# Leqr/MSMP-PDE

Measured on AMD Instinct MI355X. Metric: rollout-steps/sec (whole node), E2 nx=100 tw=25, higher is better.
Workload: dtype f32; 1 GPU; E2 MSMP-PDE (MP_PDE_SolverLEMLinGated), 2048 graphs x nx=100, time_window=25, 6 gated layer pairs, radius graph n=3; graphs_total=2048, graphs_per_gpu=2048, nodes_per_gpu=204800, edges_per_gpu=1204224, parallelism=dp1 (graph-sharded, no collective in the rollout), sub_batches=1, range_policy_switched_to_exact_fp32=False, preheat=170 untimed steps (>= 1 s) after the 5 warm-up steps

## Files before the change

### include/msmp_pde.h

```cpp
#ifndef MSMP_PDE_H
#define MSMP_PDE_H

#include <stddef.h>
#include <stdint.h>

#if defined(__GNUC__)
#pragma GCC visibility push(default)
#endif

#ifdef __cplusplus
extern "C" {
#endif

#define MSMP_HIDDEN 128
#define MSMP_MAX_VARS 8

#define MSMP_OK               0
#define MSMP_ERR_ARG         -1
#define MSMP_ERR_UNSUPPORTED -2
#define MSMP_ERR_WORKSPACE   -3
#define MSMP_ERR_HIP         -4

#define MSMP_LAYER_RESIDUAL_SWISH 0
#define MSMP_LAYER_LIN            1
#define MSMP_LAYER_DENSE_MESSAGE  16

typedef void* msmp_stream_t;

#define MSMP_ABI_VERSION 400
int msmp_version(void);
const char* msmp_last_error(void);

#define MSMP_STATUS_INPUT_RANGE    1
#define MSMP_STATUS_NODE_SATURATED 2
#define MSMP_STATUS_NONFINITE      4
int msmp_last_status(int* flags_out, int reset);
int msmp_tune(const char* key, int value);
int msmp_tune_query(const char* key);

int64_t msmp_packed_layer_floats(int tw, int nv);

int msmp_pack_layer_f32(const float* w1, const float* b1, const float* w2, const float* b2,
                        const float* w3, const float* b3, const float* w4, const float* b4,
                        int tw, int nv, float* packed_out, msmp_stream_t stream);

size_t msmp_build_csr_workspace_bytes(int64_t n_edges, int64_t n_nodes);
int msmp_build_csr(const int64_t* edge_index, int64_t n_edges, int64_t n_nodes,
                   int32_t* rowptr_out, int32_t* col_out, int32_t* tgt_out,
                   void* workspace, size_t workspace_bytes, msmp_stream_t stream);

int msmp_radius_graph_count_f64(const double* x, int dim, const int32_t* graph_ptr, int64_t n_graphs,
                                int64_t n_nodes, double r, int max_neighbors,
                                int32_t* rowptr_out, msmp_stream_t stream);
int msmp_radius_graph_fill_f64(const double* x, int dim, const int32_t* graph_ptr, int64_t n_graphs,
                               int64_t n_nodes, double r, int max_neighbors, const int32_t* rowptr,
                               int64_t n_edges, int64_t* edge_index_out, msmp_stream_t stream);

int msmp_knn_graph_f64(const double* x, int dim, const int32_t* graph_ptr, int64_t n_graphs,
                       int64_t n_nodes, int k, int64_t n_edges, int32_t* rowptr_out,
                       int64_t* edge_index_out, msmp_stream_t stream);

int msmp_edge_mlp_f32(const float* h, const float* u, const float* pos, const float* vars,
                      const int32_t* tgt, const int32_t* col, int64_t n_nodes, int64_t n_edges,
                      int tw, int nv, const float* packed, float* msg_out, msmp_stream_t stream);

int msmp_edge_aggregate_f32(const float* h, const float* u, const float* pos, const float* vars,
                            const int32_t* rowptr, const int32_t* col, const int32_t* tgt,
                            int64_t n_nodes, int64_t n_edges, int max_in_degree, int tw, int nv,
                            const float* packed, float* agg_out, msmp_stream_t stream);

int msmp_node_project_f32(const float* h, const float* u, const float* pos, const float* vars,
                          int64_t n_nodes, int tw, int nv, const float* packed, float* p_out,
                          float* q_out, msmp_stream_t stream);
int msmp_edge_aggregate_projected_f32(const float* p, const float* q, const int32_t* rowptr,
                                      const int32_t* col, const int32_t* tgt, int64_t n_nodes,
                                      int64_t n_edges, int max_in_degree, int tw, int nv,
                                      const float* packed, float* agg_out, msmp_stream_t stream);

#define MSMP_TILE_NCAP  32
#define MSMP_TILE_EDGES 128
typedef struct {
    int32_t tile_nodes;
    int32_t group_nodes;
    int32_t n_tiles;
    const int32_t* tile_node;
    const int32_t* tile_count;
    const int32_t* tile_halo;
    const int32_t* edge_slot;
    int32_t listed;
    int32_t period_tiles;
    int32_t period_nodes;
} msmp_tiles_t;
int msmp_build_tiles(const int32_t* rowptr, const int32_t* col, int64_t n_nodes, int64_t n_edges, int group_nodes,
                     int32_t* tile_node_out, int32_t* tile_count_out, int32_t* tile_halo_out, int32_t* edge_slot_out,
                     int32_t* stats_out, msmp_stream_t stream);
int msmp_node_feature_stride(int tw, int nv);
int msmp_prepare_nodes(const void* x, int x_f64, const void* pos, int pos_f64, int64_t n_nodes, int tw, double L, double tmax,
                       int n_cols, const void* const* cols, const int* col_f64, const double* col_div, float* u_out,
                       float* pos_x_out, float* pos_t_out, float* vars_out, float* feat_out, msmp_stream_t stream);
int msmp_pack_node_features_f32(const float* u, const float* pos, const float* vars, int64_t n_nodes, int tw, int nv,
                                float* feat_out, msmp_stream_t stream);
int msmp_edge_aggregate_tiled_f32(const float* h, const float* u, const float* pos, const float* vars, const float* feat,
                                  const float* p, const float* q, const int32_t* rowptr, const msmp_tiles_t* tiles, int64_t n_nodes,
                                  int64_t n_edges, int tw, int nv, const float* packed, float* agg_out, msmp_stream_t stream);

int msmp_scatter_mean_f32(const float* msg, const int32_t* rowptr, int64_t n_nodes,
                          float* agg_out, msmp_stream_t stream);

int msmp_node_update_f32(const float* h, const float* agg, const float* vars, int64_t n_nodes, int nv,
                         const float* packed, int mode, float* out, msmp_stream_t stream);

int msmp_node_tail_f32(const float* h, const float* agg_main, const float* agg_gate, const float* vars,
                       const int32_t* graph_ptr, int64_t n_nodes, int64_t n_graphs, int max_graph_nodes, int nv,
                       const float* packed_main, const float* packed_gate, int mode, float eps, float* out,
                       msmp_stream_t stream);

int msmp_instance_norm_f32(const float* x, const int32_t* graph_ptr, int64_t n_graphs,
                           int max_graph_nodes, float eps, float* out, msmp_stream_t stream);

int msmp_gate_blend_f32(const float* h, const float* gate_pre, const float* main_pre,
                        const int32_t* graph_ptr, int64_t n_graphs, int max_graph_nodes, float eps,
                        float* out, msmp_stream_t stream);

size_t msmp_mp_layer_workspace_bytes(int64_t n_nodes, int64_t n_edges, int gated, int max_in_degree);
int msmp_mp_layer_f32(const float* h, const float* u, const float* pos, const float* vars,
                      const float* feat, const int32_t* rowptr, const int32_t* col, const int32_t* tgt,
                      const msmp_tiles_t* tiles, const int32_t* graph_ptr, int64_t n_nodes, int64_t n_edges, int64_t n_graphs,
                      int max_in_degree, int max_graph_nodes, int tw, int nv, const float* packed_main,
                      const float* packed_gate, int mode,
                      float eps, float* h_out, void* workspace, size_t workspace_bytes,
                      msmp_stream_t stream);

typedef struct {
    const float* w1;
    const float* b1;
    const float* w2;
    const float* b2;
    const float* u;
    float dt;
    int32_t time_window;
    float* out;
} msmp_decoder_t;
int msmp_mp_layer_decode_f32(const float* h, const float* u, const float* pos, const float* vars,
                             const float* feat, const int32_t* rowptr, const int32_t* col, const int32_t* tgt,
                             const msmp_tiles_t* tiles, const int32_t* graph_ptr, int64_t n_nodes, int64_t n_edges, int64_t n_graphs,
                             int max_in_degree, int max_graph_nodes, int tw, int nv, const float* packed_main,
                             const float* packed_gate, int mode,
                             float eps, float* h_out, const msmp_decoder_t* dec, void* workspace, size_t workspace_bytes,
                             msmp_stream_t stream);

int64_t msmp_packed_lem_floats(void);
int msmp_pack_lem_f32(const float* weights, const float* weights_lin_z, const float* bias,
                      const float* bias_lin_z, const float* mlp_w0, const float* mlp_b0,
                      const float* mlp_w1, const float* mlp_b1, int ninp, float* packed_out,
                      msmp_stream_t stream);

int msmp_lem_input_stride(int ninp);

int msmp_lem_encoder_f32(const float* xin, int64_t n_nodes, int t_len, int ninp, float dt,
                         const float* packed, int with_mlp, float* h_out, msmp_stream_t stream);

int msmp_decoder_f32(const float* h, const float* u, int64_t n_nodes, int tw, const float* w1,
                     const float* b1, const float* w2, const float* b2, float dt, float* out,
                     msmp_stream_t stream);

int msmp_decoder2d_f32(const float* hd, const float* u, int64_t n_nodes, int tw, const float* w1,
                       const float* b1, const float* w2, const float* b2, float dt, float* out,
                       msmp_stream_t stream);

size_t msmp_linear_swish_workspace_bytes(int k, int n_out);
int msmp_linear_swish_f32(const float* x, int64_t rows, int k, const float* w, const float* bias, int n_out, float* out,
                          void* workspace, size_t workspace_bytes, msmp_stream_t stream);

int msmp_lem_encoder_nodes_f32(const float* u, const float* pos_x, const float* pos_t, const float* vars, const float* dt_cum,
                               int64_t n_nodes, int tw, int nv, int two_d, float dt, const float* packed, int with_mlp,
                               float* h_out, msmp_stream_t stream);

int64_t msmp_lem_saved_floats(int64_t n_nodes, int t_len);
int msmp_lem_train_fwd_f32(const float* xin, int64_t n_nodes, int t_len, int ninp, float dt, const float* packed,
                           const float* y0, const float* z0, float* saved, float* y_out, float* z_out, msmp_stream_t stream);
int64_t msmp_packed_lem_bwd_floats(void);
int msmp_pack_lem_bwd_f32(const float* weights, const float* weights_lin_z, int ninp, float* packed_out,
                          msmp_stream_t stream);
int msmp_lem_train_bwd_f32(const float* grad_y, const float* saved, const float* y0, const float* z0, int64_t n_nodes, int t_len,
                           float dt, const float* packed_bwd, float* dg_out, msmp_stream_t stream);

size_t msmp_mp_layer_bwd_workspace_bytes(int64_t n_nodes, int64_t n_edges, int tw, int nv, int gated);
int msmp_mp_layer_bwd_f32(const float* grad_out, const float* h, const float* u, const float* pos, const float* vars,
                          const int32_t* rowptr, const int32_t* col, const int32_t* tgt, const int32_t* src_rowptr,
                          const int32_t* src_perm, const int32_t* graph_ptr,
                          int64_t n_nodes, int64_t n_edges, int64_t n_graphs, int tw, int nv,
                          const float* const* params_main, const float* const* params_gate, int mode, float eps,
                          float* dh_out, float* const* grads_main, float* const* grads_gate, void* workspace,
                          size_t workspace_bytes, msmp_stream_t stream);

int msmp_adamw_f32(int n_tensors, float* const* params, const float* const* grads, float* const* exp_avg,
                   float* const* exp_avg_sq, const int64_t* numel, float lr, float beta1, float beta2, float eps,
                   float weight_decay, int64_t step, msmp_stream_t stream);
int msmp_adamw_capturable_f32(int n_tensors, float* const* params, const float* const* grads, float* const* exp_avg,
                              float* const* exp_avg_sq, const int64_t* numel, const float* lr_dev, float beta1, float beta2,
                              float eps, float weight_decay, int64_t* step_dev, msmp_stream_t stream);

size_t msmp_reduce_workspace_bytes(int cols);
int msmp_colsum_f32(const float* x, int64_t rows, int cols, int group, float* out, void* workspace, size_t workspace_bytes,
                    msmp_stream_t stream);
int msmp_sqerr_sum_f32(const float* a, const float* b, int64_t n, float* out, void* workspace, size_t workspace_bytes,
                       msmp_stream_t stream);

int msmp_edge_concat_f32(const float* h, const float* u, const float* pos, const float* vars, const int32_t* tgt,
                         const int32_t* col, int64_t n_edges, int tw, int nv, int ld, float* out, msmp_stream_t stream);
int msmp_mean_bwd_dswish_f32(const float* dagg, const int32_t* rowptr, const int32_t* tgt, const float* a2, int64_t n_edges,
                             float* out, msmp_stream_t stream);
int msmp_instance_norm_bwd_f32(const float* x, const float* grad_y, const int32_t* graph_ptr, int64_t n_graphs, float eps,
                               float* dx_out, msmp_stream_t stream);
int msmp_gate_blend_bwd_f32(const float* grad_out, const float* h, const float* gate_pre, const float* main_pre,
                            const int32_t* graph_ptr, int64_t n_graphs, float eps, float* d_gate_pre, float* d_main_pre,
                            float* dh_out, msmp_stream_t stream);

int64_t msmp_grad_weights_workspace_floats(int n_jobs, const int64_t* rows, const int* k2);
int msmp_grad_weights_f32(int n_jobs, const float* const* a, const float* const* b, const int64_t* rows, const int* lda,
                          const int* ldb, const int* k2, float* const* out_w, float* const* out_b, float* workspace,
                          int64_t workspace_floats, msmp_stream_t stream);
int msmp_grad_weights_cat_f32(int n_jobs, const float* const* a, const float* const* b, const float* const* b2, const int64_t* rows,
                              const int* lda, const int* ldb, const int* ldb2, const int* ksplit, const int* k2, float* const* out_w,
                              float* const* out_b, float* workspace, int64_t workspace_floats, msmp_stream_t stream);

int64_t msmp_packed_mlp2_floats(int k_in);
int msmp_mlp2_input_stride(int k_in);
int msmp_pack_mlp2_f32(const float* w1, const float* b1, const float* w2, const float* b2, int k_in, float* packed_out,
                       msmp_stream_t stream);
int msmp_mlp2_swish_f32(const float* x, int64_t n_nodes, int k_in, const float* packed, float* out, msmp_stream_t stream);

size_t msmp_linear_workspace_bytes(int k, int n_out);
int msmp_linear_f32(const float* x, int ldx, int64_t rows, int k, const float* w, int ldw, const float* bias, int n_out, int mode,
                    float* out, int ld_out, void* workspace, size_t workspace_bytes, msmp_stream_t stream);
int msmp_wide_gather_swish_f32(const float* p, const float* q, const int32_t* tgt, const int32_t* col, int64_t n_edges, int width, int ld,
                               float* out, msmp_stream_t stream);
int msmp_wide_scatter_mean_f32(const float* msg, const int32_t* rowptr, int64_t n_nodes, int width, int ld, float* agg_out, msmp_stream_t stream);
int msmp_wide_swish_f32(const float* x, int64_t n_floats, float* out, msmp_stream_t stream);
int msmp_wide_lem_z_f32(const float* g, int64_t n_nodes, int width, float dt, float* z, float* dtbar_out, msmp_stream_t stream);
int msmp_wide_lem_y_f32(const float* lin, const float* dtbar, int64_t n_floats, float* y, msmp_stream_t stream);
int msmp_wide_norm_blend_f32(const float* h, const float* gate_pre, const float* main_pre, const int32_t* graph_ptr, int64_t n_graphs,
                             int width, int ld, float eps, float* out, msmp_stream_t stream);

#define MSMP_K_EDGE_MLP     0
#define MSMP_K_SCATTER_MEAN 1
#define MSMP_K_NODE_UPDATE  2
#define MSMP_K_NORM         3
// ... 16 lines not shown
```

### msmp-pde_amd/_lib.py

```python
import ctypes
import os
from ctypes import c_int, c_int64, c_size_t, c_void_p, c_float, c_double, c_char_p

PKG = os.path.dirname(os.path.abspath(__file__))
LIB_PATH = os.environ.get('MSMP_LIB_PATH') or os.path.join(PKG, 'libmsmp_pde.so')

class MsmpTiles(ctypes.Structure):
    _fields_ = [('tile_nodes', ctypes.c_int32), ('group_nodes', ctypes.c_int32), ('n_tiles', ctypes.c_int32), ('tile_node', c_void_p), ('tile_count', c_void_p),
                ('tile_halo', c_void_p), ('edge_slot', c_void_p), ('listed', ctypes.c_int32), ('period_tiles', ctypes.c_int32), ('period_nodes', ctypes.c_int32)]


class MsmpDecoder(ctypes.Structure):
    _fields_ = [('w1', c_void_p), ('b1', c_void_p), ('w2', c_void_p), ('b2', c_void_p), ('u', c_void_p), ('dt', ctypes.c_float),
                ('time_window', ctypes.c_int32), ('out', c_void_p)]


MSMP_TILE_NCAP = 32
MSMP_TILE_EDGES = 128
MSMP_TILE_GROUP_EDGES = 32
MSMP_LAYER_RESIDUAL_SWISH = 0
MSMP_LAYER_LIN = 1
MSMP_ERR_UNSUPPORTED = -2
MSMP_MAX_VARS = 8
HIDDEN = 128
MSMP_ABI_VERSION = 400
MSMP_STATUS_INPUT_RANGE, MSMP_STATUS_NODE_SATURATED, MSMP_STATUS_NONFINITE = 1, 2, 4

SIGNATURES = {
    'msmp_version': (c_int, []),
    'msmp_last_error': (c_char_p, []),
    'msmp_last_status': (c_int, [ctypes.POINTER(c_int), c_int]),
    'msmp_tune': (c_int, [c_char_p, c_int]),
    'msmp_tune_query': (c_int, [c_char_p]),
    'msmp_packed_layer_floats': (c_int64, [c_int, c_int]),
    'msmp_pack_layer_f32': (c_int, [c_void_p] * 8 + [c_int, c_int, c_void_p, c_void_p]),
    'msmp_build_csr_workspace_bytes': (c_size_t, [c_int64, c_int64]),
    'msmp_build_csr': (c_int, [c_void_p, c_int64, c_int64, c_void_p, c_void_p, c_void_p, c_void_p, c_size_t, c_void_p]),
    'msmp_radius_graph_count_f64': (c_int, [c_void_p, c_int, c_void_p, c_int64, c_int64, c_double, c_int, c_void_p, c_void_p]),
    'msmp_radius_graph_fill_f64': (c_int, [c_void_p, c_int, c_void_p, c_int64, c_int64, c_double, c_int, c_void_p, c_int64,
                                           c_void_p, c_void_p]),
    'msmp_knn_graph_f64': (c_int, [c_void_p, c_int, c_void_p, c_int64, c_int64, c_int, c_int64, c_void_p, c_void_p, c_void_p]),
    'msmp_edge_mlp_f32': (c_int, [c_void_p] * 6 + [c_int64, c_int64, c_int, c_int, c_void_p, c_void_p, c_void_p]),
    'msmp_scatter_mean_f32': (c_int, [c_void_p, c_void_p, c_int64, c_void_p, c_void_p]),
    'msmp_node_update_f32': (c_int, [c_void_p, c_void_p, c_void_p, c_int64, c_int, c_void_p, c_int, c_void_p, c_void_p]),
    'msmp_instance_norm_f32': (c_int, [c_void_p, c_void_p, c_int64, c_int, c_float, c_void_p, c_void_p]),
    'msmp_gate_blend_f32': (c_int, [c_void_p, c_void_p, c_void_p, c_void_p, c_int64, c_int, c_float, c_void_p, c_void_p]),
    'msmp_edge_aggregate_f32': (c_int, [c_void_p] * 7 + [c_int64, c_int64, c_int, c_int, c_int, c_void_p, c_void_p, c_void_p]),
    'msmp_node_project_f32': (c_int, [c_void_p] * 4 + [c_int64, c_int, c_int, c_void_p, c_void_p, c_void_p, c_void_p]),
    'msmp_edge_aggregate_projected_f32': (c_int, [c_void_p] * 5 + [c_int64, c_int64, c_int, c_int, c_int, c_void_p, c_void_p, c_void_p]),
    'msmp_build_tiles': (c_int, [c_void_p, c_void_p, c_int64, c_int64, c_int, c_void_p, c_void_p, c_void_p, c_void_p, c_void_p, c_void_p]),
    'msmp_node_feature_stride': (c_int, [c_int, c_int]),
    'msmp_prepare_nodes': (c_int, [c_void_p, c_int, c_void_p, c_int, c_int64, c_int, c_double, c_double, c_int, c_void_p, c_void_p, c_void_p,
                                   c_void_p, c_void_p, c_void_p, c_void_p, c_void_p, c_void_p]),
    'msmp_pack_node_features_f32': (c_int, [c_void_p, c_void_p, c_void_p, c_int64, c_int, c_int, c_void_p, c_void_p]),
    'msmp_edge_aggregate_tiled_f32': (c_int, [c_void_p] * 8 + [ctypes.POINTER(MsmpTiles), c_int64, c_int64, c_int, c_int, c_void_p, c_void_p, c_void_p]),
    'msmp_mp_layer_workspace_bytes': (c_size_t, [c_int64, c_int64, c_int, c_int]),
    'msmp_mp_layer_f32': (c_int, [c_void_p] * 8 + [ctypes.POINTER(MsmpTiles), c_void_p] + [c_int64, c_int64, c_int64, c_int, c_int, c_int, c_int, c_void_p, c_void_p, c_int,
                                                   c_float, c_void_p, c_void_p, c_size_t, c_void_p]),
    'msmp_mp_layer_decode_f32': (c_int, [c_void_p] * 8 + [ctypes.POINTER(MsmpTiles), c_void_p] + [c_int64, c_int64, c_int64, c_int, c_int, c_int, c_int, c_void_p, c_void_p, c_int,
                                                          c_float, c_void_p, ctypes.POINTER(MsmpDecoder), c_void_p, c_size_t, c_void_p]),
    'msmp_packed_lem_floats': (c_int64, []),
    'msmp_pack_lem_f32': (c_int, [c_void_p] * 8 + [c_int, c_void_p, c_void_p]),
    'msmp_lem_input_stride': (c_int, [c_int]),
    'msmp_lem_encoder_f32': (c_int, [c_void_p, c_int64, c_int, c_int, c_float, c_void_p, c_int, c_void_p, c_void_p]),
    'msmp_decoder_f32': (c_int, [c_void_p, c_void_p, c_int64, c_int, c_void_p, c_void_p, c_void_p, c_void_p, c_float, c_void_p, c_void_p]),
    'msmp_decoder2d_f32': (c_int, [c_void_p, c_void_p, c_int64, c_int, c_void_p, c_void_p, c_void_p, c_void_p, c_float, c_void_p, c_void_p]),
    'msmp_node_tail_f32': (c_int, [c_void_p] * 5 + [c_int64, c_int64, c_int, c_int, c_void_p, c_void_p, c_int, c_float, c_void_p, c_void_p]),
    'msmp_lem_encoder_nodes_f32': (c_int, [c_void_p] * 5 + [c_int64, c_int, c_int, c_int, c_float, c_void_p, c_int, c_void_p, c_void_p]),
    'msmp_lem_saved_floats': (c_int64, [c_int64, c_int]),
    'msmp_lem_train_fwd_f32': (c_int, [c_void_p, c_int64, c_int, c_int, c_float] + [c_void_p] * 7),
    'msmp_packed_lem_bwd_floats': (c_int64, []),
    'msmp_pack_lem_bwd_f32': (c_int, [c_void_p, c_void_p, c_int, c_void_p, c_void_p]),
    'msmp_lem_train_bwd_f32': (c_int, [c_void_p] * 4 + [c_int64, c_int, c_float, c_void_p, c_void_p, c_void_p]),
    'msmp_edge_concat_f32': (c_int, [c_void_p] * 6 + [c_int64, c_int, c_int, c_int, c_void_p, c_void_p]),
    'msmp_mean_bwd_dswish_f32': (c_int, [c_void_p] * 4 + [c_int64, c_void_p, c_void_p]),
    'msmp_instance_norm_bwd_f32': (c_int, [c_void_p, c_void_p, c_void_p, c_int64, c_float, c_void_p, c_void_p]),
    'msmp_gate_blend_bwd_f32': (c_int, [c_void_p] * 5 + [c_int64, c_float, c_void_p, c_void_p, c_void_p, c_void_p]),
    'msmp_grad_weights_workspace_floats': (c_int64, [c_int, c_void_p, c_void_p]),
    'msmp_grad_weights_f32': (c_int, [c_int] + [c_void_p] * 9 + [c_int64, c_void_p]),
    'msmp_grad_weights_cat_f32': (c_int, [c_int] + [c_void_p] * 12 + [c_int64, c_void_p]),
    'msmp_mp_layer_bwd_workspace_bytes': (c_size_t, [c_int64, c_int64, c_int, c_int, c_int]),
    'msmp_mp_layer_bwd_f32': (c_int, [c_void_p] * 11 + [c_int64, c_int64, c_int64, c_int, c_int, c_void_p, c_void_p, c_int, c_float,
                                      c_void_p, c_void_p, c_void_p, c_void_p, c_size_t, c_void_p]),
    'msmp_adamw_f32': (c_int, [c_int, c_void_p, c_void_p, c_void_p, c_void_p, c_void_p, c_float, c_float, c_float, c_float, c_float, c_int64, c_void_p]),
    'msmp_adamw_capturable_f32': (c_int, [c_int, c_void_p, c_void_p, c_void_p, c_void_p, c_void_p, c_void_p, c_float, c_float, c_float, c_float, c_void_p, c_void_p]),
    'msmp_reduce_workspace_bytes': (c_size_t, [c_int]),
    'msmp_colsum_f32': (c_int, [c_void_p, c_int64, c_int, c_int, c_void_p, c_void_p, c_size_t, c_void_p]),
    'msmp_sqerr_sum_f32': (c_int, [c_void_p, c_void_p, c_int64, c_void_p, c_void_p, c_size_t, c_void_p]),
    'msmp_packed_mlp2_floats': (c_int64, [c_int]),
    'msmp_mlp2_input_stride': (c_int, [c_int]),
    'msmp_pack_mlp2_f32': (c_int, [c_void_p] * 4 + [c_int, c_void_p, c_void_p]),
    'msmp_mlp2_swish_f32': (c_int, [c_void_p, c_int64, c_int, c_void_p, c_void_p, c_void_p]),
    'msmp_linear_swish_workspace_bytes': (c_size_t, [c_int, c_int]),
    'msmp_linear_swish_f32': (c_int, [c_void_p, c_int64, c_int, c_void_p, c_void_p, c_int, c_void_p, c_void_p, c_size_t, c_void_p]),
    'msmp_linear_workspace_bytes': (c_size_t, [c_int, c_int]),
    'msmp_linear_f32': (c_int, [c_void_p, c_int, c_int64, c_int, c_void_p, c_int, c_void_p, c_int, c_int, c_void_p, c_int, c_void_p, c_size_t, c_void_p]),
    'msmp_wide_gather_swish_f32': (c_int, [c_void_p, c_void_p, c_void_p, c_void_p, c_int64, c_int, c_int, c_void_p, c_void_p]),
    'msmp_wide_scatter_mean_f32': (c_int, [c_void_p, c_void_p, c_int64, c_int, c_int, c_void_p, c_void_p]),
    'msmp_wide_swish_f32': (c_int, [c_void_p, c_int64, c_void_p, c_void_p]),
    'msmp_wide_lem_z_f32': (c_int, [c_void_p, c_int64, c_int, c_float, c_void_p, c_void_p, c_void_p]),
    'msmp_wide_lem_y_f32': (c_int, [c_void_p, c_void_p, c_int64, c_void_p, c_void_p]),
    'msmp_wide_norm_blend_f32': (c_int, [c_void_p, c_void_p, c_void_p, c_void_p, c_int64, c_int, c_int, c_float, c_void_p, c_void_p]),
    'msmp_timing_enable': (c_int, [c_int]),
    'msmp_timing_reset': (c_int, []),
    'msmp_timing_read': (c_int, [c_int, ctypes.POINTER(c_int64), ctypes.POINTER(c_double)]),
}

K_EDGE_MLP, K_SCATTER_MEAN, K_NODE_UPDATE, K_NORM, K_LEM, K_NODE_PROJ, K_DECODER = 0, 1, 2, 3, 4, 5, 6
MSMP_LAYER_DENSE_MESSAGE = 16

_lib = None


class MsmpError(RuntimeError):
    pass


def lib():
    global _lib
    if _lib is None:
        if not os.path.exists(LIB_PATH):
            raise MsmpError(f'{LIB_PATH} not found: build it with `python msmp-pde_amd/build.py` '
                            '(or __graft_entry__.build()); there is no CPU fallback')
        handle = ctypes.CDLL(LIB_PATH)
        for name, (res, args) in SIGNATURES.items():
            fn = getattr(handle, name)
            fn.restype = res
            fn.argtypes = args
        if handle.msmp_version() != MSMP_ABI_VERSION:
            raise MsmpError(f'{LIB_PATH} reports ABI version {handle.msmp_version()}, this binding was written for {MSMP_ABI_VERSION}: '
                            'rebuild it with `python msmp-pde_amd/build.py`')
        _lib = handle
    return _lib


def check(rc, what=''):
    if rc != 0:
        msg = lib().msmp_last_error()
        raise MsmpError(f'{what} failed with code {rc}: {msg.decode() if msg else ""}')


def ptr(t):
    return None if t is None else t.data_ptr()


PARAM_EPOCH = [0]


def invalidate_packed_weights(*_args, **_kwargs):
    PARAM_EPOCH[0] += 1


def _install_optimizer_hook():
    try:
        from torch.optim.optimizer import register_optimizer_step_post_hook
        register_optimizer_step_post_hook(invalidate_packed_weights)
    except Exception as exc:
        import warnings
        warnings.warn(f'msmp_pde_amd: no global optimizer hook ({exc}); call invalidate_packed_weights() after fused optimizer steps')


_install_optimizer_hook()

_raw_stream = None


def current_stream():
    global _raw_stream
    import torch
    if _raw_stream is None:
        _raw_stream = getattr(torch._C, '_cuda_getCurrentRawStream', False)
    if _raw_stream:
        return _raw_stream(torch.cuda.current_device())
    return torch.cuda.current_stream().cuda_stream


def timing_read(kernel):
    n, ms = c_int64(0), c_double(0.0)
    check(lib().msmp_timing_read(kernel, ctypes.byref(n), ctypes.byref(ms)), 'msmp_timing_read')
    return n.value, ms.value


class MsmpRangeWarning(RuntimeWarning):
    """A value left the range the default (fp16-split) kernels represent: results are saturated or not finite."""


_STATUS_TEXT = {
    MSMP_STATUS_INPUT_RANGE: 'an input feature (u, pos / L or a variables column) has |x| > 255 or is not finite',
    MSMP_STATUS_NODE_SATURATED: 'a hidden-state / aggregate row has |x| > 255 or is NaN (saturated at 255.87 in the GEMM operands)',
    MSMP_STATUS_NONFINITE: 'the InstanceNorm statistics of a graph are not finite (an activation above 1023 overflowed fp16 upstream)',
}
_status_seen = [0]


def last_status(reset=False):
    flags = c_int(0)
    check(lib().msmp_last_status(ctypes.byref(flags), int(bool(reset))), 'msmp_last_status')
    if reset:
        _status_seen[0] = 0
    return flags.value


def status_check():
# ... 29 lines not shown
```

### msmp-pde_amd/csrc/aux_kernels.hip

```cpp
#include <stdarg.h>
#include "graph_norm.h"
#include <vector>
#include "mfma_tiles.h"

namespace msmp {

static thread_local char g_err[512] = "";

void set_error(const char* fmt, ...) {
    va_list ap;
    va_start(ap, fmt);
    vsnprintf(g_err, sizeof(g_err), fmt, ap);
    va_end(ap);
}

int check_launch(const char* what) {
    const hipError_t e = hipGetLastError();
    if (e != hipSuccess) {
        set_error("%s: %s", what, hipGetErrorString(e));
        return MSMP_ERR_HIP;
    }
    return MSMP_OK;
}

// ... 367 lines not shown
    MSMP_REQUIRE(flags_out, MSMP_ERR_ARG, "msmp_last_status: null pointer");
    int* dp = status_ptr();
    *flags_out = 0;
    if (g_status_mode == 1) {
        *flags_out = __atomic_load_n(g_status_host, __ATOMIC_RELAXED);
        if (reset) __atomic_store_n(g_status_host, 0, __ATOMIC_RELAXED);
    } else if (g_status_mode == 2) {
        hipError_t e = hipMemcpy(flags_out, dp, sizeof(int), hipMemcpyDeviceToHost);
        if (e == hipSuccess && reset) e = hipMemset(dp, 0, sizeof(int));
        MSMP_REQUIRE(e == hipSuccess, MSMP_ERR_HIP, "msmp_last_status: %s", hipGetErrorString(e));
    } else {
        MSMP_REQUIRE(false, MSMP_ERR_HIP, "msmp_last_status: no status word (allocation failed)");
    }
    return MSMP_OK;
}

extern "C" int msmp_version(void) { return MSMP_ABI_VERSION; }
extern "C" const char* msmp_last_error(void) { return g_err; }

extern "C" int64_t msmp_packed_layer_floats(int tw, int nv) {
    if (tw <= 0 || nv < 1 || nv > MSMP_MAX_VARS) return -1;
    return packed_layout(tw, nv).total;
}

extern "C" int msmp_pack_layer_f32(const float* w1, const float* b1, const float* w2, const float* b2,
                                   const float* w3, const float* b3, const float* w4, const float* b4,
                                   int tw, int nv, float* packed_out, msmp_stream_t stream) {
    MSMP_REQUIRE(w1 && b1 && w2 && b2 && w3 && b3 && w4 && b4 && packed_out, MSMP_ERR_ARG, "msmp_pack_layer_f32: null pointer");
    MSMP_REQUIRE(tw > 0 && nv >= 1 && nv <= MSMP_MAX_VARS, MSMP_ERR_ARG, "msmp_pack_layer_f32: bad tw=%d nv=%d", tw, nv);
    PackArgs a{w1, b1, w2, b2, w3, b3, w4, b4, tw, nv, packed_out};
    hipLaunchKernelGGL(pack_layer_kernel, dim3(256), dim3(256), 0, (hipStream_t)stream, a);
    hipLaunchKernelGGL(pack_layer_scale_kernel, dim3(4), dim3(256), 0, (hipStream_t)stream, a);
    hipLaunchKernelGGL(pack_layer_split_kernel, dim3(256), dim3(256), 0, (hipStream_t)stream, a);
    return check_launch("pack_layer_kernel");
}

extern "C" int msmp_scatter_mean_f32(const float* msg, const int32_t* rowptr, int64_t n_nodes, float* agg_out,
                                     msmp_stream_t stream) {
    MSMP_REQUIRE(rowptr && agg_out, MSMP_ERR_ARG, "msmp_scatter_mean_f32: null pointer");
    MSMP_REQUIRE(n_nodes > 0 && n_nodes < (1L << 31), MSMP_ERR_ARG, "msmp_scatter_mean_f32: bad n_nodes");
    const unsigned grid = (unsigned)((n_nodes + 7) / 8);
    timing_begin(MSMP_K_SCATTER_MEAN, (hipStream_t)stream);
    hipLaunchKernelGGL(scatter_mean_kernel, dim3(grid), dim3(256), 0, (hipStream_t)stream, msg, rowptr, (long)n_nodes, agg_out, msmp_tune_get("split") ? status_ptr() : nullptr);
    timing_end(MSMP_K_SCATTER_MEAN, (hipStream_t)stream);
    return check_launch("scatter_mean_kernel");
}

static const int kRegNormMaxNodes = 128;

extern "C" int msmp_instance_norm_f32(const float* x, const int32_t* graph_ptr, int64_t n_graphs, int max_graph_nodes, float eps,
                                      float* out, msmp_stream_t stream) {
    const int g_max_graph_nodes = max_graph_nodes;
    MSMP_REQUIRE(x && graph_ptr && out, MSMP_ERR_ARG, "msmp_instance_norm_f32: null pointer");
    MSMP_REQUIRE(n_graphs > 0 && n_graphs < (1L << 31), MSMP_ERR_ARG, "msmp_instance_norm_f32: bad n_graphs");
    timing_begin(MSMP_K_NORM, (hipStream_t)stream);
    if (g_max_graph_nodes > 0 && g_max_graph_nodes <= 104)
        hipLaunchKernelGGL(instance_norm_reg_kernel<13>, dim3((unsigned)n_graphs), dim3(256), 0, (hipStream_t)stream, x, graph_ptr, eps, out);
    else if (g_max_graph_nodes > 0 && g_max_graph_nodes <= kRegNormMaxNodes)
        hipLaunchKernelGGL(instance_norm_reg_kernel<16>, dim3((unsigned)n_graphs), dim3(256), 0, (hipStream_t)stream, x, graph_ptr, eps, out);
    else
    hipLaunchKernelGGL(instance_norm_kernel, dim3((unsigned)n_graphs), dim3(256), 0, (hipStream_t)stream, x, graph_ptr, eps, out);
    timing_end(MSMP_K_NORM, (hipStream_t)stream);
    return check_launch("instance_norm_kernel");
}

extern "C" int msmp_gate_blend_f32(const float* h, const float* gate_pre, const float* main_pre, const int32_t* graph_ptr,
                                   int64_t n_graphs, int max_graph_nodes, float eps, float* out, msmp_stream_t stream) {
    const int g_max_graph_nodes = max_graph_nodes;
    MSMP_REQUIRE(h && gate_pre && main_pre && graph_ptr && out, MSMP_ERR_ARG, "msmp_gate_blend_f32: null pointer");
    MSMP_REQUIRE(n_graphs > 0 && n_graphs < (1L << 31), MSMP_ERR_ARG, "msmp_gate_blend_f32: bad n_graphs");
    timing_begin(MSMP_K_NORM, (hipStream_t)stream);
    if (g_max_graph_nodes > 0 && g_max_graph_nodes <= 104)
        hipLaunchKernelGGL(gate_blend_reg_kernel<13>, dim3((unsigned)n_graphs), dim3(256), 0, (hipStream_t)stream, h, gate_pre,
                           main_pre, graph_ptr, eps, out);
    else if (g_max_graph_nodes > 0 && g_max_graph_nodes <= kRegNormMaxNodes)
        hipLaunchKernelGGL(gate_blend_reg_kernel<16>, dim3((unsigned)n_graphs), dim3(256), 0, (hipStream_t)stream, h, gate_pre,
                           main_pre, graph_ptr, eps, out);
    else
    hipLaunchKernelGGL(gate_blend_kernel, dim3((unsigned)n_graphs), dim3(256), 0, (hipStream_t)stream, h, gate_pre, main_pre,
                       graph_ptr, eps, out);
    timing_end(MSMP_K_NORM, (hipStream_t)stream);
    return check_launch("gate_blend_kernel");
}

static size_t align256(size_t b) { return (b + 255) & ~(size_t)255; }
static bool fused_ok(int max_in_degree) { return max_in_degree >= 0 && max_in_degree <= 256; }

extern "C" size_t msmp_mp_layer_workspace_bytes(int64_t n_nodes, int64_t n_edges, int gated, int max_in_degree) {
    const size_t msg = fused_ok(max_in_degree) ? 0 : align256((size_t)n_edges * H * sizeof(float));
    const size_t nod = align256((size_t)n_nodes * H * sizeof(float));
    (void)gated;
    return msg + nod * 6 + 256;
}

static int mp_layer_impl(const float* h, const float* u, const float* pos, const float* vars, const float* feat,
                         const int32_t* rowptr, const int32_t* col, const int32_t* tgt, const msmp_tiles_t* tiles,
                         const int32_t* graph_ptr,
                         int64_t n_nodes, int64_t n_edges, int64_t n_graphs, int max_in_degree, int max_graph_nodes,
                         int tw, int nv, const float* packed_main, const float* packed_gate, int mode, float eps, float* h_out,
                         const msmp_decoder_t* dec, void* workspace, size_t workspace_bytes, msmp_stream_t stream);

extern "C" int msmp_mp_layer_f32(const float* h, const float* u, const float* pos, const float* vars, const float* feat,
                                 const int32_t* rowptr, const int32_t* col, const int32_t* tgt, const msmp_tiles_t* tiles,
                                 const int32_t* graph_ptr,
                                 int64_t n_nodes, int64_t n_edges, int64_t n_graphs, int max_in_degree, int max_graph_nodes,
                                 int tw, int nv, const float* packed_main, const float* packed_gate, int mode, float eps, float* h_out,
                                 void* workspace, size_t workspace_bytes, msmp_stream_t stream) {
    return mp_layer_impl(h, u, pos, vars, feat, rowptr, col, tgt, tiles, graph_ptr, n_nodes, n_edges, n_graphs, max_in_degree, max_graph_nodes, tw, nv,
                         packed_main, packed_gate, mode, eps, h_out, nullptr, workspace, workspace_bytes, stream);
}

extern "C" int msmp_mp_layer_decode_f32(const float* h, const float* u, const float* pos, const float* vars, const float* feat,
                                        const int32_t* rowptr, const int32_t* col, const int32_t* tgt, const msmp_tiles_t* tiles,
                                        const int32_t* graph_ptr,
                                        int64_t n_nodes, int64_t n_edges, int64_t n_graphs, int max_in_degree, int max_graph_nodes,
                                        int tw, int nv, const float* packed_main, const float* packed_gate, int mode, float eps, float* h_out,
                                        const msmp_decoder_t* dec, void* workspace, size_t workspace_bytes, msmp_stream_t stream) {
    MSMP_REQUIRE(dec, MSMP_ERR_ARG, "msmp_mp_layer_decode_f32: null decoder description");
    MSMP_REQUIRE(dec->time_window == 25 && msmp_tune_get("split") && msmp_tune_get("tail") && max_graph_nodes > 0 && max_graph_nodes <= 128,
                 MSMP_ERR_UNSUPPORTED, "msmp_mp_layer_decode_f32: the fused tail does not apply (time_window %d, max_graph_nodes %d)", dec->time_window,
                 max_graph_nodes);
    return mp_layer_impl(h, u, pos, vars, feat, rowptr, col, tgt, tiles, graph_ptr, n_nodes, n_edges, n_graphs, max_in_degree, max_graph_nodes, tw, nv,
                         packed_main, packed_gate, mode, eps, h_out, dec, workspace, workspace_bytes, stream);
}

static int mp_layer_impl(const float* h, const float* u, const float* pos, const float* vars, const float* feat,
                         const int32_t* rowptr, const int32_t* col, const int32_t* tgt, const msmp_tiles_t* tiles,
                         const int32_t* graph_ptr,
                         int64_t n_nodes, int64_t n_edges, int64_t n_graphs, int max_in_degree, int max_graph_nodes,
                         int tw, int nv, const float* packed_main, const float* packed_gate, int mode, float eps, float* h_out,
                         const msmp_decoder_t* dec, void* workspace, size_t workspace_bytes, msmp_stream_t stream) {
    MSMP_REQUIRE(h && u && pos && vars && rowptr && col && tgt && graph_ptr && packed_main && h_out && workspace,
                 MSMP_ERR_ARG, "msmp_mp_layer_f32: null pointer");
    MSMP_REQUIRE(h_out != h, MSMP_ERR_ARG, "msmp_mp_layer_f32: h_out may not alias h");
    MSMP_REQUIRE(!tiles || msmp_tiles_ok(tiles, n_nodes), MSMP_ERR_ARG, "msmp_mp_layer_f32: tile descriptor does not cover %ld nodes", (long)n_nodes);
    const int gated = packed_gate != nullptr;
    const bool dense = (mode & MSMP_LAYER_DENSE_MESSAGE) != 0;
    mode &= ~MSMP_LAYER_DENSE_MESSAGE;
    MSMP_REQUIRE(!gated || mode == MSMP_LAYER_LIN, MSMP_ERR_ARG, "msmp_mp_layer_f32: the gated pair uses GNN_LayerLin layers");
    const size_t need = msmp_mp_layer_workspace_bytes(n_nodes, n_edges, gated, max_in_degree);
    MSMP_REQUIRE(workspace_bytes >= need, MSMP_ERR_WORKSPACE, "msmp_mp_layer_f32: workspace %zu < %zu", workspace_bytes, need);
    const bool fused = fused_ok(max_in_degree);
    char* ws = (char*)workspace;
    float* msg = (float*)ws;
    if (!fused) ws += align256((size_t)n_edges * H * sizeof(float));
    const size_t nod = align256((size_t)n_nodes * H * sizeof(float));
    float* const agg = (float*)ws;
    float* pre_main = (float*)(ws + nod);
    float* pre_gate = (float*)(ws + 2 * nod);
    float* pbuf = (float*)(ws + 3 * nod);
    float* qbuf = (float*)(ws + 4 * nod);
    int rc;
    int tile_mode = (tiles && n_edges > 0 && msmp_tune_get("split")) ? msmp_tune_get("tile") : 0;
    if (tile_mode == 2 && n_edges < (int64_t)76 * tiles->n_tiles) tile_mode = 0;
    if (tile_mode == 3) tile_mode = 2;
    auto aggregate = [&](const float* packed, float* agg) -> int {
        if (fused && !dense && tile_mode == 2)
            return msmp_edge_aggregate_tiled_f32(h, u, pos, vars, feat, nullptr, nullptr, rowptr, tiles, n_nodes, n_edges, tw, nv, packed, agg, stream);
        if (fused && !dense && tile_mode == 1) {
            const int r = msmp_node_project_f32(h, u, pos, vars, n_nodes, tw, nv, packed, pbuf, qbuf, stream);
            return r ? r : msmp_edge_aggregate_tiled_f32(nullptr, nullptr, nullptr, nullptr, nullptr, pbuf, qbuf, rowptr, tiles, n_nodes, n_edges, tw,
                                                         nv, packed, agg, stream);
        }
        if (fused && !dense) {
            const int r = msmp_node_project_f32(h, u, pos, vars, n_nodes, tw, nv, packed, pbuf, qbuf, stream);
            return r ? r : msmp_edge_aggregate_projected_f32(pbuf, qbuf, rowptr, col, tgt, n_nodes, n_edges, max_in_degree, tw,
                                                              nv, packed, agg, stream);
        }
        if (fused)
            return msmp_edge_aggregate_f32(h, u, pos, vars, rowptr, col, tgt, n_nodes, n_edges, max_in_degree, tw, nv, packed,
                                           agg, stream);
        const int r = msmp_edge_mlp_f32(h, u, pos, vars, tgt, col, n_nodes, n_edges, tw, nv, packed, msg, stream);
        return r ? r : msmp_scatter_mean_f32(msg, rowptr, n_nodes, agg, stream);
    };
    if (msmp_tune_get("split") && msmp_tune_get("tail") && max_graph_nodes > 0 && max_graph_nodes <= 128) {
        rc = MSMP_ERR_UNSUPPORTED;
        if (gated && fused && !dense && tile_mode == 2 && msmp_tune_get("pair") && (msmp_tune_get("pair") == 2 || n_nodes <= 65536))
            rc = msmp_edge_aggregate_tiled_pair(h, u, pos, vars, feat, rowptr, tiles, n_nodes, n_edges, tw, nv, packed_gate, packed_main, pre_gate,
                                                agg, stream);
        else if (gated && fused && !dense && !tile_mode)
            rc = msmp_pair_project_aggregate(h, u, pos, vars, rowptr, col, tgt, n_nodes, n_edges, max_in_degree, tw, nv, packed_gate,
                                             packed_main, pbuf, qbuf, pre_main, (float*)(ws + 5 * nod), pre_gate, agg, stream);
        if (rc == MSMP_ERR_UNSUPPORTED) {
            if (gated && (rc = aggregate(packed_gate, pre_gate))) return rc;
            if ((rc = aggregate(packed_main, agg))) return rc;
        } else if (rc) return rc;
        return msmp_node_tail_impl(h, agg, gated ? pre_gate : nullptr, vars, graph_ptr, n_nodes, n_graphs, max_graph_nodes, nv,
                                   packed_main, packed_gate, mode, eps, h_out, dec, stream);
    }
    MSMP_REQUIRE(!dec, MSMP_ERR_UNSUPPORTED, "msmp_mp_layer_decode_f32: the fused tail does not apply");
    if (gated) {
        if ((rc = aggregate(packed_gate, agg))) return rc;
        if ((rc = msmp_node_update_f32(h, agg, vars, n_nodes, nv, packed_gate, MSMP_LAYER_LIN, pre_gate, stream))) return rc;
    }
    if ((rc = aggregate(packed_main, agg))) return rc;
    if ((rc = msmp_node_update_f32(h, agg, vars, n_nodes, nv, packed_main, mode, pre_main, stream))) return rc;
    if (gated) return msmp_gate_blend_f32(h, pre_gate, pre_main, graph_ptr, n_graphs, max_graph_nodes, eps, h_out, stream);
    return msmp_instance_norm_f32(pre_main, graph_ptr, n_graphs, max_graph_nodes, eps, h_out, stream);
}
```

### msmp-pde_amd/csrc/mlp_kernels.hip

```cpp
#include <string.h>
#include "mfma_tiles.h"
#include "decoder_body.h"

namespace msmp {

struct EdgeArgs {
    const float* h;
    const float* u;
    const float* pos;
    const float* vars;
    const int* tgt;
    const int* col;
    const int* rowptr;
    long n_edges, n_nodes;
    int tile_nodes;
    int xcd_map;
    int tw, nv, nc1;
    const float* w1;
    const float* w2;
    const float* w2s;
    const float* scales;
    const float* b1;
    const float* b2;
    const float* P;
// ... 1074 lines not shown
    const int c = lane & 31, hh = lane >> 5;
    const int n0 = a.graph_ptr[blockIdx.x], n1 = a.graph_ptr[blockIdx.x + 1];
    const int cnt = n1 - n0;
    if (cnt <= 0) return;
    const long n = (long)n0 + wave * 32 + c;
    const long nc = n < n1 ? n : n1 - 1;

    PROF_DECL
#pragma unroll
    for (int i = 0; i < 4; ++i) {
        const int e = tid + 256 * i, row = e >> 3, f = e & 7;
        const float v = a.vars[(size_t)min(n0 + row, n1 - 1) * a.nv + min(f, a.nv - 1)];
        xvl[e] = v * (row < cnt && f < a.nv ? 1.0f : 0.f);
    }
    f32x16 tau[4];
    if (GATED) {
        tail_rows_issue(a.h, a.agg[1], n0, n1, 0, rowbuf, tid);
        head_compute(rowbuf, n0, n1, a.h, a.agg[1], a.vars, nc, a.nv, a.b3[1], a.b4[1], a.w3vh[1], a.w3s[1], a.w4t[1], a.scales[1], lds, xvl, tid, lane,
                     c, hh, tau, [&] { tail_rows_issue(a.h, a.agg[0], n0, n1, 0, rowbuf, tid); }, true, tot PROF_PASS);
        PROF_MARK(0);
        tile_t_instance_norm(tau, wave, cnt, uniform_ro(a.scales[1], 7) * (1.0f / TAIL_ACT_SCALE), a.eps, part, tot, tid, c, hh, a.status);
#pragma unroll
        for (int T = 0; T < 4; ++T)
#pragma unroll
            for (int r = 0; r < 16; ++r) tau[T][r] = sigmoidf_(tau[T][r]);
        PROF_MARK(1);
    } else {
        tail_rows_issue(a.h, a.agg[0], n0, n1, 0, rowbuf, tid);
    }
    f32x16 y[4];
    head_compute(rowbuf, n0, n1, a.h, a.agg[0], a.vars, nc, a.nv, a.b3[0], a.b4[0], a.w3vh[0], a.w3s[0], a.w4t[0], a.scales[0], lds, xvl, tid, lane, c, hh,
                 y, [] {}, GATED || a.mode == MSMP_LAYER_LIN, tot PROF_PASS);
    PROF_MARK(2);
    const size_t base = ((size_t)n0 + wave * 32 + 4 * hh) * H + 4 * c;
    const int lim = cnt - wave * 32 - 4 * hh;
    const bool full = wave * 32 + 32 <= cnt;
    const bool need_h = GATED || a.mode != MSMP_LAYER_LIN;
    f32x4 hx[16];
    if (need_h) {
        if (full) {
#pragma unroll
            for (int r = 0; r < 16; ++r) hx[r] = *reinterpret_cast<const f32x4*>(a.h + base + (size_t)((r & 3) + 8 * (r >> 2)) * H);
        } else {
#pragma unroll
            for (int r = 0; r < 16; ++r) {
                const int row = (r & 3) + 8 * (r >> 2);
                hx[r] = row < lim ? *reinterpret_cast<const f32x4*>(a.h + base + (size_t)row * H) : f32x4{0.f, 0.f, 0.f, 0.f};
            }
        }
    }
    float unit = uniform_ro(a.scales[0], 7) * (1.0f / TAIL_ACT_SCALE);
    if (!GATED && a.mode != MSMP_LAYER_LIN) {
#pragma unroll
        for (int T = 0; T < 4; ++T)
#pragma unroll
            for (int r = 0; r < 16; ++r) y[T][r] = hx[r][T] + swishf(y[T][r] * unit);
        unit = 1.0f;
    }
    tile_t_instance_norm(y, wave, cnt, unit, a.eps, part, tot, tid, c, hh, a.status);
    if (need_h) {
        float mx = 0.f;
#pragma unroll
        for (int r = 0; r < 16; ++r) mx = fmaxf(fmaxf(fmaxf(fabsf(hx[r][0]), fabsf(hx[r][1])), fmaxf(fabsf(hx[r][2]), fabsf(hx[r][3]))), mx);
        if (mx > NODE_RANGE) status_raise(a.status, MSMP_STATUS_NODE_SATURATED);
    }
    PROF_MARK(3);
    if (GATED) {
#pragma unroll
        for (int T = 0; T < 4; ++T)
#pragma unroll
            for (int r = 0; r < 16; ++r) y[T][r] = fmaf(tau[T][r], swishf(y[T][r]) - hx[r][T], hx[r][T]);
    }
    if (full) {
#pragma unroll
        for (int r = 0; r < 16; ++r)
            *reinterpret_cast<f32x4*>(a.out + base + (size_t)((r & 3) + 8 * (r >> 2)) * H) = f32x4{y[0][r], y[1][r], y[2][r], y[3][r]};
    } else {
#pragma unroll
        for (int r = 0; r < 16; ++r) {
            const int row = (r & 3) + 8 * (r >> 2);
            if (row < lim) *reinterpret_cast<f32x4*>(a.out + base + (size_t)row * H) = f32x4{y[0][r], y[1][r], y[2][r], y[3][r]};
        }
    }
    PROF_MARK(4);
    if (a.dec.w1) {
        using G = DecSplit<25, 16, 3, 14>;
        static_assert(16 * 8 * G::LP <= 2 * SPLIT_CHUNK_FLOATS && 16 * 8 * G::LP <= 2 * ROWBUF_FLOATS, "decoder tables must fit the dead buffers");
        __syncthreads();
        const int q = tid & 7, nl = tid >> 3;
        float* mrow = (nl < 16 ? lds : rowbuf) + (nl & 15) * 8 * G::LP;
        for (int p = 0; p < cnt; p += 32) {
            const bool live = p + nl < cnt;
            const long nn = live ? (long)n0 + p + nl : (long)n1 - 1;
            decoder_split_node<25, 16, 3, 14, true>(a.out + (size_t)nn * H, mrow, q, live, nn, a.dec, [] { __syncthreads(); });
            __syncthreads();
        }
    }
    PROF_FLUSH
}

}

using namespace msmp;

extern int g_lem_tail;
extern int g_lem_share;
static int* split_status() { return msmp_tune_get("split") ? msmp::status_ptr() : nullptr; }
static int g_split = 1;

extern "C" int msmp_edge_mlp_f32(const float* h, const float* u, const float* pos, const float* vars,
                                 const int32_t* tgt, const int32_t* col, int64_t n_nodes, int64_t n_edges,
                                 int tw, int nv, const float* packed, float* msg_out, msmp_stream_t stream) {
    MSMP_REQUIRE(h && u && pos && vars && tgt && col && packed && msg_out, MSMP_ERR_ARG, "msmp_edge_mlp_f32: null pointer");
    MSMP_REQUIRE(n_nodes > 0 && n_edges >= 0 && tw > 0 && nv >= 1 && nv <= MSMP_MAX_VARS, MSMP_ERR_ARG,
                 "msmp_edge_mlp_f32: bad sizes N=%ld E=%ld tw=%d nv=%d", (long)n_nodes, (long)n_edges, tw, nv);
    MSMP_REQUIRE(n_edges < (1L << 31) && n_nodes < (1L << 31), MSMP_ERR_UNSUPPORTED, "msmp_edge_mlp_f32: int32 index range");
    if (n_edges == 0) return MSMP_OK;
    const PackedLayout L = packed_layout(tw, nv);
    EdgeArgs a{h, u, pos, vars, tgt, col, nullptr, (long)n_edges, (long)n_nodes, 0, 0, tw, nv, L.nc1,
               packed + L.w1, packed + L.w2, packed + L.w2s, packed + L.scales, packed + L.b1, packed + L.b2, nullptr, nullptr, msg_out, nullptr, split_status()};
    constexpr int NB = 2;
    const unsigned grid = (unsigned)((n_edges + 128 * NB - 1) / (128 * NB));
    timing_begin(MSMP_K_EDGE_MLP, (hipStream_t)stream);
    hipLaunchKernelGGL((edge_mlp_kernel<NB, false, false>), dim3(grid), dim3(256), 0, (hipStream_t)stream, a);
    timing_end(MSMP_K_EDGE_MLP, (hipStream_t)stream);
    return check_launch("edge_mlp_kernel");
}

extern "C" int msmp_node_project_f32(const float* h, const float* u, const float* pos, const float* vars, int64_t n_nodes,
                                     int tw, int nv, const float* packed, float* p_out, float* q_out, msmp_stream_t stream) {
    MSMP_REQUIRE(h && u && pos && vars && packed && p_out && q_out, MSMP_ERR_ARG, "msmp_node_project_f32: null pointer");
    MSMP_REQUIRE(n_nodes > 0 && n_nodes < (1L << 31) && tw > 0 && nv >= 1 && nv <= MSMP_MAX_VARS, MSMP_ERR_ARG,
                 "msmp_node_project_f32: bad sizes");
    const PackedLayout L = packed_layout(tw, nv);
    ProjArgs a{h, u, pos, vars, (long)n_nodes, tw, nv, L.nc1, packed + L.w1, packed + L.b1, p_out, q_out};
    const unsigned grid = (unsigned)((n_nodes + 127) / 128);
    timing_begin(MSMP_K_NODE_PROJ, (hipStream_t)stream);
    if (g_split) {
        ProjSplitArgs sa{a, packed + L.w1t, packed + L.scales};
        hipLaunchKernelGGL(node_proj_split_kernel, dim3(grid), dim3(256), 0, (hipStream_t)stream, sa);
    } else
        hipLaunchKernelGGL(node_proj_kernel, dim3(grid), dim3(256), 0, (hipStream_t)stream, a);
    timing_end(MSMP_K_NODE_PROJ, (hipStream_t)stream);
    return check_launch("node_proj_kernel");
}

static int g_edge_nb = 0;

static int g_pair = 1;
constexpr int64_t PAIR_MAX_NODES = 65536;
static int g_decoder = 1;
static int g_tile_arith = 1;
static int g_tile_align = 0;
static int g_tile = 2;
static int g_bwd_gemm = 1;
static int g_dec_fuse = 0;
static int g_tail = 1;
int msmp_tune_get(const char* key) {
    if (!strcmp(key, "split")) return g_split;
    if (!strcmp(key, "tail")) return g_tail;
    if (!strcmp(key, "bwd_gemm")) return g_bwd_gemm;
    if (!strcmp(key, "pair")) return g_pair;
    if (!strcmp(key, "tile")) return g_tile;
    if (!strcmp(key, "tile_arith")) return g_tile_arith;
    if (!strcmp(key, "tile_align")) return g_tile_align;
    if (!strcmp(key, "decoder")) return g_decoder;
    if (!strcmp(key, "dec_fuse")) return g_dec_fuse;
    if (!strcmp(key, "lem_tail")) return g_lem_tail;
    if (!strcmp(key, "lem_share")) return g_lem_share;
    return 0;
}

extern "C" int msmp_tune_query(const char* key) { return key ? msmp_tune_get(key) : 0; }

extern "C" int msmp_tune(const char* key, int value) {
    if (key && !strcmp(key, "tail")) { g_tail = value; return MSMP_OK; }
    if (key && !strcmp(key, "bwd_gemm")) { g_bwd_gemm = value; return MSMP_OK; }
    if (key && !strcmp(key, "pair")) { g_pair = value; return MSMP_OK; }
    if (key && !strcmp(key, "tile")) { g_tile = value; return MSMP_OK; }
    if (key && !strcmp(key, "tile_arith")) { g_tile_arith = value; return MSMP_OK; }
    if (key && !strcmp(key, "tile_align")) { g_tile_align = value; return MSMP_OK; }
    if (key && !strcmp(key, "decoder")) { g_decoder = value != 0; return MSMP_OK; }
    if (key && !strcmp(key, "dec_fuse")) { g_dec_fuse = value != 0; return MSMP_OK; }
    if (key && !strcmp(key, "lem_tail")) { g_lem_tail = value != 0; return MSMP_OK; }
    if (key && !strcmp(key, "lem_share") && value >= 1 && value <= 16) { g_lem_share = value; return MSMP_OK; }
    if (key && !strcmp(key, "edge_nb")) { g_edge_nb = value; return MSMP_OK; }
    if (key && !strcmp(key, "split")) { g_split = value; return MSMP_OK; }
    msmp::set_error("msmp_tune: unknown key");
    return MSMP_ERR_ARG;
}

static int edge_aggregate(const float* h, const float* u, const float* pos, const float* vars, const float* P, const float* Q,
                          const int32_t* rowptr, const int32_t* col, const int32_t* tgt, int64_t n_nodes, int64_t n_edges,
                          int max_in_degree, int tw, int nv, const float* packed, float* agg_out, msmp_stream_t stream,
                          const char* who) {
    MSMP_REQUIRE(rowptr && col && tgt && packed && agg_out, MSMP_ERR_ARG, "%s: null pointer", who);
    MSMP_REQUIRE(n_nodes > 0 && n_edges >= 0 && tw > 0 && nv >= 1 && nv <= MSMP_MAX_VARS && max_in_degree >= 0, MSMP_ERR_ARG,
                 "%s: bad sizes", who);
    MSMP_REQUIRE(n_edges < (1L << 31) && n_nodes < (1L << 31), MSMP_ERR_UNSUPPORTED, "%s: int32 index range", who);
    if (n_edges == 0) {
        const hipError_t me = hipMemsetAsync(agg_out, 0, (size_t)n_nodes * H * sizeof(float), (hipStream_t)stream);
        MSMP_REQUIRE(me == hipSuccess, MSMP_ERR_HIP, "%s: memset: %s", who, hipGetErrorString(me));
        return MSMP_OK;
    }
    MSMP_REQUIRE(max_in_degree <= 256, MSMP_ERR_UNSUPPORTED,
                 "%s: max in-degree %d > 256 (use msmp_edge_mlp_f32 + msmp_scatter_mean_f32)", who, max_in_degree);
    const int edges_per_tile = (P && max_in_degree <= 128 && g_edge_nb != 2) ? 128 : 256;
    const PackedLayout L = packed_layout(tw, nv);
    int tile_nodes = max_in_degree > 0 ? edges_per_tile / max_in_degree : edges_per_tile;
    if (tile_nodes > 256) tile_nodes = 256;
    EdgeArgs a{h, u, pos, vars, tgt, col, rowptr, (long)n_edges, (long)n_nodes, tile_nodes, 0, tw, nv, L.nc1,
               packed + L.w1, packed + L.w2, packed + L.w2s, packed + L.scales, packed + L.b1, packed + L.b2, P, Q, nullptr, agg_out, split_status()};
    const unsigned grid = (unsigned)((n_nodes + tile_nodes - 1) / tile_nodes);
    timing_begin(MSMP_K_EDGE_MLP, (hipStream_t)stream);
    if (P && edges_per_tile == 128 && g_split) hipLaunchKernelGGL((edge_mlp_kernel_occ2<1, true, true, true>), dim3(grid), dim3(256), 0, (hipStream_t)stream, a);
    else if (P && edges_per_tile == 128) hipLaunchKernelGGL((edge_mlp_kernel<1, true, true>), dim3(grid), dim3(256), 0, (hipStream_t)stream, a);
    else if (P) hipLaunchKernelGGL((edge_mlp_kernel<2, true, true>), dim3(grid), dim3(256), 0, (hipStream_t)stream, a);
    else hipLaunchKernelGGL((edge_mlp_kernel<2, true, false>), dim3(grid), dim3(256), 0, (hipStream_t)stream, a);
    timing_end(MSMP_K_EDGE_MLP, (hipStream_t)stream);
    return check_launch("edge_mlp_kernel<fused mean>");
}

int msmp_pair_project_aggregate(const float* h, const float* u, const float* pos, const float* vars, const int32_t* rowptr,
                                const int32_t* col, const int32_t* tgt, int64_t n_nodes, int64_t n_edges, int max_in_degree, int tw,
                                int nv, const float* packed_a, const float* packed_b, float* p_a, float* q_a, float* p_b, float* q_b,
                                float* agg_a, float* agg_b, msmp_stream_t stream) {
    if (!g_pair || (g_pair == 1 && n_nodes > PAIR_MAX_NODES)) return MSMP_ERR_UNSUPPORTED;
    if (!g_split || g_edge_nb == 2) return MSMP_ERR_UNSUPPORTED;
    if (n_edges <= 0 || max_in_degree <= 0 || max_in_degree > 128 || n_edges >= (1L << 31) || n_nodes >= (1L << 31)) return MSMP_ERR_UNSUPPORTED;
    const PackedLayout L = packed_layout(tw, nv);
    hipStream_t st = (hipStream_t)stream;
    ProjSplitArgs2 pa;
    const float* packed[2] = {packed_a, packed_b};
    float* pp[2] = {p_a, p_b};
    float* qq[2] = {q_a, q_b};
    float* agg[2] = {agg_a, agg_b};
    for (int i = 0; i < 2; ++i)
        pa.head[i] = ProjSplitArgs{ProjArgs{h, u, pos, vars, (long)n_nodes, tw, nv, L.nc1, packed[i] + L.w1, packed[i] + L.b1, pp[i], qq[i]},
                                   packed[i] + L.w1t, packed[i] + L.scales};
    timing_begin(MSMP_K_NODE_PROJ, st);
    hipLaunchKernelGGL(node_proj_split_pair_kernel, dim3((unsigned)((n_nodes + 127) / 128), 2), dim3(256), 0, st, pa);
    timing_end(MSMP_K_NODE_PROJ, st);
    int tile_nodes = 128 / max_in_degree;
    if (tile_nodes > 256) tile_nodes = 256;
    EdgeArgs2 ea;
    for (int i = 0; i < 2; ++i)
        ea.head[i] = EdgeArgs{nullptr, nullptr, nullptr, nullptr, tgt, col, rowptr, (long)n_edges, (long)n_nodes, tile_nodes, 0, tw, nv, L.nc1,
                              packed[i] + L.w1, packed[i] + L.w2, packed[i] + L.w2s, packed[i] + L.scales, packed[i] + L.b1,
                              packed[i] + L.b2, pp[i], qq[i], nullptr, agg[i], split_status()};
    timing_begin(MSMP_K_EDGE_MLP, st);
    hipLaunchKernelGGL(edge_mlp_pair_kernel_occ2, dim3((unsigned)((n_nodes + tile_nodes - 1) / tile_nodes), 2), dim3(256), 0, st, ea);
    timing_end(MSMP_K_EDGE_MLP, st);
    return check_launch("edge_mlp_pair_kernel_occ2");
}

extern "C" int msmp_edge_aggregate_f32(const float* h, const float* u, const float* pos, const float* vars,
                                       const int32_t* rowptr, const int32_t* col, const int32_t* tgt, int64_t n_nodes,
                                       int64_t n_edges, int max_in_degree, int tw, int nv, const float* packed,
                                       float* agg_out, msmp_stream_t stream) {
    MSMP_REQUIRE(h && u && pos && vars, MSMP_ERR_ARG, "msmp_edge_aggregate_f32: null pointer");
    return edge_aggregate(h, u, pos, vars, nullptr, nullptr, rowptr, col, tgt, n_nodes, n_edges, max_in_degree, tw, nv, packed,
                          agg_out, stream, "msmp_edge_aggregate_f32");
}

extern "C" int msmp_edge_aggregate_projected_f32(const float* p, const float* q, const int32_t* rowptr, const int32_t* col,
                                                 const int32_t* tgt, int64_t n_nodes, int64_t n_edges, int max_in_degree,
                                                 int tw, int nv, const float* packed, float* agg_out, msmp_stream_t stream) {
    MSMP_REQUIRE(p && q, MSMP_ERR_ARG, "msmp_edge_aggregate_projected_f32: null pointer");
    return edge_aggregate(nullptr, nullptr, nullptr, nullptr, p, q, rowptr, col, tgt, n_nodes, n_edges, max_in_degree, tw, nv,
                          packed, agg_out, stream, "msmp_edge_aggregate_projected_f32");
}

#if MSMP_PROF
extern "C" __attribute__((visibility("default"))) int msmp_debug_prof(unsigned long long* out16, int reset) {
    if (reset) { unsigned long long z[16] = {0}; return (int)hipMemcpyToSymbol(HIP_SYMBOL(g_prof), z, sizeof(z)); }
    return (int)hipMemcpyFromSymbol(out16, HIP_SYMBOL(g_prof), 16 * sizeof(unsigned long long));
}
#endif

extern "C" int msmp_node_tail_f32(const float* h, const float* agg_main, const float* agg_gate, const float* vars,
                                  const int32_t* graph_ptr, int64_t n_nodes, int64_t n_graphs, int max_graph_nodes, int nv,
                                  const float* packed_main, const float* packed_gate, int mode, float eps, float* out,
                                  msmp_stream_t stream) {
    return msmp_node_tail_impl(h, agg_main, agg_gate, vars, graph_ptr, n_nodes, n_graphs, max_graph_nodes, nv, packed_main, packed_gate, mode,
                               eps, out, nullptr, stream);
}

int msmp_node_tail_impl(const float* h, const float* agg_main, const float* agg_gate, const float* vars, const int32_t* graph_ptr,
                        int64_t n_nodes, int64_t n_graphs, int max_graph_nodes, int nv, const float* packed_main, const float* packed_gate,
                        int mode, float eps, float* out, const msmp_decoder_t* dec, msmp_stream_t stream) {
    MSMP_REQUIRE(h && agg_main && vars && graph_ptr && packed_main && out, MSMP_ERR_ARG, "msmp_node_tail_f32: null pointer");
    MSMP_REQUIRE((agg_gate != nullptr) == (packed_gate != nullptr), MSMP_ERR_ARG, "msmp_node_tail_f32: give both gate arguments or none");
    MSMP_REQUIRE(n_nodes > 0 && n_graphs > 0 && n_graphs < (1L << 31) && nv >= 1 && nv <= MSMP_MAX_VARS, MSMP_ERR_ARG,
                 "msmp_node_tail_f32: bad sizes");
    MSMP_REQUIRE(mode == MSMP_LAYER_LIN || mode == MSMP_LAYER_RESIDUAL_SWISH, MSMP_ERR_ARG, "msmp_node_tail_f32: bad mode %d", mode);
    MSMP_REQUIRE(!packed_gate || mode == MSMP_LAYER_LIN, MSMP_ERR_ARG, "msmp_node_tail_f32: the gated pair uses GNN_LayerLin layers");
    MSMP_REQUIRE(out != h, MSMP_ERR_ARG, "msmp_node_tail_f32: out may not alias h");
    MSMP_REQUIRE(max_graph_nodes > 0 && max_graph_nodes <= 128, MSMP_ERR_UNSUPPORTED,
                 "msmp_node_tail_f32: graphs of up to 128 nodes (got max_graph_nodes=%d); use the piecewise entry points", max_graph_nodes);
    MSMP_REQUIRE(g_split, MSMP_ERR_UNSUPPORTED, "msmp_node_tail_f32: only on the fp16-split matrix path");
    const PackedLayout L = packed_layout(1, nv);
    const float* pg = packed_gate ? packed_gate : packed_main;
    TailArgs a{h, {agg_main, agg_gate}, vars, graph_ptr, nv, mode, eps,
               {packed_main + L.b3, pg + L.b3}, {packed_main + L.b4, pg + L.b4}, {packed_main + L.w3vh, pg + L.w3vh},
               {packed_main + L.w3s, pg + L.w3s}, {packed_main + L.w4t, pg + L.w4t}, {packed_main + L.scales, pg + L.scales}, out, split_status(), DecW{}};
    if (dec) {
        MSMP_REQUIRE(dec->w1 && dec->b1 && dec->w2 && dec->b2 && dec->out, MSMP_ERR_ARG, "msmp_mp_layer_decode_f32: null pointer in the decoder description");
        MSMP_REQUIRE(dec->time_window == 25, MSMP_ERR_UNSUPPORTED, "msmp_mp_layer_decode_f32: the fused decoder is built for time_window 25 (got %d)", dec->time_window);
        a.dec = DecW{dec->w1, dec->b1, dec->w2, dec->b2, dec->u, dec->dt, dec->out};
    }
    timing_begin(MSMP_K_NODE_UPDATE, (hipStream_t)stream);
    if (packed_gate) hipLaunchKernelGGL(node_tail_split_kernel<true>, dim3((unsigned)n_graphs), dim3(256), 0, (hipStream_t)stream, a);
    else hipLaunchKernelGGL(node_tail_split_kernel<false>, dim3((unsigned)n_graphs), dim3(256), 0, (hipStream_t)stream, a);
    timing_end(MSMP_K_NODE_UPDATE, (hipStream_t)stream);
    return check_launch("node_tail_split_kernel");
}

extern "C" int msmp_node_update_f32(const float* h, const float* agg, const float* vars, int64_t n_nodes, int nv,
                                    const float* packed, int mode, float* out, msmp_stream_t stream) {
    MSMP_REQUIRE(h && agg && vars && packed && out, MSMP_ERR_ARG, "msmp_node_update_f32: null pointer");
    MSMP_REQUIRE(n_nodes > 0 && nv >= 1 && nv <= MSMP_MAX_VARS, MSMP_ERR_ARG, "msmp_node_update_f32: bad sizes");
    MSMP_REQUIRE(mode == MSMP_LAYER_LIN || mode == MSMP_LAYER_RESIDUAL_SWISH, MSMP_ERR_ARG, "msmp_node_update_f32: bad mode %d", mode);
    MSMP_REQUIRE(out != h, MSMP_ERR_ARG, "msmp_node_update_f32: out may not alias h");
    const PackedLayout L = packed_layout(1, nv);
    NodeArgs a{h, agg, vars, (long)n_nodes, nv, mode, packed + L.w3, packed + L.w4,
               packed + L.b3, packed + L.b4, packed + L.w3v, out};
    constexpr int NB = 1;
    const unsigned grid = (unsigned)((n_nodes + 128 * NB - 1) / (128 * NB));
    timing_begin(MSMP_K_NODE_UPDATE, (hipStream_t)stream);
    if (g_split) {
        NodeSplitArgs sa{a, packed + L.w3s, packed + L.scales};
        hipLaunchKernelGGL(node_update_split_kernel, dim3(grid), dim3(256), 0, (hipStream_t)stream, sa);
    } else
        hipLaunchKernelGGL(node_update_kernel<NB>, dim3(grid), dim3(256), 0, (hipStream_t)stream, a);
// ... 4 lines not shown
```

### msmp-pde_amd/csrc/tile_kernels.hip

```cpp
#include "mfma_tiles.h"

#define TILE_SCHED_BARRIER() __builtin_amdgcn_sched_barrier(0)

namespace msmp {

#if MSMP_PROF_TILE
__device__ unsigned long long g_prof_tile[16];
#define TPROF_DECL unsigned pacc[12] = {0, 0, 0, 0, 0, 0, 0, 0, 0, 0, 0, 0}; unsigned tp = (unsigned)__builtin_readcyclecounter();
#define TPROF(i) do { const unsigned t_ = (unsigned)__builtin_readcyclecounter(); pacc[i] += t_ - tp; tp = t_; } while (0)
#define TPROF_FLUSH if (tid == 0 && (blockIdx.x & 63) == 0) { for (int i_ = 0; i_ < 12; ++i_) atomicAdd(&g_prof_tile[i_], (unsigned long long)pacc[i_]); atomicAdd(&g_prof_tile[15], 1ull); }
#else
#define TPROF_DECL
#define TPROF(i)
#define TPROF_FLUSH
#endif

constexpr int TILE_NCAP = MSMP_TILE_NCAP;
constexpr int TILE_EDGES = MSMP_TILE_EDGES;
constexpr int PQLD = H + 4;
constexpr int BROW_T = 72;
constexpr int FRAG_SKEW = 32;
__device__ __forceinline__ int frag_row(int chunk, int slot) { return (chunk * 32 + slot) * BROW_T + chunk * FRAG_SKEW; }
constexpr float ACT_SCALE = 64.0f;
constexpr float NODE_SCALE = 256.0f;
constexpr float NODE_MAX = 65504.0f;
__device__ __forceinline__ float node_scaled(float x) { return __builtin_amdgcn_fmed3f(x * NODE_SCALE, -NODE_MAX, NODE_MAX); }

__global__ __launch_bounds__(128) void build_tiles_kernel(const int* __restrict__ rowptr, const int* __restrict__ col, int n_nodes,
                                                          int tile_nodes, int group_nodes, int* __restrict__ tile_node,
                                                          int* __restrict__ tile_count, int* __restrict__ tile_halo,
                                                          int* __restrict__ edge_slot, int* __restrict__ stats) {
    __shared__ int s_col[TILE_EDGES];
    __shared__ int s_first[TILE_EDGES];
    __shared__ int s_slot[TILE_EDGES];
    __shared__ int s_halo[5];
    __shared__ int s_stat[6];
    const int t = blockIdx.x, k = threadIdx.x;
    const int n0 = t * tile_nodes, n1 = min(n0 + tile_nodes, n_nodes);
    const int nt = n1 - n0;
    const int g = k >> 5, kk = k & 31;
    const int gf = min(n0 + g * group_nodes, n1), gl = min(gf + group_nodes, n1);
    const int ge0 = rowptr[gf], ge1 = rowptr[gl];
    const bool valid = kk < ge1 - ge0 && kk < 32;
    const int e = ge0 + kk;
    int j = -1;
    if (valid) j = col[e];
    s_col[k] = j;
    __syncthreads();
    int first = 0, owner = k;
    if (valid && (j < n0 || j >= n1)) {
        first = 1;
        for (int i = 0; i < k; ++i)
            if (s_col[i] == j) { first = 0; owner = i; break; }
    }
    s_first[k] = first;
    if (k < 6) s_stat[k] = (k == 0 || k == 3) ? 0x7fffffff : (k == 1 || k == 4) ? -1 : 0;
    __syncthreads();
    if (first) {
        int* st3 = s_stat + (j < n0 ? 0 : 3);
        atomicMin(st3, j);
        atomicMax(st3 + 1, j);
        atomicAdd(st3 + 2, 1);
    }
    __syncthreads();
    if (k == 0) {
        const int lo_min = s_stat[0], lo_max = s_stat[1], lo_cnt = s_stat[2], hi_min = s_stat[3], hi_max = s_stat[4], hi_cnt = s_stat[5];
        const bool ranged = (lo_cnt == 0 || lo_max - lo_min + 1 == lo_cnt) && (hi_cnt == 0 || hi_max - hi_min + 1 == hi_cnt);
        s_halo[0] = lo_cnt ? lo_min : 0; s_halo[1] = lo_cnt; s_halo[2] = hi_cnt ? hi_min : 0; s_halo[3] = hi_cnt; s_halo[4] = ranged;
    }
    __syncthreads();
    const bool ranged = s_halo[4] != 0;
    int slot = 0;
    if (valid) {
        if (j >= n0 && j < n1) slot = j - n0;
        else if (ranged) slot = j < n0 ? nt + (j - s_halo[0]) : nt + s_halo[1] + (j - s_halo[2]);
        else if (first) {
            int before = 0;
            for (int i = 0; i < k; ++i) before += s_first[i];
            slot = nt + before;
        }
    }
    s_slot[k] = slot;
    __syncthreads();
    if (valid && !(j >= n0 && j < n1) && !first && !ranged) slot = s_slot[owner];
    if (valid) {
        int ts = gf - n0;
        while (ts + 1 < gl - n0 && rowptr[n0 + ts + 1] <= e) ++ts;
        edge_slot[(size_t)t * TILE_EDGES + k] = ts | (min(slot, 255) << 8);
        if (first && slot < TILE_NCAP) tile_node[(size_t)t * TILE_NCAP + slot] = j;
    } else
        edge_slot[(size_t)t * TILE_EDGES + k] = 0;
    if (k < TILE_NCAP && k < nt) tile_node[(size_t)t * TILE_NCAP + k] = n0 + k;
    __syncthreads();
    const int total = nt + s_stat[2] + s_stat[5];
    if (k == 0) {
        tile_count[t] = min(total, TILE_NCAP);
        const bool use = ranged && total <= TILE_NCAP;
        tile_halo[4 * t + 0] = use ? s_halo[0] : 0;
        tile_halo[4 * t + 1] = use ? s_halo[1] : -1;
        tile_halo[4 * t + 2] = use ? s_halo[2] : 0;
        tile_halo[4 * t + 3] = use ? s_halo[3] : 0;
        atomicMax(&stats[0], total);
        if (!use) atomicAdd(&stats[2], 1);
    }
    if (kk == 0) atomicMax(&stats[1], ge1 - ge0);
    __syncthreads();
    if (k < TILE_NCAP && k >= total) tile_node[(size_t)t * TILE_NCAP + k] = n0;
}

__global__ __launch_bounds__(256) void pack_features_kernel(const float* __restrict__ u, const float* __restrict__ pos,
                                                            const float* __restrict__ vars, long n, int tw, int nv, int stride,
                                                            float* __restrict__ out, int* status) {
    const long i = (long)blockIdx.x * 256 + threadIdx.x;
    if (i >= n * stride) return;
    const long node = i / stride;
    const int k = (int)(i - node * stride);
    float v = 0.f;
    if (k < tw) v = u[node * tw + k];
    else if (k == tw) v = pos[node];
    else if (k <= tw + nv) v = vars[node * nv + (k - tw - 1)];
    out[i] = v;
    if (out_of_range(v)) status_raise(status, MSMP_STATUS_INPUT_RANGE);
}

struct PrepArgs {
    const void* x;
    const void* pos;
    const void* col[MSMP_MAX_VARS];
    double col_div[MSMP_MAX_VARS];
    int col_f64[MSMP_MAX_VARS];
    int x_f64, pos_f64, n_cols;
    double L, tmax;
    long n;
    int tw, stride;
    float *u, *pos_x, *pos_t, *vars, *feat;
    int* status;
};
__device__ __forceinline__ float prep_load(const void* p, int f64, long i) {
    return f64 ? (float)reinterpret_cast<const double*>(p)[i] : reinterpret_cast<const float*>(p)[i];
}
__device__ __forceinline__ float prep_div(const void* p, int f64, long i, double d) {
    return f64 ? (float)(reinterpret_cast<const double*>(p)[i] / d) : reinterpret_cast<const float*>(p)[i] / (float)d;
}
__global__ __launch_bounds__(256) void prepare_nodes_kernel(PrepArgs a) {
    const int groups = a.stride >> 2;
    const long i = (long)blockIdx.x * 256 + threadIdx.x;
    if (i >= a.n * groups) return;
    const long node = groups == 8 ? i >> 3 : (groups == 16 ? i >> 4 : i / groups);
    const int k0 = 4 * (int)(i - node * groups);
    const int nv = 1 + a.n_cols;
    f32x4 out = {0.f, 0.f, 0.f, 0.f};
    bool bad = false;
#pragma unroll
    for (int m = 0; m < 4; ++m) {
        const int k = k0 + m;
        float v = 0.f;
        if (k < a.tw) {
            v = prep_load(a.x, a.x_f64, node * a.tw + k);
            a.u[node * a.tw + k] = v;
        } else if (k == a.tw) {
            v = prep_div(a.pos, a.pos_f64, 2 * node + 1, a.L);
            a.pos_x[node] = v;
        } else if (k == a.tw + 1) {
            v = prep_div(a.pos, a.pos_f64, 2 * node, a.tmax);
            a.pos_t[node] = v;
            a.vars[node * nv] = v;
        } else if (k <= a.tw + nv) {
            const int c = k - a.tw - 2;
            v = prep_div(a.col[c], a.col_f64[c], node, a.col_div[c]);
            a.vars[node * nv + 1 + c] = v;
        }
        out[m] = v;
        bad |= out_of_range(v);
    }
    if (a.feat) *reinterpret_cast<f32x4*>(a.feat + node * a.stride + k0) = out;
    if (bad) status_raise(a.status, MSMP_STATUS_INPUT_RANGE);
}

struct TileArgs {
    const float* h;
    const float* u;
    const float* pos;
    const float* vars;
    const float* feat;
    const float* P;
    const float* Q;
    const int* rowptr;
    const int* tile_node;
    const int* tile_halo;
    const int* edge_slot;
    long n_nodes, n_edges;
    int tile_nodes, group_nodes;
    int period_tiles, period_nodes;
    unsigned period_magic;
    int tw, nv, nc1;
    const float* w1s;
    const float* w2s;
    const float* scales;
    const float* b1;
    const float* b2;
    float* agg;
    int* status;
};

constexpr int WHALF_FLOATS = SPLIT_CHUNK_FLOATS / 2;
constexpr int WBUF_FLOATS = 2 * WHALF_FLOATS;
constexpr int TILE_MAIN_FLOATS = WBUF_FLOATS + 2 * TILE_NCAP * PQLD;
constexpr int TILE_LUT_FLOATS = 32;
constexpr int TILE_LDS_FLOATS = TILE_MAIN_FLOATS + TILE_LUT_FLOATS;
static_assert((8 * 32 * BROW_T + 8 * FRAG_SKEW) * 2 <= TILE_MAIN_FLOATS * 4, "fragment tile of the folded projections must fit");

struct WHalf {
    f32x4 r[2];
};
__device__ __forceinline__ void whalf_load(WHalf& w, const float* __restrict__ half_chunk, int tid) {
#pragma unroll
    for (int i = 0; i < 2; ++i) w.r[i] = *reinterpret_cast<const f32x4*>(half_chunk + 4 * (tid + 256 * i));
}
__device__ __forceinline__ void whalf_store(const WHalf& w, float* buf, int tid) {
#pragma unroll
    for (int i = 0; i < 2; ++i) *reinterpret_cast<f32x4*>(buf + 4 * (tid + 256 * i)) = w.r[i];
}
__device__ __forceinline__ void whalf_dma(const float* __restrict__ half_chunk, float* buf, int tid) {
#pragma unroll
    for (int i = 0; i < 2; ++i)
        __builtin_amdgcn_global_load_lds((const __attribute__((address_space(1))) void*)(half_chunk + 4 * (tid + 256 * i)),
                                         (__attribute__((address_space(3))) void*)(buf + 4 * (tid + 256 * i)), 16, 0, 0);
}

using half4v = __attribute__((ext_vector_type(4))) _Float16;

template <int MODE, bool LISTED>
__device__ __forceinline__ void edge_tile_body(const TileArgs& a, float* lds) {
    constexpr bool FOLD = MODE != 0;
    float* wbuf = lds;
    float* pl = lds + WBUF_FLOATS;
    float* ql = pl + TILE_NCAP * PQLD;
    const int tid = threadIdx.x, lane = tid & 63, wave = tid >> 6;
    const int c = lane & 31, hh = lane >> 5;
    TPROF_DECL
    constexpr bool packed_feat = MODE == 2;
    int tm = blockIdx.x, node_off = 0;
    long n_end = a.n_nodes;
    if (a.period_tiles > 0) {
        const int q = a.period_tiles == 1 ? (int)blockIdx.x : (int)__umulhi((unsigned)blockIdx.x, a.period_magic);
        tm = (int)blockIdx.x - q * a.period_tiles;
        node_off = q * a.period_nodes;
        n_end = (long)node_off + a.period_nodes;
    }
    const int tile_n0 = node_off + tm * a.tile_nodes;
    const int tile_n1 = (int)min((long)tile_n0 + a.tile_nodes, n_end);
    const int nt_ = tile_n1 - tile_n0;
    int h_lo = 0, h_nlo = 0, h_hi = 0, h_nhi = 0;
    if (!LISTED) {
        h_lo = a.tile_halo[4 * tm] + node_off; h_nlo = a.tile_halo[4 * tm + 1]; h_hi = a.tile_halo[4 * tm + 2] + node_off; h_nhi = a.tile_halo[4 * tm + 3];
    }
    auto node_of = [&](int slot) -> int {
        const int r = slot - nt_;
        int node = r < h_nlo + h_nhi ? h_hi + (r - h_nlo) : tile_n0;
        node = r < h_nlo ? h_lo + r : node;
        node = r < 0 ? tile_n0 + slot : node;
        return node;
    };

    const int sl = a.edge_slot[(size_t)tm * TILE_EDGES + wave * 32 + c];
    const int gf = min(tile_n0 + wave * a.group_nodes, tile_n1), gl = min(gf + a.group_nodes, tile_n1);
    const int* rp = a.rowptr - node_off;
    const int rp_base = rp[__builtin_amdgcn_readfirstlane(gf)];
    const int rp_row = gf + min(c, max(gl - gf - 1, 0));
    int rp_lo = rp[rp_row], rp_hi = rp[rp_row + 1];
    int er0 = 0, edeg = 0;
    auto edge_ranges = [&]() {
        __builtin_amdgcn_sched_barrier(0);
        asm volatile("" : "+v"(rp_lo), "+v"(rp_hi));
        er0 = rp_lo - rp_base;
        edeg = c < gl - gf ? rp_hi - rp_lo : 0;
    };
    if (tid < 16) {
        unsigned* lut = reinterpret_cast<unsigned*>(lds + TILE_MAIN_FLOATS);
        lut[2 * tid] = ((tid & 1) ? 0x3C00u : 0u) | ((tid & 2) ? 0x3C000000u : 0u);
        lut[2 * tid + 1] = ((tid & 4) ? 0x3C00u : 0u) | ((tid & 8) ? 0x3C000000u : 0u);
    }
    const float* prow = pl + (sl & 255) * PQLD + 4 * hh;
    const float* qrow = ql + ((sl >> 8) & 255) * PQLD + 4 * hh;

    float b2v[4];
    int rnode[4], fnode;
    if (LISTED) {
        const int* tnode = a.tile_node + (size_t)tm * TILE_NCAP;
#pragma unroll
        for (int i = 0; i < 4; ++i) rnode[i] = tnode[(tid >> 5) + 8 * i];
        fnode = tnode[tid >> 3];
#pragma unroll
        for (int i = 0; i < 4; ++i) rnode[i] += node_off;
        fnode += node_off;
    } else {
#pragma unroll
        for (int i = 0; i < 4; ++i) rnode[i] = node_of((tid >> 5) + 8 * i);
        fnode = node_of(tid >> 3);
    }

    WHalf ws;
    whalf_load(ws, a.w2s, tid);

    if (!FOLD) {
        const int piece = tid & 31;
        f32x4 pv[4], qv[4];
#pragma unroll
        for (int i = 0; i < 4; ++i) {
            pv[i] = *reinterpret_cast<const f32x4*>(a.P + (size_t)rnode[i] * H + 4 * piece) * ACT_SCALE;
            qv[i] = *reinterpret_cast<const f32x4*>(a.Q + (size_t)rnode[i] * H + 4 * piece) * ACT_SCALE;
        }
#pragma unroll
        for (int T = 0; T < 4; ++T) b2v[T] = a.b2[32 * T + c];
        edge_ranges();
#pragma unroll
        for (int i = 0; i < 4; ++i) {
            const int slot = (tid >> 5) + 8 * i;
            *reinterpret_cast<f32x4*>(pl + slot * PQLD + 4 * piece) = pv[i];
            *reinterpret_cast<f32x4*>(ql + slot * PQLD + 4 * piece) = qv[i];
        }
        whalf_store(ws, wbuf, tid);
        __syncthreads();
        TPROF(0);
    } else {
        _Float16* bt = reinterpret_cast<_Float16*>(lds);
        const int ntail = a.nc1 - 8;
        unsigned woff = (unsigned)((wave * 2 * 64 + lane) * 16);
        asm volatile("" : "+v"(woff));
        auto wfrag = [&](int ch, int s, int plane) {
            const char* base = reinterpret_cast<const char*>(a.w1s) + (size_t)ch * (SPLIT_CHUNK_FLOATS * 4) + (s * 8 + plane) * 1024;
            return *reinterpret_cast<const half8*>(base + woff);
        };
        half8 wp[3][2][2], wq[3][2][2];
        f32x4 b1v[4];
        auto wload = [&](int i) {
            const int chp = i < 4 ? i : 8, chq = i < 4 ? 4 + i : (ntail > 1 ? 9 : 8);
#pragma unroll
            for (int s = 0; s < 2; ++s)
#pragma unroll
                for (int p = 0; p < 2; ++p) { wp[i % 3][s][p] = wfrag(chp, s, p); wq[i % 3][s][p] = wfrag(chq, s, p); }
        };
        {
            f32x4 hv[4];
#pragma unroll
            for (int i = 0; i < 4; ++i) hv[i] = *reinterpret_cast<const f32x4*>(a.h + (size_t)rnode[i] * H + 4 * (tid & 31));
            const int g = tid & 7;
            float tx[2][4] = {{0.f, 0.f, 0.f, 0.f}, {0.f, 0.f, 0.f, 0.f}};
            if (packed_feat) {
#pragma unroll
                for (int jc = 0; jc < 2; ++jc) {
                    const bool on = jc < ntail;
                    const f32x4 fv = *reinterpret_cast<const f32x4*>(a.feat + (size_t)fnode * (32 * ntail) + 32 * (on ? jc : 0) + 4 * g);
#pragma unroll
                    for (int m = 0; m < 4; ++m) tx[jc][m] = on ? fv[m] : 0.f;
                }
            } else {
#pragma unroll
                for (int jc = 0; jc < 2; ++jc)
                    if (jc < ntail) {
#pragma unroll
                        for (int m = 0; m < 4; ++m) {
                            const int k = 32 * jc + 4 * g + m;
                            const float uv = a.u[(size_t)fnode * a.tw + min(k, a.tw - 1)];
                            const float vv = a.vars[(size_t)fnode * a.nv + min(max(k - a.tw - 1, 0), a.nv - 1)];
                            tx[jc][m] = k < a.tw ? uv : (k == a.tw ? a.pos[fnode] : (k <= a.tw + a.nv ? vv : 0.f));
                        }
                    }
            }
#pragma unroll
            for (int q = 0; q < 4; ++q) b1v[q] = *reinterpret_cast<const f32x4*>(a.b1 + 32 * wave + 8 * q + 4 * hh);
            wload(0);
            wload(1);
            edge_ranges();
#pragma unroll
            for (int i = 0; i < 4; ++i) {
                half2v h01, l01, h23, l23;
                split_node_pair(hv[i][0], hv[i][1], h01, l01);
                split_node_pair(hv[i][2], hv[i][3], h23, l23);
                const int piece = tid & 31;
                _Float16* row = bt + frag_row(piece >> 3, (tid >> 5) + 8 * i) + 4 * (piece & 7);
                *reinterpret_cast<half4v*>(row) = half4v{h01[0], h01[1], h23[0], h23[1]};
                *reinterpret_cast<half4v*>(row + 32) = half4v{l01[0], l01[1], l23[0], l23[1]};
            }
#pragma unroll
            for (int jc = 0; jc < 2; ++jc) {
                if (jc < ntail) {
                    half2v ph[2], pl2[2], qh[2], ql2[2];
#pragma unroll
                    for (int m = 0; m < 2; ++m) {
                        split_node_pair(tx[jc][2 * m], tx[jc][2 * m + 1], ph[m], pl2[m]);
                        const int k = 32 * jc + 4 * g + 2 * m;
                        const half2v nm = {(_Float16)(k <= a.tw ? -1.f : 0.f), (_Float16)(k + 1 <= a.tw ? -1.f : 0.f)};
                        qh[m] = ph[m] * nm;
                        ql2[m] = pl2[m] * nm;
                    }
                    _Float16* rp_ = bt + frag_row(4 + 2 * jc, tid >> 3) + 4 * g;
                    _Float16* rq_ = bt + frag_row(5 + 2 * jc, tid >> 3) + 4 * g;
                    *reinterpret_cast<half4v*>(rp_) = half4v{ph[0][0], ph[0][1], ph[1][0], ph[1][1]};
                    *reinterpret_cast<half4v*>(rp_ + 32) = half4v{pl2[0][0], pl2[0][1], pl2[1][0], pl2[1][1]};
                    *reinterpret_cast<half4v*>(rq_) = half4v{qh[0][0], qh[0][1], qh[1][0], qh[1][1]};
                    *reinterpret_cast<half4v*>(rq_ + 32) = half4v{ql2[0][0], ql2[0][1], ql2[1][0], ql2[1][1]};
                }
            }
        }
        __syncthreads();
        TPROF(0);

        const float sc = uniform_ro(a.scales, 0) * NODE_SCALE;
        f32x16 accP, accQ;
#pragma unroll
        for (int q = 0; q < 4; ++q) {
            const f32x4 bv = b1v[q];
#pragma unroll
            for (int m = 0; m < 4; ++m) { accP[4 * q + m] = bv[m] * sc; accQ[4 * q + m] = 0.f; }
        }
        auto afrag = [&](int ch, half8 (&ahi)[2], half8 (&alo)[2]) {
            const _Float16* row = bt + frag_row(ch, c) + 8 * hh;
#pragma unroll
            for (int s = 0; s < 2; ++s) {
                ahi[s] = *reinterpret_cast<const half8*>(row + 16 * s);
                alo[s] = *reinterpret_cast<const half8*>(row + 32 + 16 * s);
            }
        };
        auto mma3 = [&](f32x16& acc, const half8& ahi, const half8& alo, const half8& whi, const half8& wlo) {
            MSMP_MFMA_LOLO(2, acc, wlo, alo);
            acc = __builtin_amdgcn_mfma_f32_32x32x16_f16(wlo, ahi, acc, 0, 0, 0);
            acc = __builtin_amdgcn_mfma_f32_32x32x16_f16(whi, alo, acc, 0, 0, 0);
            acc = __builtin_amdgcn_mfma_f32_32x32x16_f16(whi, ahi, acc, 0, 0, 0);
        };
#pragma unroll
        for (int ch = 0; ch < 4; ++ch) {
            const int cur = ch % 3;
            if (ch + 2 < 4 || (ch + 2 == 4 && ntail > 0)) wload(ch + 2);
            half8 ahi[2], alo[2];
            afrag(ch, ahi, alo);
#pragma unroll
            for (int s = 0; s < 2; ++s) {
                mma3(accP, ahi[s], alo[s], wp[cur][s][0], wp[cur][s][1]);
                mma3(accQ, ahi[s], alo[s], wq[cur][s][0], wq[cur][s][1]);
            }
        }
        for (int jc = 0; jc < ntail; ++jc) {
            half8 phi[2], plo[2], qhi[2], qlo[2];
            afrag(4 + 2 * jc, phi, plo);
            afrag(5 + 2 * jc, qhi, qlo);
#pragma unroll
            for (int s = 0; s < 2; ++s) {
                const half8 whi = jc == 0 ? wp[1][s][0] : wq[1][s][0], wlo = jc == 0 ? wp[1][s][1] : wq[1][s][1];
                mma3(accP, phi[s], plo[s], whi, wlo);
                mma3(accQ, qhi[s], qlo[s], whi, wlo);
            }
        }
        TPROF(1);
#pragma unroll
        for (int T = 0; T < 4; ++T) b2v[T] = a.b2[32 * T + c];
        __syncthreads();
#pragma unroll
        for (int q = 0; q < 4; ++q) {
            *reinterpret_cast<f32x4*>(pl + c * PQLD + 32 * wave + 8 * q + 4 * hh) = f32x4{accP[4 * q], accP[4 * q + 1], accP[4 * q + 2], accP[4 * q + 3]};
            *reinterpret_cast<f32x4*>(ql + c * PQLD + 32 * wave + 8 * q + 4 * hh) = f32x4{accQ[4 * q], accQ[4 * q + 1], accQ[4 * q + 2], accQ[4 * q + 3]};
        }
        whalf_store(ws, wbuf, tid);
        __syncthreads();
        TPROF(2);
    }

    f32x16 y[4];
    {
        const float s2 = uniform_ro(a.scales, 1) * ACT_SCALE;
#pragma unroll
        for (int T = 0; T < 4; ++T) {
            float bv = b2v[T] * s2;
            asm volatile("" : "+v"(bv));
#pragma unroll
            for (int r = 0; r < 16; ++r) y[T][r] = bv;
        }
        __builtin_amdgcn_sched_barrier(0);
    }
    f32x4 pq[4];
    auto gather_step = [&](int t, int s) {
#pragma unroll
        for (int j = 0; j < 2; ++j) {
            pq[j] = *reinterpret_cast<const f32x4*>(prow + 32 * t + 16 * s + 8 * j);
            pq[2 + j] = *reinterpret_cast<const f32x4*>(qrow + 32 * t + 16 * s + 8 * j);
        }
    };
    float zt[8];
    const float act_g = FOLD ? uniform_ro(a.scales, 0) * (NODE_SCALE / ACT_SCALE) : 1.0f;
    const float act_ct = (-1.44269504088896340736f / ACT_SCALE) * (FOLD ? uniform_ro(a.scales, 4) * (ACT_SCALE / NODE_SCALE) : 1.0f);
    auto act_slice = [&](int i) {
        const int j = i >> 1, m0 = 2 * (i & 1);
#if MSMP_PRECISE_ACT
        for (int m = m0; m < m0 + 2; ++m) zt[4 * j + m] = ACT_SCALE * swishf((pq[j][m] + pq[2 + j][m]) * (1.0f / (ACT_SCALE * act_g)));
        (void)act_ct;
#else
        const f32x2 x = f32x2{pq[j][m0], pq[j][m0 + 1]} + f32x2{pq[2 + j][m0], pq[2 + j][m0 + 1]};
        const f32x2 t = x * f32x2{act_ct, act_ct};
        const f32x2 d = f32x2{__builtin_amdgcn_exp2f(t[0]), __builtin_amdgcn_exp2f(t[1])} * f32x2{act_g, act_g} + f32x2{act_g, act_g};
        const f32x2 z = x * f32x2{__builtin_amdgcn_rcpf(d[0]), __builtin_amdgcn_rcpf(d[1])};
        zt[4 * j + m0] = z[0];
        zt[4 * j + m0 + 1] = z[1];
#endif
    };
    half8 bhi[2], blo[2];
    gather_step(0, 0);
#pragma unroll
    for (int i = 0; i < 4; ++i) act_slice(i);
    split8(zt, bhi[0], blo[0]);
    TPROF(3);
#pragma unroll
    for (int u = 0; u < 7; ++u) {
        const int par = u & 1;
        whalf_dma(a.w2s + (size_t)(u + 1) * WHALF_FLOATS, wbuf + (par ^ 1) * WHALF_FLOATS, tid);
        const half8* w = reinterpret_cast<const half8*>(wbuf + par * WHALF_FLOATS) + lane;
        half8 ahi[4], alo[4];
#pragma unroll
        for (int T = 0; T < 2; ++T) {
            ahi[T] = w[(T * 2 + 0) * 64];
            alo[T] = w[(T * 2 + 1) * 64];
        }
        gather_step((u + 1) >> 1, (u + 1) & 1);
#pragma unroll
        for (int T = 2; T < 4; ++T) {
            ahi[T] = w[(T * 2 + 0) * 64];
            alo[T] = w[(T * 2 + 1) * 64];
        }
        TILE_SCHED_BARRIER();
#pragma unroll
        for (int T = 0; T < 4; ++T) {
            MSMP_MFMA_LOLO(2, y[T], blo[par], alo[T]);
            y[T] = __builtin_amdgcn_mfma_f32_32x32x16_f16(bhi[par], alo[T], y[T], 0, 0, 0);
            y[T] = __builtin_amdgcn_mfma_f32_32x32x16_f16(blo[par], ahi[T], y[T], 0, 0, 0);
            y[T] = __builtin_amdgcn_mfma_f32_32x32x16_f16(bhi[par], ahi[T], y[T], 0, 0, 0);
            TILE_SCHED_BARRIER();
            act_slice(T);
            if (T == 3) split8(zt, bhi[par ^ 1], blo[par ^ 1]);
            TILE_SCHED_BARRIER();
        }
        TPROF(4);
        __syncthreads();
        TPROF(5);
    }

    const float kinv = uniform_ro(a.scales, 1);
    const float inv2 = uniform_ro(a.scales, 5) * (1.0f / ACT_SCALE);
    const float cexp = -1.44269504088896340736f * inv2;
    auto swish2 = [&](int T, int r0, int r1) {
#pragma unroll
        for (int r = r0; r < r1; r += 2) {
#if MSMP_PRECISE_ACT
            y[T][r] = ACT_SCALE * swishf(y[T][r] * inv2);
            y[T][r + 1] = ACT_SCALE * swishf(y[T][r + 1] * inv2);
            (void)kinv; (void)cexp;
#else
            const f32x2 yy = {y[T][r], y[T][r + 1]};
            const f32x2 t = yy * f32x2{cexp, cexp};
            const f32x2 e = f32x2{__builtin_amdgcn_exp2f(t[0]), __builtin_amdgcn_exp2f(t[1])};
            const f32x2 d = e * f32x2{kinv, kinv} + f32x2{kinv, kinv};
            const f32x2 z = yy * f32x2{__builtin_amdgcn_rcpf(d[0]), __builtin_amdgcn_rcpf(d[1])};
            y[T][r] = z[0];
            y[T][r + 1] = z[1];
#endif
        }
    };
    half8 sf[2];
    {
        constexpr int par = 1;
        const half8* w = reinterpret_cast<const half8*>(wbuf + par * WHALF_FLOATS) + lane;
        half8 ahi[4], alo[4];
#pragma unroll
        for (int T = 0; T < 4; ++T) {
            ahi[T] = w[(T * 2 + 0) * 64];
            alo[T] = w[(T * 2 + 1) * 64];
        }
        TILE_SCHED_BARRIER();
#pragma unroll
        for (int T = 0; T < 4; ++T) {
            MSMP_MFMA_LOLO(2, y[T], blo[par], alo[T]);
            y[T] = __builtin_amdgcn_mfma_f32_32x32x16_f16(bhi[par], alo[T], y[T], 0, 0, 0);
            TILE_SCHED_BARRIER();
            if (T > 0) swish2(T - 1, 0, 6);
            TILE_SCHED_BARRIER();
            y[T] = __builtin_amdgcn_mfma_f32_32x32x16_f16(blo[par], ahi[T], y[T], 0, 0, 0);
            TILE_SCHED_BARRIER();
            if (T > 0) swish2(T - 1, 6, 12);
            TILE_SCHED_BARRIER();
            y[T] = __builtin_amdgcn_mfma_f32_32x32x16_f16(bhi[par], ahi[T], y[T], 0, 0, 0);
            TILE_SCHED_BARRIER();
            if (T > 0) swish2(T - 1, 12, 16);
            if (T == 0) {
                const unsigned mask = edeg >= 32 ? 0xffffffffu : ((1u << edeg) - 1u) << (er0 & 31);
                const char* lut = reinterpret_cast<const char*>(lds + TILE_MAIN_FLOATS);
                using u32x2 = __attribute__((ext_vector_type(2))) unsigned;
#pragma unroll
                for (int s = 0; s < 2; ++s) {
                    const u32x2 lo = *reinterpret_cast<const u32x2*>(lut + 8 * ((mask >> (16 * s + 4 * hh)) & 15u));
                    const u32x2 hi = *reinterpret_cast<const u32x2*>(lut + 8 * ((mask >> (16 * s + 8 + 4 * hh)) & 15u));
                    const u32x4 wv = {lo[0], lo[1], hi[0], hi[1]};
                    sf[s] = __builtin_bit_cast(half8, wv);
                }
            }
            TILE_SCHED_BARRIER();
        }
        TPROF(4);
    }
    f32x4 fr[4];
    {
        float* ftab = pl + wave * 32;
        if (hh == 0) ftab[c] = (1.0f / ACT_SCALE) / (float)max(edeg, 1);
#pragma unroll
        for (int q = 0; q < 4; ++q) fr[q] = *reinterpret_cast<const f32x4*>(ftab + 8 * q + 4 * hh);
    }
    {
        half8 mh[2], ml[2];
        auto splitT = [&](int T) {
#pragma unroll
            for (int s = 0; s < 2; ++s) {
                float v[8];
#pragma unroll
                for (int j = 0; j < 8; ++j) v[j] = y[T][8 * s + j];
                split8(v, mh[s], ml[s]);
            }
        };
        splitT(0);
#pragma unroll
        for (int T = 0; T < 4; ++T) {
            const half8 h0 = mh[0], l0 = ml[0], h1 = mh[1], l1 = ml[1];
            f32x16 z16;
#pragma unroll
            for (int r = 0; r < 16; ++r) z16[r] = 0.f;
            TILE_SCHED_BARRIER();
            y[T] = __builtin_amdgcn_mfma_f32_32x32x16_f16(sf[0], l0, z16, 0, 0, 0);
            TILE_SCHED_BARRIER();
            if (T == 0) swish2(3, 0, 8);
            TILE_SCHED_BARRIER();
            y[T] = __builtin_amdgcn_mfma_f32_32x32x16_f16(sf[0], h0, y[T], 0, 0, 0);
            TILE_SCHED_BARRIER();
            if (T == 0) swish2(3, 8, 16);
            TILE_SCHED_BARRIER();
            y[T] = __builtin_amdgcn_mfma_f32_32x32x16_f16(sf[1], l1, y[T], 0, 0, 0);
            TILE_SCHED_BARRIER();
            if (T < 3) splitT(T + 1);
            TILE_SCHED_BARRIER();
            y[T] = __builtin_amdgcn_mfma_f32_32x32x16_f16(sf[1], h1, y[T], 0, 0, 0);
            TILE_SCHED_BARRIER();
        }
    }
    TPROF(7);
    {
        const int ng = gl - gf;
        float* out = a.agg + (size_t)gf * H + c;
        bool bad = false;
#pragma unroll
        for (int q = 0; q < 4; ++q) {
            if (8 * q < ng) {
#pragma unroll
                for (int m = 0; m < 4; ++m) {
                    const int row = 8 * q + 4 * hh + m;
                    if (row < ng) {
#pragma unroll
                        for (int T = 0; T < 4; ++T) {
                            const float v = y[T][4 * q + m] * fr[q][m];
                            out[(size_t)row * H + 32 * T] = v;
                            bad |= out_of_range(v);
                        }
                    }
                }
            }
        }
        if (bad) status_raise(a.status, MSMP_STATUS_NODE_SATURATED);
    }
    TPROF(9);
    TPROF_FLUSH
}

template <int MODE, bool LISTED>
__global__ __launch_bounds__(256, 3) void edge_tile_kernel(TileArgs a) {
    __shared__ __attribute__((aligned(16))) float lds[TILE_LDS_FLOATS];
    edge_tile_body<MODE, LISTED>(a, lds);
}

struct TileArgs2 {
    TileArgs head[2];
};
template <int MODE, bool LISTED>
__global__ __launch_bounds__(256, 3) void edge_tile_pair_kernel(TileArgs2 a) {
    __shared__ __attribute__((aligned(16))) float lds[TILE_LDS_FLOATS];
    edge_tile_body<MODE, LISTED>(a.head[blockIdx.y], lds);
}

}

using namespace msmp;

#if MSMP_PROF_TILE
extern "C" __attribute__((visibility("default"))) int msmp_debug_prof_tile(unsigned long long* out16, int reset) {
    if (reset) { unsigned long long z[16] = {0}; return (int)hipMemcpyToSymbol(HIP_SYMBOL(g_prof_tile), z, sizeof(z)); }
    return (int)hipMemcpyFromSymbol(out16, HIP_SYMBOL(g_prof_tile), 16 * sizeof(unsigned long long));
}
#endif

extern "C" int msmp_node_feature_stride(int tw, int nv) {
    if (tw <= 0 || nv < 1 || nv > MSMP_MAX_VARS) return -1;
    return 32 * tail_chunks(tw, nv);
}

extern "C" int msmp_pack_node_features_f32(const float* u, const float* pos, const float* vars, int64_t n_nodes, int tw, int nv,
                                           float* feat_out, msmp_stream_t stream) {
    MSMP_REQUIRE(u && pos && vars && feat_out, MSMP_ERR_ARG, "msmp_pack_node_features_f32: null pointer");
    const int stride = msmp_node_feature_stride(tw, nv);
    MSMP_REQUIRE(n_nodes > 0 && stride > 0, MSMP_ERR_ARG, "msmp_pack_node_features_f32: bad sizes");
    const long total = (long)n_nodes * stride;
    hipLaunchKernelGGL(pack_features_kernel, dim3((unsigned)((total + 255) / 256)), dim3(256), 0, (hipStream_t)stream, u, pos, vars,
                       (long)n_nodes, tw, nv, stride, feat_out, msmp_tune_get("split") ? status_ptr() : nullptr);
    return check_launch("pack_features_kernel");
}

extern "C" int msmp_prepare_nodes(const void* x, int x_f64, const void* pos, int pos_f64, int64_t n_nodes, int tw, double L, double tmax,
                                  int n_cols, const void* const* cols, const int* col_f64, const double* col_div, float* u_out,
                                  float* pos_x_out, float* pos_t_out, float* vars_out, float* feat_out, msmp_stream_t stream) {
    MSMP_REQUIRE(x && pos && u_out && pos_x_out && pos_t_out && vars_out && (n_cols == 0 || (cols && col_f64 && col_div)), MSMP_ERR_ARG,
                 "msmp_prepare_nodes: null pointer");
    MSMP_REQUIRE(n_nodes > 0 && tw > 0 && n_cols >= 0 && n_cols < MSMP_MAX_VARS, MSMP_ERR_ARG, "msmp_prepare_nodes: bad sizes");
    const int stride = msmp_node_feature_stride(tw, 1 + n_cols);
    MSMP_REQUIRE(stride > 0 && stride <= 64 + 32, MSMP_ERR_ARG, "msmp_prepare_nodes: bad sizes");
    PrepArgs a{};
    a.x = x; a.pos = pos; a.x_f64 = x_f64; a.pos_f64 = pos_f64; a.n_cols = n_cols; a.L = L; a.tmax = tmax; a.n = (long)n_nodes; a.tw = tw;
    a.stride = stride; a.u = u_out; a.pos_x = pos_x_out; a.pos_t = pos_t_out; a.vars = vars_out; a.feat = feat_out;
    a.status = msmp_tune_get("split") ? status_ptr() : nullptr;
    for (int c = 0; c < n_cols; ++c) {
        MSMP_REQUIRE(cols[c] && col_div[c] != 0.0, MSMP_ERR_ARG, "msmp_prepare_nodes: bad column %d", c);
        a.col[c] = cols[c]; a.col_f64[c] = col_f64[c]; a.col_div[c] = col_div[c];
    }
    const long total = (long)n_nodes * (stride / 4);
    hipLaunchKernelGGL(prepare_nodes_kernel, dim3((unsigned)((total + 255) / 256)), dim3(256), 0, (hipStream_t)stream, a);
    return check_launch("prepare_nodes_kernel");
}

extern "C" int msmp_build_tiles(const int32_t* rowptr, const int32_t* col, int64_t n_nodes, int64_t n_edges, int group_nodes,
                                int32_t* tile_node_out, int32_t* tile_count_out, int32_t* tile_halo_out, int32_t* edge_slot_out,
                                int32_t* stats_out, msmp_stream_t stream) {
    MSMP_REQUIRE(rowptr && col && tile_node_out && tile_count_out && tile_halo_out && edge_slot_out && stats_out, MSMP_ERR_ARG,
                 "msmp_build_tiles: null pointer");
    MSMP_REQUIRE(n_nodes > 0 && n_edges >= 0 && n_nodes < (1L << 31) && n_edges < (1L << 31), MSMP_ERR_ARG, "msmp_build_tiles: bad sizes");
    MSMP_REQUIRE(group_nodes >= 1 && 4 * group_nodes <= MSMP_TILE_NCAP, MSMP_ERR_ARG, "msmp_build_tiles: group_nodes must be in 1..%d",
                 MSMP_TILE_NCAP / 4);
    hipStream_t st = (hipStream_t)stream;
    const hipError_t me = hipMemsetAsync(stats_out, 0, 3 * sizeof(int32_t), st);
    MSMP_REQUIRE(me == hipSuccess, MSMP_ERR_HIP, "msmp_build_tiles: memset: %s", hipGetErrorString(me));
    const int tile_nodes = 4 * group_nodes;
    const unsigned n_tiles = (unsigned)((n_nodes + tile_nodes - 1) / tile_nodes);
    hipLaunchKernelGGL(build_tiles_kernel, dim3(n_tiles), dim3(128), 0, st, rowptr, col, (int)n_nodes, tile_nodes, group_nodes, tile_node_out,
                       tile_count_out, tile_halo_out, edge_slot_out, stats_out);
    return check_launch("build_tiles_kernel");
}

bool msmp_tiles_ok(const msmp_tiles_t* t, int64_t n_nodes) {
    if (!(t->tile_node && t->tile_count && t->tile_halo && t->edge_slot && t->group_nodes >= 1 && t->tile_nodes == 4 * t->group_nodes &&
          t->tile_nodes <= MSMP_TILE_NCAP && t->n_tiles >= 1))
        return false;
    if (t->period_tiles > 0) {
        return t->period_nodes >= 1 && n_nodes % t->period_nodes == 0 && (int64_t)t->period_tiles * t->tile_nodes >= t->period_nodes &&
               (int64_t)(t->period_tiles - 1) * t->tile_nodes < t->period_nodes && (int64_t)t->n_tiles == n_nodes / t->period_nodes * t->period_tiles &&
               (int64_t)t->n_tiles * t->period_tiles < (1LL << 32);
    }
    return (int64_t)t->n_tiles * t->tile_nodes >= n_nodes && (int64_t)(t->n_tiles - 1) * t->tile_nodes < n_nodes;
}

static TileArgs tile_args(const float* h, const float* u, const float* pos, const float* vars, const float* feat, const float* p, const float* q,
                          const int32_t* rowptr, const msmp_tiles_t* t, int64_t n_nodes, int64_t n_edges, int tw, int nv, const PackedLayout& L,
                          const float* packed, float* agg) {
    TileArgs a{};
    a.h = h; a.u = u; a.pos = pos; a.vars = vars; a.feat = feat; a.P = p; a.Q = q; a.rowptr = rowptr;
    a.tile_node = t->tile_node; a.tile_halo = t->tile_halo; a.edge_slot = t->edge_slot;
    a.n_nodes = (long)n_nodes; a.n_edges = (long)n_edges; a.tile_nodes = t->tile_nodes; a.group_nodes = t->group_nodes;
    a.period_tiles = t->period_tiles > 0 ? t->period_tiles : 0;
    a.period_nodes = t->period_tiles > 0 ? t->period_nodes : 0;
    a.period_magic = t->period_tiles > 1 ? (unsigned)(((1ULL << 32) + t->period_tiles - 1) / t->period_tiles) : 0u;
    a.tw = tw; a.nv = nv; a.nc1 = L.nc1; a.w1s = packed + L.w1s; a.w2s = packed + L.w2s; a.scales = packed + L.scales; a.b1 = packed + L.b1;
    a.b2 = packed + L.b2; a.agg = agg; a.status = status_ptr();
    return a;
}

template <int MODE>
static void launch_tiles(const TileArgs& a, bool listed, unsigned n_tiles, hipStream_t st) {
    if (listed) hipLaunchKernelGGL((edge_tile_kernel<MODE, true>), dim3(n_tiles), dim3(256), 0, st, a);
    else hipLaunchKernelGGL((edge_tile_kernel<MODE, false>), dim3(n_tiles), dim3(256), 0, st, a);
}

extern "C" int msmp_edge_aggregate_tiled_f32(const float* h, const float* u, const float* pos, const float* vars, const float* feat,
                                             const float* p, const float* q, const int32_t* rowptr, const msmp_tiles_t* tiles, int64_t n_nodes,
                                             int64_t n_edges, int tw, int nv, const float* packed, float* agg_out,
                                             msmp_stream_t stream) {
    MSMP_REQUIRE(rowptr && tiles && packed && agg_out, MSMP_ERR_ARG, "msmp_edge_aggregate_tiled_f32: null pointer");
    MSMP_REQUIRE((p != nullptr) == (q != nullptr), MSMP_ERR_ARG, "msmp_edge_aggregate_tiled_f32: give both of p, q or neither");
    const bool fold = p == nullptr;
    MSMP_REQUIRE(!fold || (h && u && pos && vars), MSMP_ERR_ARG, "msmp_edge_aggregate_tiled_f32: null pointer (h, u, pos, vars)");
    MSMP_REQUIRE(msmp_tiles_ok(tiles, n_nodes), MSMP_ERR_ARG, "msmp_edge_aggregate_tiled_f32: the tile descriptor does not cover %ld nodes", (long)n_nodes);
    MSMP_REQUIRE(n_nodes > 0 && n_edges >= 0 && n_nodes < (1L << 31) && n_edges < (1L << 31) && tw > 0 && nv >= 1 && nv <= MSMP_MAX_VARS,
                 MSMP_ERR_ARG, "msmp_edge_aggregate_tiled_f32: bad sizes");
    MSMP_REQUIRE(msmp_tune_get("split"), MSMP_ERR_UNSUPPORTED, "msmp_edge_aggregate_tiled_f32: only on the fp16-split matrix path");
    const PackedLayout L = packed_layout(tw, nv);
    MSMP_REQUIRE(!fold || L.nc1 - 8 <= 2, MSMP_ERR_UNSUPPORTED, "msmp_edge_aggregate_tiled_f32: tw + 1 + nv <= 64");
    const TileArgs a = tile_args(h, u, pos, vars, feat, p, q, rowptr, tiles, n_nodes, n_edges, tw, nv, L, packed, agg_out);
    hipStream_t st = (hipStream_t)stream;
    timing_begin(MSMP_K_EDGE_MLP, st);
    const bool listed = tiles->listed != 0 || !msmp_tune_get("tile_arith");
    if (fold && feat) launch_tiles<2>(a, listed, (unsigned)tiles->n_tiles, st);
    else if (fold) launch_tiles<1>(a, listed, (unsigned)tiles->n_tiles, st);
    else launch_tiles<0>(a, listed, (unsigned)tiles->n_tiles, st);
    timing_end(MSMP_K_EDGE_MLP, st);
    return check_launch("edge_tile_kernel");
}

int msmp_edge_aggregate_tiled_pair(const float* h, const float* u, const float* pos, const float* vars, const float* feat, const int32_t* rowptr,
                                   const msmp_tiles_t* tiles, int64_t n_nodes, int64_t n_edges, int tw, int nv, const float* packed_a,
                                   const float* packed_b, float* agg_a, float* agg_b, msmp_stream_t stream) {
    MSMP_REQUIRE(h && u && pos && vars && rowptr && tiles && packed_a && packed_b && agg_a && agg_b, MSMP_ERR_ARG,
                 "msmp_edge_aggregate_tiled_pair: null pointer");
    MSMP_REQUIRE(msmp_tiles_ok(tiles, n_nodes), MSMP_ERR_ARG, "msmp_edge_aggregate_tiled_pair: the tile descriptor does not cover %ld nodes", (long)n_nodes);
    const PackedLayout L = packed_layout(tw, nv);
    MSMP_REQUIRE(L.nc1 - 8 <= 2 && msmp_tune_get("split"), MSMP_ERR_UNSUPPORTED, "msmp_edge_aggregate_tiled_pair: unsupported configuration");
    TileArgs2 a2;
    a2.head[0] = tile_args(h, u, pos, vars, feat, nullptr, nullptr, rowptr, tiles, n_nodes, n_edges, tw, nv, L, packed_a, agg_a);
    a2.head[1] = tile_args(h, u, pos, vars, feat, nullptr, nullptr, rowptr, tiles, n_nodes, n_edges, tw, nv, L, packed_b, agg_b);
    hipStream_t st = (hipStream_t)stream;
    timing_begin(MSMP_K_EDGE_MLP, st);
    const dim3 grid((unsigned)tiles->n_tiles, 2);
    const bool listed = tiles->listed != 0 || !msmp_tune_get("tile_arith");
    if (feat && listed) hipLaunchKernelGGL((edge_tile_pair_kernel<2, true>), grid, dim3(256), 0, st, a2);
    else if (feat) hipLaunchKernelGGL((edge_tile_pair_kernel<2, false>), grid, dim3(256), 0, st, a2);
    else if (listed) hipLaunchKernelGGL((edge_tile_pair_kernel<1, true>), grid, dim3(256), 0, st, a2);
    else hipLaunchKernelGGL((edge_tile_pair_kernel<1, false>), grid, dim3(256), 0, st, a2);
    timing_end(MSMP_K_EDGE_MLP, st);
    return check_launch("edge_tile_pair_kernel");
}
```

### msmp-pde_amd/graph.py

```python
import math

import torch

from . import _lib
from ._lib import lib, check, ptr, current_stream


import os as _os
_NO_SLICE = _os.environ.get('MSMP_NO_WINDOW_SLICE') == '1'


class Data(object):

    def __init__(self, x=None, edge_index=None, **kwargs):
        self.x = x
        self.edge_index = edge_index
        for k, v in kwargs.items():
            setattr(self, k, v)

    def keys(self):
        return [k for k in self.__dict__ if not k.startswith('_')]

    def to(self, device):
        for k in list(self.__dict__):
            v = self.__dict__[k]
            if torch.is_tensor(v):
                self.__dict__[k] = v.to(device)
            elif isinstance(v, GraphStructure):
                self.__dict__[k] = None if torch.device(device) != v.rowptr.device else v
        return self


class GraphStructure(object):

    def __init__(self, edge_index, batch, n_nodes):
        dev = edge_index.device
        if dev.type != 'cuda':
            raise _lib.MsmpError('GraphStructure needs device tensors (HIP path only, no CPU fallback)')
        L = lib()
        self.n_nodes = int(n_nodes)
        self.n_edges = int(edge_index.shape[1])
        ei = edge_index.contiguous()
        if ei.dtype != torch.int64:
            ei = ei.long()
        counts = torch.bincount(batch, minlength=int(batch[-1].item()) + 1 if batch.numel() else 1)
        self.n_graphs = int(counts.numel())
        self.graph_ptr = torch.zeros(self.n_graphs + 1, dtype=torch.int32, device=dev)
        self.graph_ptr[1:] = torch.cumsum(counts, 0).to(torch.int32)
        self.max_graph_nodes = int(counts.max().item()) if counts.numel() else 0
        self._tgt_long = self._col_long = self._by_source = None
        self.rowptr = torch.empty(self.n_nodes + 1, dtype=torch.int32, device=dev)
        self.col = torch.empty(max(self.n_edges, 1), dtype=torch.int32, device=dev)
        self.tgt = torch.empty(max(self.n_edges, 1), dtype=torch.int32, device=dev)
        ws_bytes = L.msmp_build_csr_workspace_bytes(self.n_edges, self.n_nodes)
        ws = torch.empty(ws_bytes, dtype=torch.uint8, device=dev)
        check(L.msmp_build_csr(ptr(ei), self.n_edges, self.n_nodes, ptr(self.rowptr), ptr(self.col), ptr(self.tgt),
                               ptr(ws), ws_bytes, current_stream()), 'msmp_build_csr')
        self.max_in_degree = int((self.rowptr[1:] - self.rowptr[:-1]).max().item()) if self.n_edges else 0
        self._key = (edge_index.data_ptr(), tuple(edge_index.shape), edge_index._version,
                     batch.data_ptr(), batch._version)
        self._tiles = False
        self._period = False

    def period(self):
        if self._period is not False:
            return self._period
        self._period = None
        b = self.n_graphs
        if b >= 2 and self.n_edges and self.n_nodes % b == 0 and self.n_edges % b == 0 and self.max_graph_nodes * b == self.n_nodes:
            nx, eg = self.n_nodes // b, self.n_edges // b
            dev = self.rowptr.device
            k = torch.arange(b, dtype=torch.int32, device=dev)[:, None]
            same = ((self.col[:self.n_edges].view(b, eg) - k * nx == self.col[:eg]).all()
                    & (self.rowptr[:-1].view(b, nx) - k * eg == self.rowptr[:nx]).all())
            if bool(same):
                self._period = (nx, eg)
        return self._period

    def tiles(self):
        if self._tiles is not False:
            return self._tiles
        self._tiles = None
        if self.n_edges == 0 or self.max_in_degree <= 0 or self.max_in_degree > _lib.MSMP_TILE_GROUP_EDGES:
            return None
        L = lib()
        dev = self.rowptr.device
        gn0 = min(_lib.MSMP_TILE_NCAP // 4, _lib.MSMP_TILE_GROUP_EDGES // self.max_in_degree)
        gn = gn0
        per = self.period()
        align = bool(L.msmp_tune_query(b'tile_align'))
        for _attempt in range(4):
            if gn < max(1, gn0 // 2):
                return None
            tn = 4 * gn
            periodic = per is not None and (per[0] % tn == 0 or align)
            n_src, e_src = (per if periodic else (self.n_nodes, self.n_edges))
            n_meta = (n_src + tn - 1) // tn
            n_tiles = n_meta * (self.n_graphs if periodic else 1)
            if periodic and n_tiles * n_meta >= 1 << 32:
                periodic, n_src, e_src = False, self.n_nodes, self.n_edges
                n_meta = n_tiles = (n_src + tn - 1) // tn
            tile_node = torch.empty(n_meta * _lib.MSMP_TILE_NCAP, dtype=torch.int32, device=dev)
            tile_count = torch.empty(n_meta, dtype=torch.int32, device=dev)
            tile_halo = torch.empty(n_meta * 4, dtype=torch.int32, device=dev)
            edge_slot = torch.empty(n_meta * _lib.MSMP_TILE_EDGES, dtype=torch.int32, device=dev)
            stats = torch.empty(3, dtype=torch.int32, device=dev)
            check(L.msmp_build_tiles(ptr(self.rowptr), ptr(self.col), n_src, e_src, gn, ptr(tile_node), ptr(tile_count),
                                     ptr(tile_halo), ptr(edge_slot), ptr(stats), current_stream()), 'msmp_build_tiles')
            max_nodes, max_edges, n_listed = (int(v) for v in stats.tolist())
            if max_nodes <= _lib.MSMP_TILE_NCAP and max_edges <= _lib.MSMP_TILE_GROUP_EDGES:
                desc = _lib.MsmpTiles(tn, gn, n_tiles, ptr(tile_node), ptr(tile_count), ptr(tile_halo), ptr(edge_slot), int(n_listed > 0),
                                      n_meta if periodic else 0, n_src if periodic else 0)
                self._tiles = (desc, tile_node, tile_count, edge_slot, tile_halo)
                return self._tiles
            gn -= max(1, -(-(max_nodes - _lib.MSMP_TILE_NCAP) // 4)) if max_nodes > _lib.MSMP_TILE_NCAP else 1
        return None

    @property
    def tgt_long(self):
        if self._tgt_long is None:
            self._tgt_long, self._col_long = self.tgt[:self.n_edges].long(), self.col[:self.n_edges].long()
        return self._tgt_long

    @property
    def col_long(self):
        self.tgt_long
        return self._col_long

    def by_source(self):
        if self._by_source is None:
            src = self.col_long
            perm = torch.sort(src, stable=True)[1]
            rowptr = torch.zeros(self.n_nodes + 1, dtype=torch.int32, device=src.device)
            rowptr[1:] = torch.cumsum(torch.bincount(src, minlength=self.n_nodes), 0).to(torch.int32)
            self._by_source = (perm, rowptr)
        return self._by_source

    def by_source32(self):
        if getattr(self, '_by_source32', None) is None:
            perm, rowptr = self.by_source()
            self._by_source32 = (perm.to(torch.int32).contiguous(), rowptr)
        return self._by_source32

    def matches(self, edge_index, batch):
        return self._key == (edge_index.data_ptr(), tuple(edge_index.shape), edge_index._version,
                             batch.data_ptr(), batch._version)


def structure_of(data):
    gs = getattr(data, '_msmp_structure', None)
    if gs is None or not gs.matches(data.edge_index, data.batch):
        gs = GraphStructure(data.edge_index, data.batch, data.x.shape[0])
        data._msmp_structure = gs
    return gs


def _graph_ptr_from_sizes(sizes, device):
    gp = torch.zeros(len(sizes) + 1, dtype=torch.int32)
    gp[1:] = torch.cumsum(torch.as_tensor(sizes, dtype=torch.int64), 0).to(torch.int32)
    return gp.to(device)


def radius_graph(x, r, batch=None, loop=False, max_num_neighbors=32, sizes=None):
    assert not loop
    x2 = x.reshape(x.shape[0], -1).to(torch.float64).contiguous()
    dev = x2.device
    n = x2.shape[0]
    if sizes is None:
        sizes = torch.bincount(batch).tolist() if batch is not None else [n]
    gp = _graph_ptr_from_sizes(sizes, dev)
    L = lib()
    st = current_stream()
    rowptr = torch.empty(n + 1, dtype=torch.int32, device=dev)
    check(L.msmp_radius_graph_count_f64(ptr(x2), x2.shape[1], ptr(gp), len(sizes), n, float(r), int(max_num_neighbors),
                                        ptr(rowptr), st), 'msmp_radius_graph_count_f64')
    e = int(rowptr[-1].item())
    ei = torch.empty((2, e), dtype=torch.int64, device=dev)
    check(L.msmp_radius_graph_fill_f64(ptr(x2), x2.shape[1], ptr(gp), len(sizes), n, float(r), int(max_num_neighbors),
                                       ptr(rowptr), e, ptr(ei), st), 'msmp_radius_graph_fill_f64')
    return ei


def knn_graph(x, k, batch=None, loop=False, sizes=None):
    assert not loop
    x2 = x.reshape(x.shape[0], -1).to(torch.float64).contiguous()
    dev = x2.device
    n = x2.shape[0]
    if sizes is None:
        sizes = torch.bincount(batch).tolist() if batch is not None else [n]
    gp = _graph_ptr_from_sizes(sizes, dev)
    e = sum(s * min(k, s - 1) for s in sizes)
    L = lib()
    rowptr = torch.empty(n + 1, dtype=torch.int32, device=dev)
    ei = torch.empty((2, e), dtype=torch.int64, device=dev)
    check(L.msmp_knn_graph_f64(ptr(x2), x2.shape[1], ptr(gp), len(sizes), n, int(k), e, ptr(rowptr), ptr(ei),
                               current_stream()), 'msmp_knn_graph_f64')
    return ei


def torch_time_axis(pde):
    return torch.linspace(pde.tmin, pde.tmax, pde.grid_size[0], dtype=torch.float64)


class GraphCreator(object):

    def __init__(self, pde, neighbors=2, time_window=5, t_resolution=250, x_resolution=100, device=None):
        assert isinstance(neighbors, int) and isinstance(time_window, int)
        self.pde = pde
        self.n = neighbors
        self.tw = time_window
        self.t_res = t_resolution
        self.x_res = x_resolution
        self.device = device
        self._edge_cache = {}
        self._small = {}

    def _cached(self, key, make):
        v = self._small.get(key)
        if v is None:
            if len(self._small) > 256:
                self._small.clear()
            v = self._small[key] = make()
        return v

    def _steps_on(self, steps, device):
        if torch.is_tensor(steps):
            return steps.to(device=device, dtype=torch.long)
        steps = tuple(int(s) for s in steps)
        return self._cached(('steps', steps, str(device)), lambda: torch.tensor(steps, dtype=torch.long, device=device))

    def _time_axis_on(self, device):
        p = self.pde
        return self._cached(('t', float(p.tmin), float(p.tmax), int(p.grid_size[0]), str(device)),
                            lambda: torch_time_axis(p).to(device))

    def to(self, device):
        self.device = device
        return self

    def create_data(self, datapoints, steps):
        dev, tw = datapoints.device, self.tw
        if not torch.is_tensor(steps) and len(steps) > 0 and all(int(s) == int(steps[0]) for s in steps) and not _NO_SLICE:
            s0 = int(steps[0])
            if tw <= s0 <= datapoints.shape[1] - tw:
                return datapoints[:, s0 - tw:s0], datapoints[:, s0:s0 + tw]
        steps_t = self._steps_on(steps, dev)
        b = self._cached(('b', datapoints.shape[0], str(dev)), lambda: torch.arange(datapoints.shape[0], device=dev)[:, None])
        win = self._cached(('win', tw, str(dev)), lambda: torch.arange(-tw, tw, device=dev)[None, :])
        block = datapoints[b, steps_t[:, None] + win]
        return block[:, :tw], block[:, tw:]

    def _flatten(self, block):
        if f'{self.pde}' == 'AD':
            b, tw, c, nx = block.shape
            return block.permute(0, 3, 2, 1).reshape(b * nx, c * tw)
        b, tw, nx = block.shape
        return block.permute(0, 2, 1).reshape(b * nx, tw)

    def build_edge_index(self, x0, bsz, device):
        name = f'{self.pde}'
        nx = x0.shape[0]
        x0c = x0.detach().to('cpu', torch.float64).contiguous()
        key = (name, self.n, bsz, nx, str(device), bool(getattr(self.pde, 'untructured_grid', False)),
               hash(x0c.numpy().tobytes()))
        if key in self._edge_cache:
            return self._edge_cache[key]
        sizes = [nx] * bsz
        if name in ('CE', 'KF', 'KS', 'AD'):
            if name == 'AD' and getattr(self.pde, 'untructured_grid', False):
# ... 63 lines not shown
```

### msmp-pde_amd/layers.py

```python
import ctypes
import threading

import torch
from torch import nn

from . import _lib
from ._lib import lib, check, ptr, current_stream, HIDDEN
from .graph import GraphStructure


class Swish(nn.Module):

    def __init__(self, beta=1):
        super().__init__()
        self.beta = beta

    def forward(self, x):
        return x * torch.sigmoid(self.beta * x)


def _linear(i, o):
    return nn.Linear(i, o, dtype=torch.float32)


class _Workspace(object):
    _bufs = {}
    _tls = threading.local()

    class _Private(object):
        def __init__(self, device):
            self.device, self.buf = device, None

        def __enter__(self):
            self._outer = getattr(_Workspace._tls, 'private', None)
            _Workspace._tls.private = self
            return self

        def __exit__(self, *exc):
            _Workspace._tls.private = self._outer

        def buffers(self):
            return [self.buf]

    @classmethod
    def private(cls, device):
        return cls._Private(device)

    @classmethod
    def get(cls, nbytes, device):
        p = getattr(cls._tls, 'private', None)
        if p is not None and p.device == device:
            if p.buf is None or p.buf.numel() < nbytes:
                assert not torch.cuda.is_current_stream_capturing() or p.buf is None, 'workspace grew during capture'
                p.buf = torch.empty(nbytes, dtype=torch.uint8, device=device)
            return p.buf
        key = (device, torch.cuda.current_stream(device).cuda_stream)
        buf = cls._bufs.get(key)
        if buf is None or buf.numel() < nbytes:
            buf = torch.empty(nbytes, dtype=torch.uint8, device=device)
            cls._bufs[key] = buf
        return buf


class _MPLayerBase(nn.Module):
    MODE = None

    def __init__(self, in_features, out_features, hidden_features, time_window, n_variables):
        super().__init__()
        if not (in_features == out_features == hidden_features):
            raise ValueError('in_features, hidden_features and out_features must be equal (they are in every class of the reference)')
        self.wide = hidden_features != HIDDEN
        if not 1 <= n_variables <= _lib.MSMP_MAX_VARS:
            raise ValueError(f'n_variables must be in 1..{_lib.MSMP_MAX_VARS}')
        self.in_features, self.out_features, self.hidden_features = in_features, out_features, hidden_features
        self.time_window, self.n_variables = time_window, n_variables
        self.message_net_1 = nn.Sequential(_linear(2 * in_features + time_window + 1 + n_variables, hidden_features), Swish())
        self.message_net_2 = nn.Sequential(_linear(hidden_features, hidden_features), Swish())
        self.update_net_1 = nn.Sequential(_linear(in_features + hidden_features + n_variables, hidden_features), Swish())
        self._make_update_net_2(hidden_features, out_features)
        self._packed = None
        self._packed_key = None
        self._ps = None

    def _params8(self):
        ps = self._ps
        if ps is None or ps[0] is not self.message_net_1[0].weight:
            ps = self._ps = (self.message_net_1[0].weight, self.message_net_1[0].bias, self.message_net_2[0].weight,
                             self.message_net_2[0].bias, self.update_net_1[0].weight, self.update_net_1[0].bias,
                             self.update_net_2[0].weight, self.update_net_2[0].bias)
        return ps

    def packed(self):
        if self.wide:
            raise _lib.MsmpError(f'the packed layer blob exists for hidden width {HIDDEN} only')
        ps = self._params8()
        key = (_lib.PARAM_EPOCH[0], ps[0].data_ptr(), ps[7].data_ptr(), ps[0].dtype) + tuple(p._version for p in ps)
        if key != self._packed_key:
            dev = ps[0].device
            if dev.type != 'cuda' or any(p.device != dev for p in ps):
                raise _lib.MsmpError('layer parameters must be on the GPU (HIP path only, no CPU fallback)')
            L = lib()
            n = L.msmp_packed_layer_floats(self.time_window, self.n_variables)
            blob = torch.empty(n, dtype=torch.float32, device=dev)
            f = [p.detach().to(torch.float32).contiguous() for p in ps]
            check(L.msmp_pack_layer_f32(*[ptr(t) for t in f], self.time_window, self.n_variables, ptr(blob),
                                        current_stream()), 'msmp_pack_layer_f32')
            self._packed, self._packed_key = blob, key
        return self._packed

    def wide_weights(self):
        ps = self._params8()
        key = (_lib.PARAM_EPOCH[0],) + tuple((p.data_ptr(), p._version) for p in ps)
        if key != self._packed_key:
            w1 = ps[0].detach().to(torch.float32)
            W, tw = self.hidden_features, self.time_window
            wp = torch.cat((w1[:, :W], w1[:, 2 * W:]), 1).contiguous()
            wq = torch.cat((w1[:, W:2 * W], -w1[:, 2 * W:2 * W + tw + 1], torch.zeros_like(w1[:, 2 * W + tw + 1:])), 1).contiguous()
            self._packed = (wp, wq) + tuple(p.detach().to(torch.float32).contiguous() for p in ps[1:])
            self._packed_key = key
        return self._packed

    def forward(self, x, u, pos, variables, edge_index, batch, structure=None):
        if structure is None:
            structure = GraphStructure(edge_index, batch, x.shape[0])
        return mp_layer(x, u, pos, variables, structure, self, None)


class GNN_Layer(_MPLayerBase):
    MODE = _lib.MSMP_LAYER_RESIDUAL_SWISH

    def _make_update_net_2(self, h, o):
        self.update_net_2 = nn.Sequential(_linear(h, o), Swish())


class GNN_LayerLin(_MPLayerBase):
    MODE = _lib.MSMP_LAYER_LIN

    def _make_update_net_2(self, h, o):
        self.update_net_2 = nn.Sequential(_linear(h, o))


def _f32c(t):
    return t.detach().to(torch.float32).contiguous()


DENSE_MESSAGE = False


def node_features(u, pos_x, variables):
    L = lib()
    n, tw, nv = u.shape[0], u.shape[1], variables.shape[1]
    stride = L.msmp_node_feature_stride(tw, nv)
    feat = torch.empty(n, stride, dtype=torch.float32, device=u.device)
    check(L.msmp_pack_node_features_f32(ptr(u), ptr(pos_x), ptr(variables), n, tw, nv, ptr(feat), current_stream()),
          'msmp_pack_node_features_f32')
    return feat


def _mp_layer_hip(h, u, pos_x, variables, gs, main, gate, eps, dense_message=None, feat=None, decode=None):
    L = lib()
    n = h.shape[0]
    out = torch.empty_like(h)
    gated = gate is not None
    dense = DENSE_MESSAGE if dense_message is None else dense_message
    mode = main.MODE | (_lib.MSMP_LAYER_DENSE_MESSAGE if dense else 0)
    ws_bytes = L.msmp_mp_layer_workspace_bytes(n, gs.n_edges, int(gated), gs.max_in_degree)
    ws = _Workspace.get(ws_bytes, h.device)
    tiles = gs.tiles()
    if decode is not None:
        c1, c2, u_last, dt, tw = decode
        w = [p.detach().to(torch.float32).contiguous() for p in (c1.weight, c1.bias, c2.weight, c2.bias)]
        pred = torch.empty(n, tw, dtype=torch.float32, device=h.device)
        dec = _lib.MsmpDecoder(ptr(w[0]), ptr(w[1]), ptr(w[2]), ptr(w[3]), ptr(u_last), float(dt), int(tw), ptr(pred))
        rc = L.msmp_mp_layer_decode_f32(ptr(h), ptr(u), ptr(pos_x), ptr(variables), ptr(feat), ptr(gs.rowptr), ptr(gs.col), ptr(gs.tgt),
                                        None if tiles is None else ctypes.byref(tiles[0]), ptr(gs.graph_ptr), n, gs.n_edges, gs.n_graphs, gs.max_in_degree,
                                        gs.max_graph_nodes, main.time_window, main.n_variables, ptr(main.packed()), ptr(gate.packed()) if gated else None,
                                        mode, eps, ptr(out), ctypes.byref(dec), ptr(ws), ws.numel(), current_stream())
        if rc == _lib.MSMP_ERR_UNSUPPORTED:
            return None
        check(rc, 'msmp_mp_layer_decode_f32')
        out._msmp_keep = w
        return out, pred
    check(L.msmp_mp_layer_f32(ptr(h), ptr(u), ptr(pos_x), ptr(variables), ptr(feat), ptr(gs.rowptr), ptr(gs.col), ptr(gs.tgt),
                              None if tiles is None else ctypes.byref(tiles[0]), ptr(gs.graph_ptr), n, gs.n_edges, gs.n_graphs, gs.max_in_degree, gs.max_graph_nodes, main.time_window,
                              main.n_variables,
                              ptr(main.packed()), ptr(gate.packed()) if gated else None, mode, eps, ptr(out),
                              ptr(ws), ws.numel(), current_stream()), 'msmp_mp_layer_f32')
    return out


def _wide_linear(x, k, w, bias, n_out, mode, out, ws):
    L = lib()
    check(L.msmp_linear_f32(ptr(x), x.shape[1], x.shape[0], k, ptr(w), w.shape[1], ptr(bias), n_out, mode, ptr(out), out.shape[1],
                            ptr(ws), ws.numel(), current_stream()), 'msmp_linear_f32')


def _wide_head(h, feat_cat, k_feat, variables, gs, layer, ld, ws):
    L = lib()
    n, W, e = h.shape[0], layer.hidden_features, gs.n_edges
    wp, wq, b1, w2, b2, w3, b3, w4, b4 = layer.wide_weights()
    dev = h.device
    P = torch.empty(n, ld, dtype=torch.float32, device=dev)
    Q = torch.empty(n, ld, dtype=torch.float32, device=dev)
    _wide_linear(feat_cat, k_feat, wp, b1, W, 0, P, ws)
    _wide_linear(feat_cat, k_feat, wq, None, W, 0, Q, ws)
    a1 = torch.empty(max(e, 1), ld, dtype=torch.float32, device=dev)
    check(L.msmp_wide_gather_swish_f32(ptr(P), ptr(Q), ptr(gs.tgt), ptr(gs.col), e, W, ld, ptr(a1), current_stream()), 'msmp_wide_gather_swish_f32')
    msg = torch.empty(max(e, 1), ld, dtype=torch.float32, device=dev)
    if e:
        _wide_linear(a1[:e], W, w2, b2, W, 1, msg[:e], ws)
    agg = torch.empty(n, ld, dtype=torch.float32, device=dev)
    check(L.msmp_wide_scatter_mean_f32(ptr(msg), ptr(gs.rowptr), n, W, ld, ptr(agg), current_stream()), 'msmp_wide_scatter_mean_f32')
    upd_in = torch.cat((h[:, :W], agg[:, :W], variables), 1)
    pad = (-upd_in.shape[1]) % 4
    if pad:
        upd_in = torch.nn.functional.pad(upd_in, (0, pad))
    upd_in = upd_in.contiguous()
    z = torch.empty(n, ld, dtype=torch.float32, device=dev)
    _wide_linear(upd_in, 2 * W + variables.shape[1], w3, b3, W, 1, z, ws)
    y = torch.empty(n, ld, dtype=torch.float32, device=dev)
    _wide_linear(z, W, w4, b4, W, 0, y, ws)
    return y


def _mp_layer_wide(h, u, pos_x, variables, gs, main, gate, eps):
    L = lib()
    W = main.hidden_features
    if main.MODE != _lib.MSMP_LAYER_LIN:
        raise _lib.MsmpError('the width-generic layer path implements GNN_LayerLin (the layer of the GLU classes)')
    ld = 128 * ((W + 127) // 128)
    n = h.shape[0]
    hp = torch.zeros(n, ld, dtype=torch.float32, device=h.device)
    hp[:, :W] = h
    feat_cat = torch.cat((h, u, pos_x.reshape(-1, 1), variables), 1)
    k_feat = feat_cat.shape[1]
    pad = (-feat_cat.shape[1]) % 4
    if pad:
        feat_cat = torch.nn.functional.pad(feat_cat, (0, pad))
    feat_cat = feat_cat.contiguous()
    k_max = max(feat_cat.shape[1], 2 * W + variables.shape[1] + 3)
    ws = _Workspace.get(L.msmp_linear_workspace_bytes(k_max, W), h.device)
    y_main = _wide_head(hp, feat_cat, k_feat, variables, gs, main, ld, ws)
    y_gate = _wide_head(hp, feat_cat, k_feat, variables, gs, gate, ld, ws) if gate is not None else None
    out = torch.empty(n, ld, dtype=torch.float32, device=h.device)
    check(L.msmp_wide_norm_blend_f32(ptr(hp), ptr(y_gate), ptr(y_main), ptr(gs.graph_ptr), gs.n_graphs, W, ld, eps, ptr(out), current_stream()),
          'msmp_wide_norm_blend_f32')
    return out[:, :W].contiguous()


def _mp_layer_wide_autograd(h, u, pos_x, variables, gs, main, gate, eps):
    import torch.nn.functional as F
    i, j = gs.tgt_long, gs.col_long
    n = h.shape[0]
    deg = (gs.rowptr[1:] - gs.rowptr[:-1]).clamp(min=1).to(h.dtype)[:, None]
    batch = torch.repeat_interleave(torch.arange(gs.n_graphs, device=h.device), (gs.graph_ptr[1:] - gs.graph_ptr[:-1]).long())
    cnt = (gs.graph_ptr[1:] - gs.graph_ptr[:-1]).clamp(min=1).to(h.dtype)[:, None]
    pos = pos_x.reshape(-1, 1)

    def head(layer):
        sw = lambda x: x * torch.sigmoid(x)
        cat = torch.cat((h[i], h[j], u[i] - u[j], pos[i] - pos[j], variables[i]), -1)
        m = sw(layer.message_net_2[0](sw(layer.message_net_1[0](cat))))
        agg = torch.zeros(n, m.shape[1], dtype=m.dtype, device=m.device).index_add_(0, i, m) / deg
        y = layer.update_net_2[0](sw(layer.update_net_1[0](torch.cat((h, agg, variables), -1))))
        mean = torch.zeros(gs.n_graphs, y.shape[1], dtype=y.dtype, device=y.device).index_add_(0, batch, y) / cnt
        yc = y - mean[batch]
        var = torch.zeros_like(mean).index_add_(0, batch, yc * yc) / cnt
        return yc / torch.sqrt(var + eps)[batch]

    out = head(main)
    if gate is None:
        return out
    tau = torch.sigmoid(head(gate))
    return (1.0 - tau) * h + tau * (out * torch.sigmoid(out))


def mp_layer(h, u, pos_x, variables, structure, main, gate=None, eps=1e-5, dense_message=None, feat=None, decode=None):
    gs = structure
    if gs is None or h.device.type != 'cuda':
        raise _lib.MsmpError('mp_layer needs CUDA tensors and a GraphStructure (HIP path only, no CPU fallback)')
    need_grad = torch.is_grad_enabled() and (h.requires_grad or any(p.requires_grad for p in main._params8()))
    if main.wide:
        if need_grad:
            return _mp_layer_wide_autograd(h, u.to(h.dtype), pos_x, variables.to(h.dtype), gs, main, gate, eps)
        return _mp_layer_wide(_f32c(h), _f32c(u), _f32c(pos_x).reshape(-1), _f32c(variables), gs, main, gate, eps)
    hd, u, pos_x, variables = _f32c(h), _f32c(u), _f32c(pos_x).reshape(-1), _f32c(variables)
    n = hd.shape[0]
    assert n == gs.n_nodes and hd.shape[1] == HIDDEN and u.shape[1] == main.time_window
    assert variables.shape[1] == main.n_variables and pos_x.numel() == n
    if not need_grad:
        return _mp_layer_hip(hd, u, pos_x, variables, gs, main, gate, eps, dense_message, feat, decode)
    assert decode is None, 'the fused decoder epilogue is an inference path'

    from .autograd import MPLayerFunction
    params = list(main._params8()) + (list(gate._params8()) if gate is not None else [])
    hin = h if (h.dtype == torch.float32 and h.is_contiguous()) else h.to(torch.float32).contiguous()
    return MPLayerFunction.apply(hin, u, pos_x, variables, gs, main, gate, eps, _mp_layer_hip, *params)
```

### msmp-pde_amd/solvers.py

```python
import functools

import torch
from torch import nn

from . import _lib
from ._lib import lib, check, ptr, current_stream, PARAM_EPOCH
from .graph import structure_of
from .layers import GNN_Layer, GNN_LayerLin, Swish, mp_layer, node_features
from .lem import LEM, LEMS
from .reductions import bias_add

_DECODER = {20: (15, 4, 10), 25: (16, 3, 14), 50: (12, 2, 10)}


class _Linear(nn.Linear):

    def forward(self, x):
        if self.bias is None or not (x.is_cuda and x.dtype == torch.float32 and torch.is_grad_enabled() and self.bias.requires_grad):
            return super().forward(x)
        y = torch.nn.functional.linear(x, self.weight)
        return bias_add(y.reshape(-1, y.shape[-1]), self.bias).view(y.shape)


def _lin(i, o):
# ... 190 lines not shown
        if self.hidden_features != 128:
            return self.lemoutput_mlp(self.embedding_lem.forward_nodes(self._step_inputs(u, pos_x, pos_t, variables, dt)))
        grad = torch.is_grad_enabled() and any(p.requires_grad for p in self.embedding_lem.parameters())
        if not grad:
            h = self.embedding_lem.encode_nodes(u, pos_x, pos_t, variables, dt, self.TWO_D, self.lemoutput_mlp)
            if h is not None:
                return h
        lem_in = self._step_inputs(u, pos_x, pos_t, variables, dt)
        if grad:
            h = self.embedding_lem.forward_nodes(lem_in)
            return self.lemoutput_mlp(h)
        return self.embedding_lem.encode(lem_in, self.lemoutput_mlp)

    def _step_inputs(self, u, pos_x, pos_t, variables, dt):
        tw, n = self.time_window, u.shape[0]
        if self.TWO_D:
            ts = dt.view(1, tw) + pos_t
            x = torch.stack([pos_x.expand(n, tw), u[:, :tw], u[:, tw:], ts], -1)
            return torch.cat((x, variables[:, None, 1:].expand(n, tw, variables.shape[1] - 1)), -1)
        t_len = u.shape[1]
        return torch.cat((pos_x[:, None, :].expand(n, t_len, 1), u[:, :, None],
                          variables[:, None, :].expand(n, t_len, variables.shape[1])), -1)

    def _g2_pair(self, h, u, pos_x, variables, gs, i):
        t = self.swish(mp_layer(h, u, pos_x, variables, gs, self.gnn_layers_gate[i], None))
        tau = torch.tanh(_OutEdgeMean.apply((t[gs.col_long] - t[gs.tgt_long]) ** 2, gs))
        return (1.0 - tau) * h + tau * self.swish(mp_layer(h, u, pos_x, variables, gs, self.gnn_layers[i], None))

    def _embed_packed(self, dev):
        lin1, lin2 = self.embedding_mlp[0], self.embedding_mlp[2]
        ps = (lin1.weight, lin1.bias, lin2.weight, lin2.bias)
        key = (PARAM_EPOCH[0],) + tuple((p.data_ptr(), p._version, str(p.device)) for p in ps)
        if getattr(self, '_embed_key', None) != key:
            L = lib()
            f = [p.detach().to(torch.float32).contiguous() for p in ps]
            blob = torch.empty(L.msmp_packed_mlp2_floats(lin1.in_features), dtype=torch.float32, device=dev)
            check(L.msmp_pack_mlp2_f32(*[ptr(t) for t in f], lin1.in_features, ptr(blob), current_stream()), 'msmp_pack_mlp2_f32')
            self._embed_blob, self._embed_key = blob, key
        return self._embed_blob

    def _embed_hip(self, u, pos_x, variables):
        L = lib()
        k_in = self.embedding_mlp[0].in_features
        blob = self._embed_packed(u.device)
        stride = L.msmp_mlp2_input_stride(k_in)
        pad = u.new_zeros(u.shape[0], stride - k_in)
        x = torch.cat((u, pos_x, variables, pad), -1).contiguous()
        assert x.shape[1] == stride
        out = torch.empty(u.shape[0], self.hidden_features, dtype=torch.float32, device=u.device)
        check(L.msmp_mlp2_swish_f32(ptr(x), u.shape[0], k_in, ptr(blob), ptr(out), current_stream()), 'msmp_mlp2_swish_f32')
        return out

    def _dt(self, dev):
        dkey = (self.time_window, float(self.pde.dt), str(dev))
        if getattr(self, '_dt_key', None) != dkey:
            with torch.inference_mode(False):
                self._dt_cum, self._dt_key = torch.cumsum(torch.ones(self.time_window, dtype=torch.float32, device=dev) * self.pde.dt, 0), dkey
        return self._dt_cum

    def warm_caches(self, dev=None):
        dev = dev or next(self.parameters()).device
        for layers in (self.gnn_layers, getattr(self, 'gnn_layers_gate', ())):
            for layer in layers:
                layer.wide_weights() if layer.wide else layer.packed()
        if self.LEM_ENCODER and not self.LSTM_ENCODER and self.hidden_features == 128 and not isinstance(self.embedding_lem, LEMS):
            self.embedding_lem._pack(self.lemoutput_mlp)
        elif not self.LEM_ENCODER and not self.LSTM_ENCODER:
            self._embed_packed(dev)
        self._dt(dev)

    INPUT_RANGE = 255.0

    def input_range(self, data):
        prep = self._prepare(data, False)
        if prep is None:
            raise RuntimeError('input_range: device tensors of dtype float32 / float64 expected')
        u, pos_x, _, variables, _ = prep
        return float(max(u.abs().max(), pos_x.abs().max(), variables.abs().max()))

    def validate_inputs(self, data):
        r = self.input_range(data)
        if not r <= self.INPUT_RANGE:
            raise ValueError(f'node features reach |x| = {r:.4g} > {self.INPUT_RANGE:g}: the fp16-split matrix path would saturate them; '
                             "rescale the data or select the exact-fp32 kernels with lib().msmp_tune(b'split', 0)")
        return r

    sub_batches = 1

    range_policy = 'auto'
    _range_exact = False
    _range_probed = False

    def _range_switch(self, flags, when):
        self._range_exact = True
        _lib._range_report(flags, f'{type(self).__name__}: {when}; this model now runs on the exact-fp32 MFMA kernels (no range limit, about 2x slower). '
                                  'Rescale the data to keep the fast path; model._range_exact = False switches back.')
        _lib.last_status(reset=True)

    def _dispatch(self, data):
        if self.sub_batches > 1 and not torch.is_grad_enabled() and data.x.is_cuda and not torch.cuda.is_current_stream_capturing() \
                and not isinstance(getattr(self, 'embedding_lem', None), LEMS):
            return self._forward_sub_batches(data, int(self.sub_batches))
        return self._forward(data)

    def forward(self, data):
        policy = self.range_policy
        if policy == 'warn' or not data.x.is_cuda or not lib().msmp_tune_query(b'split'):
            _lib.status_check()
            return self._dispatch(data)
        if not self._range_exact:
            flags = _lib.last_status()
            if flags:
                self._range_switch(flags, 'raised by kernel work that completed before this call (an EARLIER result is saturated or not finite)')
        if self._range_exact:
            with _lib.exact_fp32():
                return self._dispatch(data)
        probe = (policy == 'sync' or not self._range_probed) and not torch.is_grad_enabled() and not torch.cuda.is_current_stream_capturing()
        stateful = isinstance(getattr(self, 'embedding_lem', None), LEMS)
        states = self.embedding_lem.states if (probe and stateful) else None
        out = self._dispatch(data)
        if probe:
            self._range_probed = True
            torch.cuda.current_stream().synchronize()
            flags = _lib.last_status()
            if flags:
                self._range_switch(flags, 'raised by this forward, which has been evaluated again')
                if stateful:
                    self.embedding_lem.states = states
                with _lib.exact_fp32():
                    out = self._dispatch(data)
        return out

    def load_state_dict(self, *args, **kwargs):
        self._range_probed = False
        return super().load_state_dict(*args, **kwargs)

    def _sub_batch_plan(self, data, parts):
        from .dist import shard_graph
        gs = structure_of(data)
        plans = gs.__dict__.setdefault('_sub_batch_plans', {})
        plan = plans.get(parts)
        if plan is None:
            n_parts = max(1, min(parts, gs.n_graphs))
            subs = []
            for r in range(n_parts):
                sub = shard_graph(data, r, n_parts)
                subs.append(sub)
            offs, o = [], 0
            for sub in subs:
                offs.append((o, o + sub.x.shape[0]))
                o += sub.x.shape[0]
            assert o == data.x.shape[0]
            for sub in subs:
                structure_of(sub).tiles()
            plan = plans[parts] = {'subs': subs, 'offs': offs, 'streams': [torch.cuda.Stream(device=data.x.device) for _ in subs]}
        return plan

    def _forward_sub_batches(self, data, parts):
        plan = self._sub_batch_plan(data, parts)
        share = lib().msmp_tune_query(b'lem_share')
        lib().msmp_tune(b'lem_share', max(1, len(plan['subs'])))
        n = data.x.shape[0]
        cur = torch.cuda.current_stream()
        self.warm_caches(data.x.device)
        out = None
        per_node = [k for k, v in data.__dict__.items() if torch.is_tensor(v) and not k.startswith('_') and k not in ('edge_index', 'batch')
                    and v.dim() >= 1 and v.shape[0] == n]
        outs = []
        try:
            for sub, (n0, n1), st in zip(plan['subs'], plan['offs'], plan['streams']):
                for k in per_node:
                    setattr(sub, k, getattr(data, k)[n0:n1])
                st.wait_stream(cur)
                with torch.cuda.stream(st):
                    outs.append(self._forward(sub))
        finally:
            lib().msmp_tune(b'lem_share', share)
        for o, st in zip(outs, plan['streams']):
            cur.wait_stream(st)
            o.record_stream(cur)
        out = torch.cat(outs, 0)
        return out

    def _forward(self, data):
        u_in = data.x
        pos = data.pos
        gs = structure_of(data)
        tw = self.time_window
        want_feat = not torch.is_grad_enabled() and self.hidden_features == 128 and gs.tiles() is not None
        prep = self._prepare(data, want_feat) if u_in.is_cuda else None
        if prep is not None:
            u, pos_x, pos_t, variables, feat = prep
        else:
            pos_x = (pos[:, 1][:, None] / self.pde.L)
            pos_t = (pos[:, 0][:, None] / self.pde.tmax)
            variables = self._variables(data, pos_t).float()
            pos_x, pos_t = pos_x.float(), pos_t.float()
            u = u_in.float().contiguous()
            feat = node_features(u, pos_x.reshape(-1).contiguous(), variables.contiguous()) if want_feat else None
        dt = self._dt(u.device)

        h = self._encode(u, pos_x, pos_t, variables, dt)
        fuse = (not self.TWO_D and not self.G2 and tw == 25 and self.hidden_features == 128 and not torch.is_grad_enabled()
                and u.is_cuda and bool(lib().msmp_tune_query(b'dec_fuse')))
        for i in range(self.hidden_layer):
            if self.G2:
                h = self._g2_pair(h, u, pos_x, variables, gs, i)
                continue
            gate = self.gnn_layers_gate[i] if self.GATED else None
            if fuse and i == self.hidden_layer - 1:
                both = mp_layer(h, u, pos_x, variables, gs, self.gnn_layers[i], gate, feat=feat,
                                decode=(self.output_mlp[0], self.output_mlp[2], None if self.RETURN_DIFF else u, float(self.pde.dt), tw))
                if both is not None:
                    return both[1].to(u_in.dtype)
            h = mp_layer(h, u, pos_x, variables, gs, self.gnn_layers[i], gate, feat=feat)

        return self._decode(h, u, u_in, dt, tw)

    def _decode(self, h, u, u_in, dt, tw):
        grad_path = torch.is_grad_enabled() and (h.requires_grad or any(p.requires_grad for p in self.output_mlp.parameters()))
        if self.TWO_D and grad_path:
            diff = _decoder_autograd(self.double_mlp(h), self.output_mlp[0], self.output_mlp[2])
            out = (u.view(-1, 2, tw) + dt.view(1, 1, tw) * diff).flatten(1, 2)
        elif self.TWO_D:
            hd = self._double_mlp_hip(h)
            out = torch.empty_like(u)
            c1, c2 = self.output_mlp[0], self.output_mlp[2]
            w = [p.detach().to(torch.float32).contiguous() for p in (c1.weight, c1.bias, c2.weight, c2.bias)]
            check(lib().msmp_decoder2d_f32(ptr(hd), ptr(u), u.shape[0], tw, ptr(w[0]), ptr(w[1]), ptr(w[2]), ptr(w[3]),
                                           float(self.pde.dt), ptr(out), current_stream()), 'msmp_decoder2d_f32')
        elif grad_path:
            diff = _decoder_autograd(h[:, None], self.output_mlp[0], self.output_mlp[2]).squeeze(1)
            out = diff if self.RETURN_DIFF else u[:, -1:] + dt.view(1, tw) * diff
        else:
            out = torch.empty_like(u)
            c1, c2 = self.output_mlp[0], self.output_mlp[2]
            w = [p.detach().to(torch.float32).contiguous() for p in (c1.weight, c1.bias, c2.weight, c2.bias)]
            h = h.contiguous()
            check(lib().msmp_decoder_f32(ptr(h), None if self.RETURN_DIFF else ptr(u), u.shape[0], tw, ptr(w[0]), ptr(w[1]), ptr(w[2]),
                                         ptr(w[3]), float(self.pde.dt), ptr(out), current_stream()), 'msmp_decoder_f32')
        return out.to(u_in.dtype)


    def _double_mlp_hip(self, h):
        lin = self.double_mlp[0]
        w, b = lin.weight.detach().to(torch.float32).contiguous(), lin.bias.detach().to(torch.float32).contiguous()
        h = h.contiguous()
        n_out, k = w.shape
        need = lib().msmp_linear_swish_workspace_bytes(k, n_out)
        if not need:
            raise RuntimeError(f'double_mlp of {k} -> {n_out} features is outside msmp_linear_swish_f32')
        from .layers import _Workspace
        ws = _Workspace.get(need, h.device)
        out = torch.empty(h.shape[0], n_out, dtype=torch.float32, device=h.device)
        check(lib().msmp_linear_swish_f32(ptr(h), h.shape[0], k, ptr(w), ptr(b), n_out, ptr(out), ptr(ws), ws.numel(), current_stream()),
              'msmp_linear_swish_f32')
        self._dmlp_keep = (w, b)
        return out.view(h.shape[0], 2, n_out // 2)

    def capture(self, data):
        return _GraphedForward(self, data)


class _GraphedForward:

    def __init__(self, model, data):
        import copy
        assert not torch.is_grad_enabled(), 'capture() is for inference: wrap it in torch.no_grad()'
        self.model = model
        self.data = copy.copy(data)
        self.data.x = data.x.clone()
        self.data.pos = data.pos.clone()
        self._capture()

    def _weight_state(self):
        pde = self.model.pde
        return (PARAM_EPOCH[0], tuple((p.data_ptr(), p._version) for p in self.model.parameters()),
                (float(pde.dt), float(pde.L), float(pde.tmax)))

    def _weight_blobs(self):
        return [getattr(m, attr) for m in self.model.modules() for attr in ('_packed', '_embed_blob') if getattr(m, attr, None) is not None]

    @torch.no_grad()
    def _capture(self):
        from .layers import _Workspace
        model = self.model
        self.graph = None
        with _Workspace.private(self.data.x.device) as ws:
            side = torch.cuda.Stream()
            side.wait_stream(torch.cuda.current_stream())
            with torch.cuda.stream(side):
                for _ in range(2):
                    model._forward(self.data)
            torch.cuda.current_stream().wait_stream(side)
            torch.cuda.synchronize()
            graph = torch.cuda.CUDAGraph()
            with torch.cuda.graph(graph):
                self.out = model(self.data)
            self.graph = graph
        self._ws = ws.buffers()
        self._blobs = self._weight_blobs()
        self._state = self._weight_state()

    def __call__(self, data):
        if self._state != self._weight_state():
            self._capture()
        self.data.x.copy_(data.x)
        self.data.pos.copy_(data.pos)
        self.graph.replay()
        return self.out.clone()


class MP_PDE_Solver(_SolverBase):
    pass


class MP_PDE_SolverGated(_SolverBase):
    GATED, LAYER = True, GNN_LayerLin


class MP_PDE_SolverLEMLinGated(_SolverBase):
    GATED, LEM_ENCODER, LAYER = True, True, GNN_LayerLin


class MP_PDE_SolverLEMLin(_SolverBase):
    LEM_ENCODER = True


class MP_PDE_Solver2D(_SolverBase):
    TWO_D = True


class MP_PDE_Solver2DGated(_SolverBase):
    TWO_D, GATED, LAYER = True, True, GNN_LayerLin


class MP_PDE_Solver2DLEMLinGated(_SolverBase):
    TWO_D, GATED, LEM_ENCODER, LAYER = True, True, True, GNN_LayerLin


class MP_PDE_Solver2DLEMLin(_SolverBase):
    TWO_D, LEM_ENCODER = True, True
# ... 97 lines not shown
```

Measured before the change: 163.4 rollout-steps/s.

## Add five-group edge tiles so each 256-thread block processes more nodes

```diff
diff --git a/include/msmp_pde.h b/include/msmp_pde.h
--- a/include/msmp_pde.h
+++ b/include/msmp_pde.h
@@ -27,7 +27,7 @@
 
 typedef void* msmp_stream_t;
 
-#define MSMP_ABI_VERSION 400
+#define MSMP_ABI_VERSION 500
 int msmp_version(void);
 const char* msmp_last_error(void);
 
@@ -94,6 +94,9 @@
 int msmp_build_tiles(const int32_t* rowptr, const int32_t* col, int64_t n_nodes, int64_t n_edges, int group_nodes,
                      int32_t* tile_node_out, int32_t* tile_count_out, int32_t* tile_halo_out, int32_t* edge_slot_out,
                      int32_t* stats_out, msmp_stream_t stream);
+int msmp_build_tiles_groups(const int32_t* rowptr, const int32_t* col, int64_t n_nodes, int64_t n_edges, int group_nodes, int groups,
+                            int32_t* tile_node_out, int32_t* tile_count_out, int32_t* tile_halo_out, int32_t* edge_slot_out,
+                            int32_t* stats_out, msmp_stream_t stream);
 int msmp_node_feature_stride(int tw, int nv);
 int msmp_prepare_nodes(const void* x, int x_f64, const void* pos, int pos_f64, int64_t n_nodes, int tw, double L, double tmax,
                        int n_cols, const void* const* cols, const int* col_f64, const double* col_div, float* u_out,
diff --git a/msmp-pde_amd/_lib.py b/msmp-pde_amd/_lib.py
--- a/msmp-pde_amd/_lib.py
+++ b/msmp-pde_amd/_lib.py
@@ -23,7 +23,7 @@
 MSMP_ERR_UNSUPPORTED = -2
 MSMP_MAX_VARS = 8
 HIDDEN = 128
-MSMP_ABI_VERSION = 400
+MSMP_ABI_VERSION = 500
 MSMP_STATUS_INPUT_RANGE, MSMP_STATUS_NODE_SATURATED, MSMP_STATUS_NONFINITE = 1, 2, 4
 
 SIGNATURES = {
@@ -49,6 +49,7 @@
     'msmp_node_project_f32': (c_int, [c_void_p] * 4 + [c_int64, c_int, c_int, c_void_p, c_void_p, c_void_p, c_void_p]),
     'msmp_edge_aggregate_projected_f32': (c_int, [c_void_p] * 5 + [c_int64, c_int64, c_int, c_int, c_int, c_void_p, c_void_p, c_void_p]),
     'msmp_build_tiles': (c_int, [c_void_p, c_void_p, c_int64, c_int64, c_int, c_void_p, c_void_p, c_void_p, c_void_p, c_void_p, c_void_p]),
+    'msmp_build_tiles_groups': (c_int, [c_void_p, c_void_p, c_int64, c_int64, c_int, c_int, c_void_p, c_void_p, c_void_p, c_void_p, c_void_p, c_void_p]),
     'msmp_node_feature_stride': (c_int, [c_int, c_int]),
     'msmp_prepare_nodes': (c_int, [c_void_p, c_int, c_void_p, c_int, c_int64, c_int, c_double, c_double, c_int, c_void_p, c_void_p, c_void_p,
                                    c_void_p, c_void_p, c_void_p, c_void_p, c_void_p, c_void_p]),
diff --git a/msmp-pde_amd/csrc/aux_kernels.hip b/msmp-pde_amd/csrc/aux_kernels.hip
--- a/msmp-pde_amd/csrc/aux_kernels.hip
+++ b/msmp-pde_amd/csrc/aux_kernels.hip
@@ -543,7 +543,7 @@
     float* qbuf = (float*)(ws + 4 * nod);
     int rc;
     int tile_mode = (tiles && n_edges > 0 && msmp_tune_get("split")) ? msmp_tune_get("tile") : 0;
-    if (tile_mode == 2 && n_edges < (int64_t)76 * tiles->n_tiles) tile_mode = 0;
+    if (tile_mode == 2 && 4 * n_edges < (int64_t)76 * (tiles->tile_nodes / tiles->group_nodes) * tiles->n_tiles) tile_mode = 0;
     if (tile_mode == 3) tile_mode = 2;
     auto aggregate = [&](const float* packed, float* agg) -> int {
         if (fused && !dense && tile_mode == 2)
diff --git a/msmp-pde_amd/csrc/mlp_kernels.hip b/msmp-pde_amd/csrc/mlp_kernels.hip
--- a/msmp-pde_amd/csrc/mlp_kernels.hip
+++ b/msmp-pde_amd/csrc/mlp_kernels.hip
@@ -1250,6 +1250,7 @@
 static int g_decoder = 1;
 static int g_tile_arith = 1;
 static int g_tile_align = 0;
+static int g_tile_groups = 4;
 static int g_tile = 2;
 static int g_bwd_gemm = 1;
 static int g_dec_fuse = 0;
@@ -1262,6 +1263,7 @@
     if (!strcmp(key, "tile")) return g_tile;
     if (!strcmp(key, "tile_arith")) return g_tile_arith;
     if (!strcmp(key, "tile_align")) return g_tile_align;
+    if (!strcmp(key, "tile_groups")) return g_tile_groups;
     if (!strcmp(key, "decoder")) return g_decoder;
     if (!strcmp(key, "dec_fuse")) return g_dec_fuse;
     if (!strcmp(key, "lem_tail")) return g_lem_tail;
@@ -1278,6 +1280,7 @@
     if (key && !strcmp(key, "tile")) { g_tile = value; return MSMP_OK; }
     if (key && !strcmp(key, "tile_arith")) { g_tile_arith = value; return MSMP_OK; }
     if (key && !strcmp(key, "tile_align")) { g_tile_align = value; return MSMP_OK; }
+    if (key && !strcmp(key, "tile_groups") && (value == 0 || value == 4 || value == 5)) { g_tile_groups = value; return MSMP_OK; }
     if (key && !strcmp(key, "decoder")) { g_decoder = value != 0; return MSMP_OK; }
     if (key && !strcmp(key, "dec_fuse")) { g_dec_fuse = value != 0; return MSMP_OK; }
     if (key && !strcmp(key, "lem_tail")) { g_lem_tail = value != 0; return MSMP_OK; }
diff --git a/msmp-pde_amd/csrc/tile_kernels.hip b/msmp-pde_amd/csrc/tile_kernels.hip
--- a/msmp-pde_amd/csrc/tile_kernels.hip
+++ b/msmp-pde_amd/csrc/tile_kernels.hip
@@ -16,7 +16,6 @@
 #endif
 
 constexpr int TILE_NCAP = MSMP_TILE_NCAP;
-constexpr int TILE_EDGES = MSMP_TILE_EDGES;
 constexpr int PQLD = H + 4;
 constexpr int BROW_T = 72;
 constexpr int FRAG_SKEW = 32;
@@ -26,16 +25,17 @@
 constexpr float NODE_MAX = 65504.0f;
 __device__ __forceinline__ float node_scaled(float x) { return __builtin_amdgcn_fmed3f(x * NODE_SCALE, -NODE_MAX, NODE_MAX); }
 
-__global__ __launch_bounds__(128) void build_tiles_kernel(const int* __restrict__ rowptr, const int* __restrict__ col, int n_nodes,
+constexpr int TILE_EDGES_MAX = 5 * 32;
+__global__ __launch_bounds__(TILE_EDGES_MAX) void build_tiles_kernel(const int* __restrict__ rowptr, const int* __restrict__ col, int n_nodes,
                                                           int tile_nodes, int group_nodes, int* __restrict__ tile_node,
                                                           int* __restrict__ tile_count, int* __restrict__ tile_halo,
                                                           int* __restrict__ edge_slot, int* __restrict__ stats) {
-    __shared__ int s_col[TILE_EDGES];
-    __shared__ int s_first[TILE_EDGES];
-    __shared__ int s_slot[TILE_EDGES];
+    __shared__ int s_col[TILE_EDGES_MAX];
+    __shared__ int s_first[TILE_EDGES_MAX];
+    __shared__ int s_slot[TILE_EDGES_MAX];
     __shared__ int s_halo[5];
     __shared__ int s_stat[6];
-    const int t = blockIdx.x, k = threadIdx.x;
+    const int t = blockIdx.x, k = threadIdx.x, n_lanes = blockDim.x;
     const int n0 = t * tile_nodes, n1 = min(n0 + tile_nodes, n_nodes);
     const int nt = n1 - n0;
     const int g = k >> 5, kk = k & 31;
@@ -86,10 +86,10 @@
     if (valid) {
         int ts = gf - n0;
         while (ts + 1 < gl - n0 && rowptr[n0 + ts + 1] <= e) ++ts;
-        edge_slot[(size_t)t * TILE_EDGES + k] = ts | (min(slot, 255) << 8);
+        edge_slot[(size_t)t * n_lanes + k] = ts | (min(slot, 255) << 8);
         if (first && slot < TILE_NCAP) tile_node[(size_t)t * TILE_NCAP + slot] = j;
     } else
-        edge_slot[(size_t)t * TILE_EDGES + k] = 0;
+        edge_slot[(size_t)t * n_lanes + k] = 0;
     if (k < TILE_NCAP && k < nt) tile_node[(size_t)t * TILE_NCAP + k] = n0 + k;
     __syncthreads();
     const int total = nt + s_stat[2] + s_stat[5];
@@ -230,8 +230,9 @@
 
 using half4v = __attribute__((ext_vector_type(4))) _Float16;
 
-template <int MODE, bool LISTED>
+template <int MODE, bool LISTED, int G>
 __device__ __forceinline__ void edge_tile_body(const TileArgs& a, float* lds) {
+    static_assert(G == 4 || G == 5, "four or five wave groups per tile");
     constexpr bool FOLD = MODE != 0;
     float* wbuf = lds;
     float* pl = lds + WBUF_FLOATS;
@@ -263,12 +264,12 @@
         return node;
     };
 
-    const int sl = a.edge_slot[(size_t)tm * TILE_EDGES + wave * 32 + c];
+    const int sl = a.edge_slot[(size_t)tm * (32 * G) + wave * 32 + c];
     const int gf = min(tile_n0 + wave * a.group_nodes, tile_n1), gl = min(gf + a.group_nodes, tile_n1);
     const int* rp = a.rowptr - node_off;
     const int rp_base = rp[__builtin_amdgcn_readfirstlane(gf)];
     const int rp_row = gf + min(c, max(gl - gf - 1, 0));
-    int rp_lo = rp[rp_row], rp_hi = rp[rp_row + 1];
+    int rp_lo = rp[rp_row], rp_hi = rp[min(rp_row + 1, tile_n1)];
     int er0 = 0, edeg = 0;
     auto edge_ranges = [&]() {
         __builtin_amdgcn_sched_barrier(0);
@@ -546,24 +547,46 @@
     const float kinv = uniform_ro(a.scales, 1);
     const float inv2 = uniform_ro(a.scales, 5) * (1.0f / ACT_SCALE);
     const float cexp = -1.44269504088896340736f * inv2;
-    auto swish2 = [&](int T, int r0, int r1) {
+    auto swish_acc = [&](f32x16& acc, int r0, int r1) {
 #pragma unroll
         for (int r = r0; r < r1; r += 2) {
 #if MSMP_PRECISE_ACT
-            y[T][r] = ACT_SCALE * swishf(y[T][r] * inv2);
-            y[T][r + 1] = ACT_SCALE * swishf(y[T][r + 1] * inv2);
+            acc[r] = ACT_SCALE * swishf(acc[r] * inv2);
+            acc[r + 1] = ACT_SCALE * swishf(acc[r + 1] * inv2);
             (void)kinv; (void)cexp;
 #else
-            const f32x2 yy = {y[T][r], y[T][r + 1]};
+            const f32x2 yy = {acc[r], acc[r + 1]};
             const f32x2 t = yy * f32x2{cexp, cexp};
             const f32x2 e = f32x2{__builtin_amdgcn_exp2f(t[0]), __builtin_amdgcn_exp2f(t[1])};
             const f32x2 d = e * f32x2{kinv, kinv} + f32x2{kinv, kinv};
             const f32x2 z = yy * f32x2{__builtin_amdgcn_rcpf(d[0]), __builtin_amdgcn_rcpf(d[1])};
-            y[T][r] = z[0];
-            y[T][r + 1] = z[1];
+            acc[r] = z[0];
+            acc[r + 1] = z[1];
 #endif
         }
     };
+    auto swish2 = [&](int T, int r0, int r1) { swish_acc(y[T], r0, r1); };
+    auto selection = [&](int e0, int deg, half8 (&sel)[2]) {
+        const unsigned mask = deg >= 32 ? 0xffffffffu : ((1u << deg) - 1u) << (e0 & 31);
+        const char* lut = reinterpret_cast<const char*>(lds + TILE_MAIN_FLOATS);
+        using u32x2 = __attribute__((ext_vector_type(2))) unsigned;
+#pragma unroll
+        for (int s = 0; s < 2; ++s) {
+            const u32x2 lo = *reinterpret_cast<const u32x2*>(lut + 8 * ((mask >> (16 * s + 4 * hh)) & 15u));
+            const u32x2 hi = *reinterpret_cast<const u32x2*>(lut + 8 * ((mask >> (16 * s + 8 + 4 * hh)) & 15u));
+            const u32x4 wv = {lo[0], lo[1], hi[0], hi[1]};
+            sel[s] = __builtin_bit_cast(half8, wv);
+        }
+    };
+    const int gf4 = min(tile_n0 + 4 * a.group_nodes, tile_n1), gl4 = min(gf4 + a.group_nodes, tile_n1);
+    int sl4 = 0, rp_base4 = 0, rp_lo4 = 0, rp_hi4 = 0;
+    if constexpr (G == 5) {
+        rp_base4 = rp[__builtin_amdgcn_readfirstlane(gf4)];
+        const int rp_row4 = gf4 + min(c, max(gl4 - gf4 - 1, 0));
+        rp_lo4 = rp[rp_row4];
+        rp_hi4 = rp[min(rp_row4 + 1, tile_n1)];
+        sl4 = a.edge_slot[(size_t)tm * (32 * G) + 4 * 32 + c];
+    }
     half8 sf[2];
     {
         constexpr int par = 1;
@@ -605,10 +628,51 @@
         }
         TPROF(4);
     }
+    const half8* fifth = reinterpret_cast<const half8*>(wbuf);
+    int er0_4 = 0, edeg4 = 0;
+    float b2v4 = 0.f;
+    half8 w4[8][2];
+    unsigned w4off = 0;
+    auto w4load = [&](int u) {
+        const half8* g = reinterpret_cast<const half8*>(reinterpret_cast<const char*>(a.w2s + (size_t)u * WHALF_FLOATS) + w4off);
+        w4[u][0] = g[0];
+        w4[u][1] = g[64];
+    };
+    if constexpr (G == 5) {
+        const float* prow4 = pl + (sl4 & 255) * PQLD + 4 * hh;
+        const float* qrow4 = ql + ((sl4 >> 8) & 255) * PQLD + 4 * hh;
+        __syncthreads();
+        {
+            unsigned tb = (unsigned)tid;
+            asm volatile("" : "+v"(tb));
+            b2v4 = a.b2[32 * (tb >> 6) + (tb & 31)];
+        }
+#pragma unroll
+        for (int v = 0; v < 2; ++v) {
+            const int u = 2 * wave + v, t = u >> 1, s = u & 1;
+#pragma unroll
+            for (int j = 0; j < 2; ++j) {
+                pq[j] = *reinterpret_cast<const f32x4*>(prow4 + 32 * t + 16 * s + 8 * j);
+                pq[2 + j] = *reinterpret_cast<const f32x4*>(qrow4 + 32 * t + 16 * s + 8 * j);
+            }
+#pragma unroll
+            for (int i = 0; i < 4; ++i) act_slice(i);
+            half8 fh, fl;
+            split8(zt, fh, fl);
+            half8* dst = reinterpret_cast<half8*>(wbuf) + 2 * u * 64 + lane;
+            dst[0] = fh;
+            dst[64] = fl;
+        }
+        er0_4 = rp_lo4 - rp_base4;
+        edeg4 = c < gl4 - gf4 ? rp_hi4 - rp_lo4 : 0;
+        __syncthreads();
+        TPROF(6);
+    }
     f32x4 fr[4];
     {
         float* ftab = pl + wave * 32;
         if (hh == 0) ftab[c] = (1.0f / ACT_SCALE) / (float)max(edeg, 1);
+        if (G == 5 && hh == 0) ftab[128 + c] = (1.0f / ACT_SCALE) / (float)max(edeg4, 1);
 #pragma unroll
         for (int q = 0; q < 4; ++q) fr[q] = *reinterpret_cast<const f32x4*>(ftab + 8 * q + 4 * hh);
     }
@@ -646,6 +710,16 @@
             y[T] = __builtin_amdgcn_mfma_f32_32x32x16_f16(sf[1], h1, y[T], 0, 0, 0);
             TILE_SCHED_BARRIER();
         }
+    }
+    int ch = 0;
+    if constexpr (G == 5) {
+        unsigned t4 = (unsigned)tid;
+        asm volatile("" : "+v"(t4));
+        w4off = ((t4 >> 6) * 128 + (t4 & 63)) * 16;
+        ch = (int)(32 * (t4 >> 6) + (t4 & 31));
+#pragma unroll
+        for (int u = 0; u < 4; ++u) w4load(u);
+        TILE_SCHED_BARRIER();
     }
     TPROF(7);
     {
@@ -672,22 +746,82 @@
         if (bad) status_raise(a.status, MSMP_STATUS_NODE_SATURATED);
     }
     TPROF(9);
+    if constexpr (G == 5) {
+        TILE_SCHED_BARRIER();
+#pragma unroll
+        for (int u = 4; u < 8; ++u) w4load(u);
+        TILE_SCHED_BARRIER();
+        f32x16 y4;
+        {
+            float bv = b2v4 * (uniform_ro(a.scales, 1) * ACT_SCALE);
+#pragma unroll
+            for (int r = 0; r < 16; ++r) y4[r] = bv;
+        }
+#pragma unroll
+        for (int u = 0; u < 8; ++u) {
+            const half8 fh = fifth[2 * u * 64 + lane], fl = fifth[(2 * u + 1) * 64 + lane];
+            const half8 whi = w4[u][0], wlo = w4[u][1];
+            MSMP_MFMA_LOLO(2, y4, fl, wlo);
+            y4 = __builtin_amdgcn_mfma_f32_32x32x16_f16(fh, wlo, y4, 0, 0, 0);
+            y4 = __builtin_amdgcn_mfma_f32_32x32x16_f16(fl, whi, y4, 0, 0, 0);
+            y4 = __builtin_amdgcn_mfma_f32_32x32x16_f16(fh, whi, y4, 0, 0, 0);
+        }
+        half8 sf4[2];
+        selection(er0_4, edeg4, sf4);
+        swish_acc(y4, 0, 16);
+        half8 mh[2], ml[2];
+#pragma unroll
+        for (int s = 0; s < 2; ++s) {
+            float v[8];
+#pragma unroll
+            for (int j = 0; j < 8; ++j) v[j] = y4[8 * s + j];
+            split8(v, mh[s], ml[s]);
+        }
+        f32x16 z16;
+#pragma unroll
+        for (int r = 0; r < 16; ++r) z16[r] = 0.f;
+        y4 = __builtin_amdgcn_mfma_f32_32x32x16_f16(sf4[0], ml[0], z16, 0, 0, 0);
+        y4 = __builtin_amdgcn_mfma_f32_32x32x16_f16(sf4[0], mh[0], y4, 0, 0, 0);
+        y4 = __builtin_amdgcn_mfma_f32_32x32x16_f16(sf4[1], ml[1], y4, 0, 0, 0);
+        y4 = __builtin_amdgcn_mfma_f32_32x32x16_f16(sf4[1], mh[1], y4, 0, 0, 0);
+        const float* ftab4 = pl + 128 + wave * 32;
+        const int gf4 = min(tile_n0 + 4 * a.group_nodes, tile_n1), ng = min(gf4 + a.group_nodes, tile_n1) - gf4;
+        float* out = a.agg + (size_t)gf4 * H + ch;
+        bool bad = false;
+#pragma unroll
+        for (int q = 0; q < 4; ++q) {
+            if (8 * q < ng) {
+                const f32x4 f = *reinterpret_cast<const f32x4*>(ftab4 + 8 * q + 4 * hh);
+#pragma unroll
+                for (int m = 0; m < 4; ++m) {
+                    const int row = 8 * q + 4 * hh + m;
+                    if (row < ng) {
+                        const float v = y4[4 * q + m] * f[m];
+                        out[(size_t)row * H] = v;
+                        bad |= out_of_range(v);
+                    }
+                }
+            }
+        }
+        if (bad) status_raise(a.status, MSMP_STATUS_NODE_SATURATED);
+        TPROF(8);
+    }
     TPROF_FLUSH
 }
 
-template <int MODE, bool LISTED>
+template <int MODE, bool LISTED, int G>
 __global__ __launch_bounds__(256, 3) void edge_tile_kernel(TileArgs a) {
     __shared__ __attribute__((aligned(16))) float lds[TILE_LDS_FLOATS];
-    edge_tile_body<MODE, LISTED>(a, lds);
+    edge_tile_body<MODE, LISTED, G>(a, lds);
 }
 
 struct TileArgs2 {
     TileArgs head[2];
 };
-template <int MODE, bool LISTED>
+template <int MODE, bool LISTED, int G>
 __global__ __launch_bounds__(256, 3) void edge_tile_pair_kernel(TileArgs2 a) {
     __shared__ __attribute__((aligned(16))) float lds[TILE_LDS_FLOATS];
-    edge_tile_body<MODE, LISTED>(a.head[blockIdx.y], lds);
+    edge_tile_body<MODE, LISTED, G>(a.head[blockIdx.y], lds);
 }
 
 }
@@ -738,26 +872,35 @@
     return check_launch("prepare_nodes_kernel");
 }
 
+extern "C" int msmp_build_tiles_groups(const int32_t* rowptr, const int32_t* col, int64_t n_nodes, int64_t n_edges, int group_nodes, int groups,
+                                       int32_t* tile_node_out, int32_t* tile_count_out, int32_t* tile_halo_out, int32_t* edge_slot_out,
+                                       int32_t* stats_out, msmp_stream_t stream) {
+    MSMP_REQUIRE(rowptr && col && tile_node_out && tile_count_out && tile_halo_out && edge_slot_out && stats_out, MSMP_ERR_ARG,
+                 "msmp_build_tiles: null pointer");
+    MSMP_REQUIRE(n_nodes > 0 && n_edges >= 0 && n_nodes < (1L << 31) && n_edges < (1L << 31), MSMP_ERR_ARG, "msmp_build_tiles: bad sizes");
+    MSMP_REQUIRE(groups == 4 || groups == 5, MSMP_ERR_ARG, "msmp_build_tiles: groups must be 4 or 5");
+    MSMP_REQUIRE(group_nodes >= 1 && groups * group_nodes <= MSMP_TILE_NCAP, MSMP_ERR_ARG, "msmp_build_tiles: group_nodes must be in 1..%d",
+                 MSMP_TILE_NCAP / groups);
+    hipStream_t st = (hipStream_t)stream;
+    const hipError_t me = hipMemsetAsync(stats_out, 0, 3 * sizeof(int32_t), st);
+    MSMP_REQUIRE(me == hipSuccess, MSMP_ERR_HIP, "msmp_build_tiles: memset: %s", hipGetErrorString(me));
+    const int tile_nodes = groups * group_nodes;
+    const unsigned n_tiles = (unsigned)((n_nodes + tile_nodes - 1) / tile_nodes);
+    hipLaunchKernelGGL(build_tiles_kernel, dim3(n_tiles), dim3(32 * groups), 0, st, rowptr, col, (int)n_nodes, tile_nodes, group_nodes, tile_node_out,
+                       tile_count_out, tile_halo_out, edge_slot_out, stats_out);
+    return check_launch("build_tiles_kernel");
+}
+
 extern "C" int msmp_build_tiles(const int32_t* rowptr, const int32_t* col, int64_t n_nodes, int64_t n_edges, int group_nodes,
                                 int32_t* tile_node_out, int32_t* tile_count_out, int32_t* tile_halo_out, int32_t* edge_slot_out,
                                 int32_t* stats_out, msmp_stream_t stream) {
-    MSMP_REQUIRE(rowptr && col && tile_node_out && tile_count_out && tile_halo_out && edge_slot_out && stats_out, MSMP_ERR_ARG,
-                 "msmp_build_tiles: null pointer");
-    MSMP_REQUIRE(n_nodes > 0 && n_edges >= 0 && n_nodes < (1L << 31) && n_edges < (1L << 31), MSMP_ERR_ARG, "msmp_build_tiles: bad sizes");
-    MSMP_REQUIRE(group_nodes >= 1 && 4 * group_nodes <= MSMP_TILE_NCAP, MSMP_ERR_ARG, "msmp_build_tiles: group_nodes must be in 1..%d",
-                 MSMP_TILE_NCAP / 4);
-    hipStream_t st = (hipStream_t)stream;
-    const hipError_t me = hipMemsetAsync(stats_out, 0, 3 * sizeof(int32_t), st);
-    MSMP_REQUIRE(me == hipSuccess, MSMP_ERR_HIP, "msmp_build_tiles: memset: %s", hipGetErrorString(me));
-    const int tile_nodes = 4 * group_nodes;
-    const unsigned n_tiles = (unsigned)((n_nodes + tile_nodes - 1) / tile_nodes);
-    hipLaunchKernelGGL(build_tiles_kernel, dim3(n_tiles), dim3(128), 0, st, rowptr, col, (int)n_nodes, tile_nodes, group_nodes, tile_node_out,
-                       tile_count_out, tile_halo_out, edge_slot_out, stats_out);
-    return check_launch("build_tiles_kernel");
+    return msmp_build_tiles_groups(rowptr, col, n_nodes, n_edges, group_nodes, 4, tile_node_out, tile_count_out, tile_halo_out, edge_slot_out,
+                                   stats_out, stream);
 }
 
 bool msmp_tiles_ok(const msmp_tiles_t* t, int64_t n_nodes) {
-    if (!(t->tile_node && t->tile_count && t->tile_halo && t->edge_slot && t->group_nodes >= 1 && t->tile_nodes == 4 * t->group_nodes &&
+    if (!(t->tile_node && t->tile_count && t->tile_halo && t->edge_slot && t->group_nodes >= 1 &&
+          (t->tile_nodes == 4 * t->group_nodes || t->tile_nodes == 5 * t->group_nodes) &&
           t->tile_nodes <= MSMP_TILE_NCAP && t->n_tiles >= 1))
         return false;
     if (t->period_tiles > 0) {
@@ -784,9 +927,14 @@
 }
 
 template <int MODE>
-static void launch_tiles(const TileArgs& a, bool listed, unsigned n_tiles, hipStream_t st) {
-    if (listed) hipLaunchKernelGGL((edge_tile_kernel<MODE, true>), dim3(n_tiles), dim3(256), 0, st, a);
-    else hipLaunchKernelGGL((edge_tile_kernel<MODE, false>), dim3(n_tiles), dim3(256), 0, st, a);
+static void launch_tiles(const TileArgs& a, bool listed, int groups, unsigned n_tiles, hipStream_t st) {
+    if (groups == 5) {
+        if (listed) hipLaunchKernelGGL((edge_tile_kernel<MODE, true, 5>), dim3(n_tiles), dim3(256), 0, st, a);
+        else hipLaunchKernelGGL((edge_tile_kernel<MODE, false, 5>), dim3(n_tiles), dim3(256), 0, st, a);
+    } else {
+        if (listed) hipLaunchKernelGGL((edge_tile_kernel<MODE, true, 4>), dim3(n_tiles), dim3(256), 0, st, a);
+        else hipLaunchKernelGGL((edge_tile_kernel<MODE, false, 4>), dim3(n_tiles), dim3(256), 0, st, a);
+    }
 }
 
 extern "C" int msmp_edge_aggregate_tiled_f32(const float* h, const float* u, const float* pos, const float* vars, const float* feat,
@@ -807,9 +955,10 @@
     hipStream_t st = (hipStream_t)stream;
     timing_begin(MSMP_K_EDGE_MLP, st);
     const bool listed = tiles->listed != 0 || !msmp_tune_get("tile_arith");
-    if (fold && feat) launch_tiles<2>(a, listed, (unsigned)tiles->n_tiles, st);
-    else if (fold) launch_tiles<1>(a, listed, (unsigned)tiles->n_tiles, st);
-    else launch_tiles<0>(a, listed, (unsigned)tiles->n_tiles, st);
+    const int groups = tiles->tile_nodes / tiles->group_nodes;
+    if (fold && feat) launch_tiles<2>(a, listed, groups, (unsigned)tiles->n_tiles, st);
+    else if (fold) launch_tiles<1>(a, listed, groups, (unsigned)tiles->n_tiles, st);
+    else launch_tiles<0>(a, listed, groups, (unsigned)tiles->n_tiles, st);
     timing_end(MSMP_K_EDGE_MLP, st);
     return check_launch("edge_tile_kernel");
 }
@@ -829,10 +978,17 @@
     timing_begin(MSMP_K_EDGE_MLP, st);
     const dim3 grid((unsigned)tiles->n_tiles, 2);
     const bool listed = tiles->listed != 0 || !msmp_tune_get("tile_arith");
-    if (feat && listed) hipLaunchKernelGGL((edge_tile_pair_kernel<2, true>), grid, dim3(256), 0, st, a2);
-    else if (feat) hipLaunchKernelGGL((edge_tile_pair_kernel<2, false>), grid, dim3(256), 0, st, a2);
-    else if (listed) hipLaunchKernelGGL((edge_tile_pair_kernel<1, true>), grid, dim3(256), 0, st, a2);
-    else hipLaunchKernelGGL((edge_tile_pair_kernel<1, false>), grid, dim3(256), 0, st, a2);
+    if (tiles->tile_nodes == 5 * tiles->group_nodes) {
+        if (feat && listed) hipLaunchKernelGGL((edge_tile_pair_kernel<2, true, 5>), grid, dim3(256), 0, st, a2);
+        else if (feat) hipLaunchKernelGGL((edge_tile_pair_kernel<2, false, 5>), grid, dim3(256), 0, st, a2);
+        else if (listed) hipLaunchKernelGGL((edge_tile_pair_kernel<1, true, 5>), grid, dim3(256), 0, st, a2);
+        else hipLaunchKernelGGL((edge_tile_pair_kernel<1, false, 5>), grid, dim3(256), 0, st, a2);
+    } else {
+        if (feat && listed) hipLaunchKernelGGL((edge_tile_pair_kernel<2, true, 4>), grid, dim3(256), 0, st, a2);
+        else if (feat) hipLaunchKernelGGL((edge_tile_pair_kernel<2, false, 4>), grid, dim3(256), 0, st, a2);
+        else if (listed) hipLaunchKernelGGL((edge_tile_pair_kernel<1, true, 4>), grid, dim3(256), 0, st, a2);
+        else hipLaunchKernelGGL((edge_tile_pair_kernel<1, false, 4>), grid, dim3(256), 0, st, a2);
+    }
     timing_end(MSMP_K_EDGE_MLP, st);
     return check_launch("edge_tile_pair_kernel");
 }
diff --git a/msmp-pde_amd/graph.py b/msmp-pde_amd/graph.py
--- a/msmp-pde_amd/graph.py
+++ b/msmp-pde_amd/graph.py
@@ -29,6 +29,13 @@
             elif isinstance(v, GraphStructure):
                 self.__dict__[k] = None if torch.device(device) != v.rowptr.device else v
         return self
+
+
+def kernel_tile_groups(group_nodes, period_nodes, periodic4, align, want=0):
+    if want == 4 or 5 * group_nodes > _lib.MSMP_TILE_NCAP:
+        return 4
+    periodic5 = period_nodes is not None and (period_nodes % (5 * group_nodes) == 0 or align)
+    return 5 if want == 5 or periodic5 or not periodic4 else 4
 
 
 class GraphStructure(object):
@@ -60,6 +67,7 @@
         self._key = (edge_index.data_ptr(), tuple(edge_index.shape), edge_index._version,
                      batch.data_ptr(), batch._version)
         self._tiles = False
+        self._kernel_tiles = False
         self._period = False
 
     def period(self):
@@ -84,7 +92,6 @@
         if self.n_edges == 0 or self.max_in_degree <= 0 or self.max_in_degree > _lib.MSMP_TILE_GROUP_EDGES:
             return None
         L = lib()
-        dev = self.rowptr.device
         gn0 = min(_lib.MSMP_TILE_NCAP // 4, _lib.MSMP_TILE_GROUP_EDGES // self.max_in_degree)
         gn = gn0
         per = self.period()
@@ -100,21 +107,56 @@
             if periodic and n_tiles * n_meta >= 1 << 32:
                 periodic, n_src, e_src = False, self.n_nodes, self.n_edges
                 n_meta = n_tiles = (n_src + tn - 1) // tn
-            tile_node = torch.empty(n_meta * _lib.MSMP_TILE_NCAP, dtype=torch.int32, device=dev)
-            tile_count = torch.empty(n_meta, dtype=torch.int32, device=dev)
-            tile_halo = torch.empty(n_meta * 4, dtype=torch.int32, device=dev)
-            edge_slot = torch.empty(n_meta * _lib.MSMP_TILE_EDGES, dtype=torch.int32, device=dev)
-            stats = torch.empty(3, dtype=torch.int32, device=dev)
-            check(L.msmp_build_tiles(ptr(self.rowptr), ptr(self.col), n_src, e_src, gn, ptr(tile_node), ptr(tile_count),
-                                     ptr(tile_halo), ptr(edge_slot), ptr(stats), current_stream()), 'msmp_build_tiles')
-            max_nodes, max_edges, n_listed = (int(v) for v in stats.tolist())
-            if max_nodes <= _lib.MSMP_TILE_NCAP and max_edges <= _lib.MSMP_TILE_GROUP_EDGES:
-                desc = _lib.MsmpTiles(tn, gn, n_tiles, ptr(tile_node), ptr(tile_count), ptr(tile_halo), ptr(edge_slot), int(n_listed > 0),
-                                      n_meta if periodic else 0, n_src if periodic else 0)
-                self._tiles = (desc, tile_node, tile_count, edge_slot, tile_halo)
+            tiles, max_nodes = self._build_tiles(gn, 4, periodic, n_src, e_src, n_meta, n_tiles)
+            if tiles is not None:
+                self._tiles = tiles
                 return self._tiles
             gn -= max(1, -(-(max_nodes - _lib.MSMP_TILE_NCAP) // 4)) if max_nodes > _lib.MSMP_TILE_NCAP else 1
         return None
+
+    def _build_tiles(self, gn, groups, periodic, n_src, e_src, n_meta, n_tiles):
+        L = lib()
+        dev = self.rowptr.device
+        tile_node = torch.empty(n_meta * _lib.MSMP_TILE_NCAP, dtype=torch.int32, device=dev)
+        tile_count = torch.empty(n_meta, dtype=torch.int32, device=dev)
+        tile_halo = torch.empty(n_meta * 4, dtype=torch.int32, device=dev)
+        edge_slot = torch.empty(n_meta * _lib.MSMP_TILE_GROUP_EDGES * groups, dtype=torch.int32, device=dev)
+        stats = torch.empty(3, dtype=torch.int32, device=dev)
+        check(L.msmp_build_tiles_groups(ptr(self.rowptr), ptr(self.col), n_src, e_src, gn, groups, ptr(tile_node), ptr(tile_count),
+                                        ptr(tile_halo), ptr(edge_slot), ptr(stats), current_stream()), 'msmp_build_tiles_groups')
+        max_nodes, max_edges, n_listed = (int(v) for v in stats.tolist())
+        if max_nodes > _lib.MSMP_TILE_NCAP or max_edges > _lib.MSMP_TILE_GROUP_EDGES:
+            return None, max_nodes
+        desc = _lib.MsmpTiles(groups * gn, gn, n_tiles, ptr(tile_node), ptr(tile_count), ptr(tile_halo), ptr(edge_slot), int(n_listed > 0),
+                              n_meta if periodic else 0, n_src if periodic else 0)
+        return (desc, tile_node, tile_count, edge_slot, tile_halo), max_nodes
+
+    def tiles_for_kernel(self):
+        if self._kernel_tiles is not False:
+            return self._kernel_tiles
+        t4 = self.tiles()
+        self._kernel_tiles = t4
+        if t4 is None:
+            return t4
+        want = int(lib().msmp_tune_query(b'tile_groups'))
+        align = bool(lib().msmp_tune_query(b'tile_align'))
+        gn, per = t4[0].group_nodes, self.period()
+        if kernel_tile_groups(gn, per[0] if per else None, t4[0].period_tiles > 0, align, want) == 4:
+            return t4
+        tn = 5 * gn
+        periodic = per is not None and (per[0] % tn == 0 or align)
+        n_src, e_src = (per if periodic else (self.n_nodes, self.n_edges))
+        n_meta = (n_src + tn - 1) // tn
+        n_tiles = n_meta * (self.n_graphs if periodic else 1)
+        if periodic and n_tiles * n_meta >= 1 << 32:
+            if want != 5:
+                return t4
+            periodic, n_src, e_src = False, self.n_nodes, self.n_edges
+            n_meta = n_tiles = (n_src + tn - 1) // tn
+        t5, _ = self._build_tiles(gn, 5, periodic, n_src, e_src, n_meta, n_tiles)
+        if t5 is not None:
+            self._kernel_tiles = t5
+        return self._kernel_tiles
 
     @property
     def tgt_long(self):
diff --git a/msmp-pde_amd/layers.py b/msmp-pde_amd/layers.py
--- a/msmp-pde_amd/layers.py
+++ b/msmp-pde_amd/layers.py
@@ -166,7 +166,7 @@
     mode = main.MODE | (_lib.MSMP_LAYER_DENSE_MESSAGE if dense else 0)
     ws_bytes = L.msmp_mp_layer_workspace_bytes(n, gs.n_edges, int(gated), gs.max_in_degree)
     ws = _Workspace.get(ws_bytes, h.device)
-    tiles = gs.tiles()
+    tiles = gs.tiles_for_kernel()
     if decode is not None:
         c1, c2, u_last, dt, tw = decode
         w = [p.detach().to(torch.float32).contiguous() for p in (c1.weight, c1.bias, c2.weight, c2.bias)]
diff --git a/msmp-pde_amd/solvers.py b/msmp-pde_amd/solvers.py
--- a/msmp-pde_amd/solvers.py
+++ b/msmp-pde_amd/solvers.py
@@ -366,7 +366,7 @@
                 o += sub.x.shape[0]
             assert o == data.x.shape[0]
             for sub in subs:
-                structure_of(sub).tiles()
+                structure_of(sub).tiles_for_kernel()
             plan = plans[parts] = {'subs': subs, 'offs': offs, 'streams': [torch.cuda.Stream(device=data.x.device) for _ in subs]}
         return plan
 
@@ -401,7 +401,7 @@
         pos = data.pos
         gs = structure_of(data)
         tw = self.time_window
-        want_feat = not torch.is_grad_enabled() and self.hidden_features == 128 and gs.tiles() is not None
+        want_feat = not torch.is_grad_enabled() and self.hidden_features == 128 and gs.tiles_for_kernel() is not None
         prep = self._prepare(data, want_feat) if u_in.is_cuda else None
         if prep is not None:
             u, pos_x, pos_t, variables, feat = prep
```

Result: no change. 163.8 rollout-steps/s, median of 6 (+0.2%).
